# Amandaynzhou/CGC-Net

Hardware: AMD Instinct MI355X
Metric: cell-graphs/sec (fwd+bwd), batch=32, ~1800 nodes/16 feat (higher is better)
Workload: dtype f32; 1 GPU; C3: full CGC-Net (3 conv blocks + 2 DiffPool) fwd+bwd+Adam, 32 graphs/GPU/step, ~1803 nodes, ~16159 edges/graph, 16 feat, max_num_nodes=11404 (C1=1140, C2=114), flags=shipped; global_batch=32, nodes_per_batch=57711, parallelism=dp1, includes=CSR build + fwd + loss + bwd + grad all-reduce + Adam, step_sequencer=True, node_order=draw order, fused_adam=True, optimiser=cgc_adam_step (one launch; torch fused Adam arithmetic)

## Files before the change

### cgc-net_amd/csrc/exec.hip

```cpp
#include <stdio.h>
#include <stdlib.h>
#include <string.h>

#include "common.hpp"
#include "groups.hpp"

struct CatArgs {
  const float* src[4];
  int ld[4], width[4], off[4];
};
__global__ __launch_bounds__(256) void k_cat_cols(float* __restrict__ dst, int ldd, long long rows, int total_w, CatArgs a, int nsrc,
                                                  int accumulate) {
  const long long total = rows * total_w;
  for (long long i = blockIdx.x * 256ll + threadIdx.x; i < total; i += (long long)gridDim.x * 256) {
    const long long r = i / total_w;
    const int c = (int)(i - r * total_w);
    int s = 0;
#pragma unroll
    for (int k = 1; k < 4; ++k)
      if (k < nsrc && c >= a.off[k]) s = k;
    const float v = a.src[s][r * a.ld[s] + (c - a.off[s])];
    float* p = dst + r * ldd + c;
    *p = accumulate ? *p + v : v;
  }
}

extern "C" int cgc_cat_cols(float* dst, int ldd, int rows, int nsrc, const float* const* srcs, const int* lds, const int* widths,
                            int accumulate, cgc_stream_t stream) {
  if (nsrc < 1 || nsrc > 4) return CGC_EINVAL;
  CatArgs a;
  int off = 0;
  for (int k = 0; k < 4; ++k) {
    a.src[k] = k < nsrc ? srcs[k] : nullptr;
    a.ld[k] = k < nsrc ? lds[k] : 0;
    a.width[k] = k < nsrc ? widths[k] : 0;
    a.off[k] = off;
    off += a.width[k];
  }
  if (rows <= 0 || off <= 0) return 0;
  const long long total = (long long)rows * off;
  const long long blocks = (total + 255) / 256;
  hipLaunchKernelGGL(k_cat_cols, dim3((unsigned)(blocks < 4096 ? blocks : 4096)), dim3(256), 0, as_stream(stream), dst, ldd,
                     (long long)rows, off, a, nsrc, accumulate);
  CGC_RETURN_IF_LAUNCH_FAILED();
  return 0;
}

__global__ __launch_bounds__(256) void k_transpose(const float* __restrict__ src, int lds, int rows, int cols, float* __restrict__ dst,
                                                   int ldd) {
  __shared__ float t[32][33];
  const int tx = threadIdx.x & 31, ty = threadIdx.x >> 5;
  const int r0 = blockIdx.y * 32, c0 = blockIdx.x * 32;
  for (int j = ty; j < 32; j += 8) {
    const int r = r0 + j, c = c0 + tx;
    if (r < rows && c < cols) t[j][tx] = src[(size_t)r * lds + c];
  }
  __syncthreads();
  for (int j = ty; j < 32; j += 8) {
    const int c = c0 + j, r = r0 + tx;
    if (r < rows && c < cols) dst[(size_t)c * ldd + r] = t[tx][j];
  }
}

extern "C" int cgc_transpose(const float* src, int lds, int rows, int cols, float* dst, int ldd, cgc_stream_t stream) {
  if (rows <= 0 || cols <= 0) return 0;
  hipLaunchKernelGGL(k_transpose, dim3((unsigned)ceil_div(cols, 32), (unsigned)ceil_div(rows, 32)), dim3(256), 0, as_stream(stream), src,
                     lds, rows, cols, dst, ldd);
  CGC_RETURN_IF_LAUNCH_FAILED();
  return 0;
}

int reduce_batch_sum_rows(const float* ws, float* out, int parts, int rows, int width, int ldo, float beta, hipStream_t stream);

namespace {

struct Arena {
  float* base;
  size_t off = 0, high = 0;
  explicit Arena(float* b) : base(b) {}
  float* f(size_t n) {
    off = (off + 63) & ~(size_t)63;
    float* p = base + off;
    off += n;
    if (off > high) high = off;
    return p;
  }
  int* i(size_t n) { return reinterpret_cast<int*>(f(n)); }
  size_t mark() const { return off; }
  void release(size_t m) { off = m; }
};

struct Ctx {
  cgc_stream_t s;
  bool dry;
  Arena* scratch;
  float* gws;
  int64_t gws_floats;
  int gemm_mode = CGC_GEMM_EXACT;
};

static int fail_at(int rc, const char* what, int line) {
  static const bool verbose = getenv("CGC_EXEC_DEBUG") != nullptr;
  if (verbose) fprintf(stderr, "cgc exec.hip:%d: rc %d from %s\n", line, rc, what);
  return rc;
}
#define CALL(expr)                                              \
  do {                                                          \
    if (!c.dry) {                                               \
      const int rc__ = (expr);                                  \
      if (rc__ != 0) return fail_at(rc__, #expr, __LINE__);     \
    }                                                           \
  } while (0)
#define TRY(expr)                                               \
  do {                                                          \
    const int rc__ = (expr);                                    \
    if (rc__ != 0) return fail_at(rc__, #expr, __LINE__);       \
  } while (0)

inline int up(int v, int m) { return (v + m - 1) / m * m; }
inline int wide_ld(int F) { return (F >= 256 && F % 32 != 0) ? up(F, 32) : (F > 32 && F % 4 != 0) ? up(F, 4) : F; }
inline int pad4_ld(int c) { return (c > 32 && c % 4 != 0) ? up(c, 4) : c; }

int gemm(const Ctx& c, int tA, int tB, int M, int N, int K, const float* A, int lda, const float* B, int ldb, float beta, float* C, int ldc,
         const float* bias = nullptr, int batch = 1, int64_t sA = 0, int64_t sB = 0, int64_t sC = 0, const int* gptr = nullptr,
         int ragged = 0, int max_ragged = 0, int nx = 0, const float* const* xA = nullptr, const int* xlda = nullptr,
         const int64_t* xsA = nullptr, const float* const* xB = nullptr, const int* xldb = nullptr, const int64_t* xsB = nullptr,
         const int* xK = nullptr) {
  if (c.dry) return 0;
  return cgc_gemm_f32(tA, tB, M, N, K, 1.f, A, lda, B, ldb, beta, C, ldc, bias, batch, sA, sB, sC, gptr, ragged, max_ragged, nx, xA, xlda,
                      xsA, xB, xldb, xsB, xK, c.gws, c.gws_floats, c.gemm_mode, c.s);
}

int gemm_x1(const Ctx& c, int tA, int tB, int M, int N, int K, const float* A, int lda, const float* B, int ldb, float beta, float* C, int ldc,
            const float* bias, int batch, int64_t sA, int64_t sB, int64_t sC, const int* gptr, int ragged, int max_ragged, const float* xA,
            int xlda, int64_t xsA, const float* xB, int xldb, int64_t xsB, int xK) {
  return gemm(c, tA, tB, M, N, K, A, lda, B, ldb, beta, C, ldc, bias, batch, sA, sB, sC, gptr, ragged, max_ragged, 1, &xA, &xlda, &xsA,
              &xB, &xldb, &xsB, &xK);
}

int split_parts(int Fa, int Fb, int n) {
  const int tm = Fa <= 32 ? 32 : Fa <= 64 ? 64 : 128, tn = Fb <= 32 ? 32 : Fb <= 64 ? 64 : 128;
  const int tiles = ceil_div(Fa, tm) * ceil_div(Fb, tn);
  int best = 1;
  double best_score = -1.0;
  int hi = n / 512;
  if (hi > 128) hi = 128;
  if (hi < 1) hi = 1;
  for (int parts = 1; parts <= hi; ++parts) {
    const int blocks = tiles * parts, rounds = ceil_div(blocks, 512);
    const double fill = (double)blocks / ((double)rounds * 512.0);
    const double score = fill - 0.02 * rounds - (blocks < 256 ? 0.5 : 0.0);
    if (score > best_score + 1e-9) {
      best = parts;
      best_score = score;
    }
  }
  return best;
}

int gemm_tn_rows(const Ctx& c, const float* A, int lda, int Fa, const float* B, int ldb, int Fb, int n, float* out, int ldo = 0) {
  if (ldo <= 0) ldo = Fb;
  int parts = split_parts(Fa, Fb, n);
  if (parts == 1) return gemm(c, 1, 0, Fa, Fb, n, A, lda, B, ldb, 0.f, out, ldo);
  const int chunk = up(ceil_div(n, parts), 32);
  parts = ceil_div(n, chunk);
  const size_t m = c.scratch->mark();
  float* ws = c.scratch->f((size_t)parts * Fa * Fb);
  TRY(gemm(c, 1, 0, Fa, Fb, n, A, lda, B, ldb, 0.f, ws, Fb, nullptr, parts, 0, 0, (int64_t)Fa * Fb, nullptr, 3, chunk));
  CALL(reduce_batch_sum_rows(ws, out, parts, Fa, Fb, ldo, 0.f, as_stream(c.s)));
  c.scratch->release(m);
  return 0;
}

struct T3 {
  float* p;
  int b, r, c, ld;
  int64_t bs() const { return (int64_t)r * ld; }
};

int bgemm(const Ctx& c, const T3& A, const T3& B, const T3& C, int tA, int tB, float beta = 0.f) {
  const int batch = C.b, M = C.r, N = C.c, Kd = tA ? A.r : A.c;
  if (tA && !tB && M <= 128 && N <= 128 && Kd >= 512 && batch * 2 < 256 && C.ld == N) {
    int parts = Kd / 128;
    const int want = ceil_div(384, batch * (N > 64 ? 2 : 1));
    if (want < parts) parts = want;
    if (parts < 2) parts = 2;
    const int step = up(ceil_div(Kd, parts), 32);
    parts = ceil_div(Kd, step);
    const size_t m = c.scratch->mark();
    float* ws = c.scratch->f((size_t)batch * parts * M * N);
    TRY(gemm(c, 1, 0, M, N, Kd, A.p, A.ld, B.p, B.ld, 0.f, ws, N, nullptr, batch * parts, 0, 0, (int64_t)M * N, nullptr, 3, step));
    CALL(cgc_reduce_batched(ws, C.p, batch, parts, M * N, beta, c.s));
    c.scratch->release(m);
    return 0;
  }
  return gemm(c, tA, tB, M, N, Kd, A.p, A.ld, B.p, B.ld, beta, C.p, C.ld, nullptr, batch, A.bs(), B.bs(), C.bs());
}

int cat2(const Ctx& c, float* dst, int ldd, int rows, const float* a, int lda, int wa, const float* b, int ldb, int wb, int accumulate = 0) {
  const float* s[2] = {a, b};
  const int l[2] = {lda, ldb}, w[2] = {wa, wb};
  CALL(cgc_cat_cols(dst, ldd, rows, 2, s, l, w, accumulate, c.s));
  return 0;
}
int cat3(const Ctx& c, float* dst, int ldd, int rows, const float* a, int lda, int wa, const float* b, int ldb, int wb, const float* d, int ldd3,
         int wd) {
  const float* s[3] = {a, b, d};
  const int l[3] = {lda, ldb, ldd3}, w[3] = {wa, wb, wd};
  CALL(cgc_cat_cols(dst, ldd, rows, 3, s, l, w, 0, c.s));
  return 0;
}
int add1(const Ctx& c, float* dst, int ldd, int rows, const float* a, int lda, int wa) {
  const float* s[1] = {a};
  const int l[1] = {lda}, w[1] = {wa};
  CALL(cgc_cat_cols(dst, ldd, rows, 1, s, l, w, 1, c.s));
  return 0;
}

struct LayerP {
  const float *W, *b, *gamma, *beta;
  float *rm, *rv;
  int64_t* nbt;
  float eps, mom;
};
struct LayerS {
  float *hn, *rinv, *mean, *istd;
};

inline LayerP layer_params(const cgc_level_desc& d, const cgc_block_params* p, int k, int slot) {
  LayerP r;
  r.W = p->W[k];
  r.b = d.has_bias ? p->b[k] : nullptr;
  r.gamma = d.has_bn ? p->gamma[k] : nullptr;
  r.beta = d.has_bn ? p->beta[k] : nullptr;
  r.rm = d.has_bn ? p->running_mean[k] : nullptr;
  r.rv = d.has_bn ? p->running_var[k] : nullptr;
  r.nbt = d.has_bn ? p->num_batches_tracked[k] : nullptr;
  r.eps = d.bn_eps[slot];
  r.mom = d.bn_momentum[slot];
  return r;
}

inline size_t stats_ws_floats(int n, int F) { return (size_t)cgc_stats_ws_floats(n, F); }

int layer_fwd(const Ctx& c, const cgc_level_desc& d, const LayerP& p, const LayerS& s, const float* agg, int lda, int n, int fin, int F,
              float* y, int ldy, float* y2 = nullptr, int ldy2 = 0) {
  const size_t m = c.scratch->mark();
  const int batch_stats = d.has_bn && !d.eval;
  float* ws = batch_stats ? c.scratch->f(stats_ws_floats(n, F)) : nullptr;
  int fused = 0;
  if ((F >= 256 || F <= 32) && fin <= 32 && !c.dry) {
    int rc;
    if (F <= 32)
      rc = cgc_sage_narrow_fwd(agg, lda, p.W, p.b, n, fin, F, 1, d.act, s.hn, s.rinv, batch_stats, ws, d.count, p.eps, p.mom, p.rm, p.rv, p.nbt,
                               s.mean, s.istd, c.s);
    else
      rc = cgc_sage_wide_fwd(agg, lda, p.W, p.b, n, fin, F, 1, d.act, s.hn, F, s.rinv, batch_stats, ws, d.count, p.eps, p.mom, p.rm, p.rv, p.nbt,
                             s.mean, s.istd, c.s);
    if (rc == 0) fused = 1;
    else if (rc != CGC_EINVAL) return rc;
  }
  if (!fused) {
    TRY(gemm(c, 0, 0, n, F, fin, agg, lda, p.W, F, 0.f, s.hn, F, p.b));
    if (batch_stats)
      CALL(cgc_l2norm_act_bn(s.hn, n, F, 1, d.act, s.hn, s.rinv, ws, d.count, p.eps, p.mom, p.rm, p.rv, p.nbt, s.mean, s.istd, c.s));
    else
      CALL(cgc_l2norm_act_stats(s.hn, n, F, 1, d.act, s.hn, s.rinv, nullptr, nullptr, c.s));
  }
  if (d.has_bn && d.eval) CALL(cgc_bn_running_stats(p.rm, p.rv, F, p.eps, s.mean, s.istd, c.s));
  CALL(cgc_bn_act_apply(s.hn, n, F, d.act, d.has_bn ? s.mean : nullptr, s.istd, p.gamma, p.beta, y, ldy, y2, ldy2, c.s));
  c.scratch->release(m);
  return 0;
}

int layer_bwd(const Ctx& c, const cgc_level_desc& d, const LayerP& p, const LayerS& s, const float* agg, int lda, int n, int fin, int F,
              const float* dy, int ldy, float* dagg, int ldd, float* dwdb, float* sums) {
  const size_t m = c.scratch->mark();
  const int mode = d.has_bn ? 2 : 0;
  const size_t slot_floats = (size_t)(cgc_stats_blocks(n, F) > 1 ? cgc_stats_blocks(n, F) : 1) * 2 * F;
  if (d.has_bn) {
    float* ws = c.scratch->f(slot_floats);
    CALL(cgc_bn_bwd_reduce(dy, ldy, s.hn, n, F, d.act, s.mean, s.istd, sums, ws, c.s));
  }
  float* db = d.has_bias ? dwdb + (size_t)fin * F : nullptr;
  if (F <= 32 && fin <= 32) {
    float* ws = c.scratch->f((size_t)cgc_sage_narrow_ws_floats(n, fin, F));
    CALL(cgc_sage_narrow_bwd(dy, ldy, s.hn, s.rinv, n, F, d.act, 1, mode, s.mean, s.istd, p.gamma, d.has_bn ? sums : nullptr, d.count, agg,
                             lda, fin, p.W, dagg, ldd, dwdb, ws, c.s));
  } else {
    float* dh = c.scratch->f((size_t)n * F);
    float* ws = db ? c.scratch->f(slot_floats) : nullptr;
    CALL(cgc_bn_act_l2_bwd(dy, ldy, s.hn, s.rinv, n, F, d.act, 1, mode, s.mean, s.istd, p.gamma, d.has_bn ? sums : nullptr, d.count, dh, db, ws,
                           c.s));
    if (dagg) TRY(gemm(c, 0, 1, n, fin, F, dh, F, p.W, F, 0.f, dagg, ldd));
    TRY(gemm_tn_rows(c, agg, lda, fin, dh, F, F, n, dwdb));
  }
  c.scratch->release(m);
  return 0;
}

inline bool pairable(int fin_e, int F_e, int fin_p, int F_p) { return fin_e == fin_p && F_e == F_p && fin_e <= 32 && F_e <= 32; }

int layer_fwd_pair(const Ctx& c, const cgc_level_desc& d, const LayerP* p, const LayerS* s, const float* const* agg, int lda, int n, int fin, int F,
                   float* const* y, int ldy, float* const* y2, const int* ldy2) {
  const size_t m = c.scratch->mark();
  SnFwdPtrs g[2];
  SnFwdBn bn[2];
  BnApplyPtrs ap[2];
  const int batch_stats = d.has_bn && !d.eval;
  for (int i = 0; i < 2; ++i) {
    float* ws = batch_stats ? c.scratch->f(stats_ws_floats(n, F)) : nullptr;
    g[i] = SnFwdPtrs{agg[i], p[i].W, p[i].b, s[i].hn, s[i].rinv, ws};
    bn[i] = SnFwdBn{p[i].eps, p[i].mom, p[i].rm, p[i].rv, p[i].nbt, s[i].mean, s[i].istd};
    ap[i] = BnApplyPtrs{s[i].hn, d.has_bn ? s[i].mean : nullptr, s[i].istd, p[i].gamma, p[i].beta, y[i], y2[i], ldy2[i]};
  }
  CALL(sage_narrow_fwd_groups(g, bn, 2, lda, n, fin, F, 1, d.act, batch_stats, d.count, as_stream(c.s)));
  if (d.has_bn && d.eval)
    for (int i = 0; i < 2; ++i) CALL(cgc_bn_running_stats(p[i].rm, p[i].rv, F, p[i].eps, s[i].mean, s[i].istd, c.s));
  CALL(bn_act_apply_groups(ap, 2, n, F, d.act, ldy, as_stream(c.s)));
  c.scratch->release(m);
  return 0;
}

int layer_bwd_pair(const Ctx& c, const cgc_level_desc& d, const LayerP* p, const LayerS* s, const float* const* agg, int lda, int n, int fin, int F,
                   const float* const* dy, int ldy, float* const* dagg, int ldd, float* const* dwdb, float* const* sums) {
  const size_t m = c.scratch->mark();
  const int mode = d.has_bn ? 2 : 0;
  const size_t slot_floats = (size_t)(cgc_stats_blocks(n, F) > 1 ? cgc_stats_blocks(n, F) : 1) * 2 * F;
  if (d.has_bn) {
    BnRedPtrs r[2];
    for (int i = 0; i < 2; ++i) r[i] = BnRedPtrs{dy[i], s[i].hn, s[i].mean, s[i].istd, c.scratch->f(slot_floats)};
    CALL(bn_bwd_reduce_groups(r, sums, 2, ldy, n, F, d.act, as_stream(c.s)));
  }
  SnBwdPtrs g[2];
  for (int i = 0; i < 2; ++i)
    g[i] = SnBwdPtrs{dy[i], s[i].hn, s[i].rinv, s[i].mean, s[i].istd, p[i].gamma, d.has_bn ? sums[i] : nullptr, agg[i], p[i].W, dagg[i],
                     c.scratch->f((size_t)cgc_sage_narrow_ws_floats(n, fin, F))};
  CALL(sage_narrow_bwd_groups(g, dwdb, 2, ldy, n, F, d.act, 1, mode, d.count, lda, fin, ldd, as_stream(c.s)));
  c.scratch->release(m);
  return 0;
}

struct Level {
  const cgc_level_desc& d;
  int n, B, R, fin, H, E, AH, C, D, D3, wp, wt, ldp, ldC, ldP, ldW, ftot, npad_jk, seg_nmax;
  bool dense, pool, tall;
  float *At, *An, *invd, *ge1, *agg0, *pair[2], *xcat, *aggk[2], *hp3, *cat_e, *HS, *CS, *jk_out, *x12, *S, *P;
  float *G, *keep;
  bool reg;
  double reg_numel, reg_rows;
  int* arg;
  LayerS L[6];
  cgc_level_grad_layout gl;

  explicit Level(const cgc_level_desc& dd) : d(dd) {
    n = d.n; B = d.B; R = d.rows_per_graph; fin = d.fin; H = d.H; E = d.E; AH = d.AH; C = d.C;
    dense = d.level >= 2;
    pool = C > 0;
    D3 = 2 * H + E;
    D = d.jk ? H : D3;
    wp = pool ? H + AH : H;
    wt = 2 * wp + fin;
    ldp = dense ? wt : wp;
    ldC = pool ? wide_ld(C) : 0;
    ldP = dense ? pad4_ld(C) : ldC;
    ftot = 2 * AH + C;
    tall = pool && n >= 8 * C;
    ldW = wide_ld(C);
    npad_jk = up(n > 1 ? n : 1, 1024);
    seg_nmax = dense ? R : d.npad;
    reg = pool && (d.flags & 8);
    const double N = dense ? R : d.npad;
    reg_numel = (double)B * N * N;
    reg_rows = (double)B * N;
    memset(&gl, 0, sizeof(gl));
  }

  void layout_saved(Arena& a) {
    At = An = invd = ge1 = nullptr;
    if (dense) {
      if (d.renorm) At = a.f((size_t)n * R);
      An = a.f((size_t)n * R);
      invd = a.f(n);
      ge1 = a.f(n);
    }
    agg0 = a.f((size_t)n * fin);
    xcat = dense ? a.f((size_t)n * wt) : nullptr;
    for (int k = 0; k < 2; ++k) {
      pair[k] = dense ? xcat + (1 - k) * wp : a.f((size_t)n * wp);
      aggk[k] = a.f((size_t)n * wp);
    }
    hp3 = pool ? a.f((size_t)n * ldC) : nullptr;
    for (int k = 0; k < 6; ++k) {
      const bool emb = k < 3;
      if (!emb && !pool) {
        L[k].hn = L[k].rinv = L[k].mean = L[k].istd = nullptr;
        continue;
      }
      const int F = width_out(k);
      L[k].hn = a.f((size_t)n * F);
      L[k].rinv = a.f(n);
      L[k].mean = a.f(F);
      L[k].istd = a.f(F);
    }
    cat_e = a.f((size_t)n * D3);
    HS = CS = jk_out = nullptr;
    if (d.jk) {
      const int Hh = 3 * H / 2;
      HS = a.f((size_t)6 * Hh * npad_jk);
      CS = a.f((size_t)6 * Hh * npad_jk);
      jk_out = a.f((size_t)n * H);
    }
    arg = a.i((size_t)B * D);
    x12 = S = P = nullptr;
    if (pool) {
      x12 = a.f((size_t)n * 2 * AH);
      S = a.f((size_t)n * ldC);
      P = a.f((size_t)n * ldP);
    }
    G = keep = nullptr;
    if (reg) {
// ... 84 lines not shown
  TRY(aggregate(c, L, g, gptr, x_in, L.fin, L.fin, L.agg0));
  if (L.dense) {
    const float* s1[1] = {x_in};
    const int l1[1] = {L.fin}, w1[1] = {L.fin};
    CALL(cgc_cat_cols(L.xcat + 2 * wp, L.wt, n, 1, s1, l1, w1, 0, c.s));
  }
  for (int k = 0; k < 3; ++k) {
    const float* ain = k == 0 ? L.agg0 : L.aggk[k - 1];
    const int lda = k == 0 ? L.fin : wp;
    if (k < 2 && L.pool && pairable(L.width_in(k), H, L.width_in(3 + k), AH)) {
      const LayerP pp[2] = {layer_params(d, emb, k, k), layer_params(d, pl, k, 3 + k)};
      const LayerS ss[2] = {L.L[k], L.L[3 + k]};
      const float* ag[2] = {ain, k == 0 ? ain : ain + H};
      float* yy[2] = {L.pair[k], L.pair[k] + H};
      float* y2[2] = {L.cat_e + k * H, L.x12 + k * AH};
      const int l2[2] = {L.D3, 2 * AH};
      TRY(layer_fwd_pair(c, d, pp, ss, ag, lda, n, L.width_in(k), H, yy, L.ldp, y2, l2));
      if (k < 2) TRY(aggregate(c, L, g, gptr, L.pair[k], L.ldp, wp, L.aggk[k]));
      continue;
    }
    if (k < 2)
      TRY(layer_fwd(c, d, layer_params(d, emb, k, k), L.L[k], ain, lda, n, L.width_in(k), L.width_out(k), L.pair[k], L.ldp, L.cat_e + k * H,
                    L.D3));
    else
      TRY(layer_fwd(c, d, layer_params(d, emb, k, k), L.L[k], ain, lda, n, L.width_in(k), L.width_out(k), L.cat_e + 2 * H, L.D3));
    if (L.pool) {
      const float* ainp = k == 0 ? ain : ain + H;
      if (k < 2)
        TRY(layer_fwd(c, d, layer_params(d, pl, k, 3 + k), L.L[3 + k], ainp, lda, n, L.width_in(3 + k), L.width_out(3 + k), L.pair[k] + H, L.ldp,
                      L.x12 + k * AH, 2 * AH));
      else
        TRY(layer_fwd(c, d, layer_params(d, pl, k, 3 + k), L.L[3 + k], ainp, lda, n, L.width_in(3 + k), L.width_out(3 + k), L.hp3, L.ldC));
    }
    if (k < 2) TRY(aggregate(c, L, g, gptr, L.pair[k], L.ldp, wp, L.aggk[k]));
  }
  if (d.jk) CALL(cgc_jk_lstm_fwd(L.cat_e, n, L.npad_jk, H, jk->lstm, jk->w_att, jk->b_att, L.jk_out, L.HS, L.CS, c.s));
  CALL(cgc_segment_max_fwd(L.embed(), gptr, L.B, L.D, L.seg_nmax, readout, L.arg, c.s));
  if (!L.pool) return 0;
  {
    const bool wide_main = C > 2 * AH;
    const float* xm = wide_main ? L.hp3 : L.x12;
    const float* xe = wide_main ? L.x12 : L.hp3;
    const int ldm = wide_main ? L.ldC : 2 * AH, lde = wide_main ? 2 * AH : L.ldC;
    const int wm = wide_main ? C : 2 * AH, we = wide_main ? 2 * AH : C;
    const int om = wide_main ? 2 * AH : 0, oe = wide_main ? 0 : 2 * AH;
    if (L.tall) {
      const size_t m = c.scratch->mark();
      float* wt = c.scratch->f((size_t)L.ftot * L.ldW);
      CALL(cgc_transpose(pl->lin_W, L.ftot, C, L.ftot, wt, L.ldW, c.s));
      TRY(gemm_x1(c, 0, 0, n, C, wm, xm, ldm, wt + (size_t)om * L.ldW, L.ldW, 0.f, L.S, L.ldC, pl->lin_b, 1, 0, 0, 0, nullptr, 0, 0, xe, lde, 0,
                  wt + (size_t)oe * L.ldW, L.ldW, 0, we));
      c.scratch->release(m);
    } else {
      TRY(gemm_x1(c, 0, 1, n, C, wm, xm, ldm, pl->lin_W + om, L.ftot, 0.f, L.S, L.ldC, pl->lin_b, 1, 0, 0, 0, nullptr, 0, 0, xe, lde, 0,
                  pl->lin_W + oe, L.ftot, 0, we));
    }
  }
  CALL(cgc_softmax_fwd(L.S, n, C, L.ldC, L.S, c.s));
  if (!L.dense) {
    CALL(cgc_spmm_graphs(g->rowptr, g->col, nullptr, g->val, nullptr, nullptr, L.S, L.P, n, C, L.ldC, gptr, L.B, d.nmax, 1 | (g->spatial ? 4 : 0), g->gorder, c.s));
    TRY(gemm(c, 1, 0, C, L.D, 0, L.S, L.ldC, L.embed(), L.D, 0.f, x_out, L.D, nullptr, L.B, 0, 0, (int64_t)C * L.D, gptr, 2, d.nmax));
    TRY(gemm(c, 1, 0, C, C, 0, L.S, L.ldC, L.P, L.ldC, 0.f, A_out, C, nullptr, L.B, 0, 0, (int64_t)C * C, gptr, 2, d.nmax));
  } else {
    const T3 s3{L.S, L.B, L.R, C, L.ldC}, e3{const_cast<float*>(L.embed()), L.B, L.R, L.D, L.D}, p3{L.P, L.B, L.R, C, L.ldP};
    const T3 a3{const_cast<float*>(d.renorm ? L.At : A_in), L.B, L.R, L.R, L.R};
    TRY(bgemm(c, s3, e3, T3{x_out, L.B, C, L.D, L.D}, 1, 0));
    TRY(bgemm(c, a3, s3, p3, 0, 0));
    TRY(bgemm(c, s3, p3, T3{A_out, L.B, C, C, C}, 1, 0));
  }
  if (L.reg) TRY(reg_fwd(c, L, g, gptr, A_in, A_out, reg_out));
  return 0;
}

int level_bwd_blocks(const Ctx& c, Level& L, const cgc_block_params* emb, const cgc_block_params* pl, const cgc_jk_params* jk,
                     const cgc_graph* g, const int* gptr, const float* x_in, const float* A_in, float* d_embed, const float* dx12,
                     float* dagg1, const float* gAt, float* grads, float* d_x_in, float* d_A_in) {
  const cgc_level_desc& d = L.d;
  Arena& sc = *c.scratch;
  const int n = L.n, H = L.H, AH = L.AH, wp = L.wp, B = L.B, R = L.R, D3 = L.D3, fin = L.fin;
  auto sums = [&](int k) { return grads + L.gl.W[k] + (int64_t)L.width_in(k) * L.width_out(k) + L.width_out(k); };
  float* d_cat = d_embed;
  if (d.jk) {
    d_cat = sc.f((size_t)n * D3);
    const size_t m = sc.mark();
    float* ws = sc.f((size_t)cgc_jk_bwd_ws_floats(H));
    CALL(cgc_jk_lstm_bwd_flat(L.cat_e, d_embed, n, L.npad_jk, H, jk->lstm, jk->w_att, jk->b_att, L.HS, L.CS, d_cat, grads + L.gl.jk, ws, c.s));
    sc.release(m);
  }
  float* dagg[2];
  const int ldg = L.ldp;
  float* const gcat = dagg1 != nullptr ? dagg1 : sc.f((size_t)n * ldg);
  dagg[1] = gcat;
  TRY(layer_bwd(c, d, layer_params(d, emb, 2, 2), L.L[2], L.aggk[1], wp, n, H, L.E, d_cat + 2 * H, D3, dagg[1], ldg, grads + L.gl.W[2], sums(2)));
  float* dpair = nullptr;
  for (int k = 1; k >= 0; --k) {
    dpair = sc.f((size_t)n * wp);
    TRY(aggregate_t(c, L, g, gptr, dagg[k], ldg, wp, dpair));
    if (L.pool) TRY(cat2(c, dpair, wp, n, d_cat + k * H, D3, H, dx12 + k * AH, 2 * AH, AH, 1));
    else TRY(add1(c, dpair, wp, n, d_cat + k * H, D3, H));
    const bool first = k == 0;
    const bool need_in = !first || L.dense;
    const float* ain = first ? L.agg0 : L.aggk[k - 1];
    const int lda = first ? fin : wp;
    const int fi_e = L.width_in(k), fi_p = L.width_in(3 + k);
    float *de = nullptr, *dp = nullptr;
    int ldd = ldg;
    if (need_in && !first) {
      de = dagg[0] = L.dense ? gcat + wp : sc.f((size_t)n * wp);
      dp = de + H;
    } else if (need_in) {
      de = gcat + 2 * wp;
      dp = L.pool ? sc.f((size_t)n * ldg) : nullptr;
    }
    if (L.pool && pairable(fi_e, H, fi_p, AH)) {
      const LayerP pp[2] = {layer_params(d, emb, k, k), layer_params(d, pl, k, 3 + k)};
      const LayerS ss[2] = {L.L[k], L.L[3 + k]};
      const float* ag[2] = {ain, first ? ain : ain + H};
      const float* dyy[2] = {dpair, dpair + H};
      float* dg[2] = {de, dp};
      float* dw[2] = {grads + L.gl.W[k], grads + L.gl.W[3 + k]};
      float* sm[2] = {sums(k), sums(3 + k)};
      TRY(layer_bwd_pair(c, d, pp, ss, ag, lda, n, fi_e, H, dyy, wp, dg, ldd, dw, sm));
    } else {
      TRY(layer_bwd(c, d, layer_params(d, emb, k, k), L.L[k], ain, lda, n, fi_e, H, dpair, wp, de, ldd, grads + L.gl.W[k], sums(k)));
      if (L.pool)
        TRY(layer_bwd(c, d, layer_params(d, pl, k, 3 + k), L.L[3 + k], first ? ain : ain + H, lda, n, fi_p, AH, dpair + H, wp, dp, ldd,
                      grads + L.gl.W[3 + k], sums(3 + k)));
    }
    if (first && L.dense) {
      if (L.pool) TRY(add1(c, de, ldg, n, dp, ldg, fin));
      TRY(aggregate_t(c, L, g, gptr, de, ldg, fin, d_x_in));
      float* dAn = sc.f((size_t)n * R);
      TRY(bgemm(c, T3{gcat, B, R, L.wt, L.wt}, T3{L.xcat, B, R, L.wt, L.wt}, T3{dAn, B, R, R, R}, 0, 1));
      CALL(cgc_adj_prep_bwd(A_in, L.An, L.invd, L.ge1, dAn, gAt, n, R, d.renorm ? d.renorm_p : -1.f, d_A_in, c.s));
    }
  }
  return 0;
}

int level_bwd(const Ctx& c, Level& L, const cgc_block_params* emb, const cgc_block_params* pl, const cgc_jk_params* jk, const cgc_graph* g,
              const int* gptr, const float* x_in, const float* A_in, const float* d_readout, const float* d_xo, const float* d_ao, float* grads,
              float* d_x_in, float* d_A_in, const float* d_reg = nullptr) {
  const cgc_level_desc& d = L.d;
  Arena& sc = *c.scratch;
  const int n = L.n, H = L.H, AH = L.AH, wp = L.wp, C = L.C, D = L.D, B = L.B, R = L.R;
  float* d_embed = sc.f((size_t)n * D);
  CALL(cgc_segment_max_bwd_full(d_readout, L.arg, gptr, B, D, L.seg_nmax, d_embed, c.s));
  float *dx12 = nullptr, *gAt = nullptr;
  if (L.pool) {
    float *Gs = nullptr, *coef = nullptr;
    if (L.reg) {
      float* dao = sc.f((size_t)B * C * C);
      Gs = sc.f((size_t)B * C * C);
      coef = sc.f(4);
      CALL(cgc_diffpool_reg_bwd_prep(d_reg, L.keep, L.reg_numel, L.reg_rows, d_ao, dao, L.G, Gs, B, C, coef, c.s));
      d_ao = dao;
    }
    const size_t m0 = sc.mark();
    float* ds = sc.f((size_t)n * L.ldC);
    if (!L.dense) {
      float* dp = sc.f((size_t)n * L.ldC);
      TRY(gemm(c, 0, 0, 0, C, C, L.S, L.ldC, d_ao, C, 0.f, dp, L.ldC, nullptr, B, 0, (int64_t)C * C, 0, gptr, 1, d.nmax));
      CALL(cgc_spmm_graphs(g->t_rowptr, g->t_col, nullptr, g->t_val, nullptr, nullptr, dp, ds, n, C, L.ldC, gptr, B, d.nmax, 2 | (g->spatial ? 4 : 0), g->gorder,
                           c.s));
      TRY(gemm_x1(c, 0, 1, 0, C, C, L.P, L.ldC, d_ao, C, 1.f, ds, L.ldC, nullptr, B, 0, (int64_t)C * C, 0, gptr, 1, d.nmax, L.embed(), D, 0, d_xo,
                  D, (int64_t)C * D, D));
      if (L.reg) TRY(gemm(c, 0, 0, 0, C, C, L.S, L.ldC, Gs, C, 1.f, ds, L.ldC, nullptr, B, 0, (int64_t)C * C, 0, gptr, 1, d.nmax));
      TRY(gemm(c, 0, 0, 0, D, C, L.S, L.ldC, d_xo, D, 1.f, d_embed, D, nullptr, B, 0, (int64_t)C * D, 0, gptr, 1, d.nmax));
    } else {
      gAt = sc.f((size_t)n * R);
      float* dP = sc.f((size_t)n * L.ldP);
      const T3 s3{L.S, B, R, C, L.ldC}, e3{const_cast<float*>(L.embed()), B, R, D, D}, p3{L.P, B, R, C, L.ldP};
      const T3 a3{const_cast<float*>(d.renorm ? L.At : A_in), B, R, R, R};
      const T3 dao{const_cast<float*>(d_ao), B, C, C, C}, dxo{const_cast<float*>(d_xo), B, C, D, D};
      const T3 ds3{ds, B, R, C, L.ldC}, dP3{dP, B, R, C, L.ldP};
      TRY(bgemm(c, p3, dao, ds3, 0, 1));
      TRY(bgemm(c, s3, dao, dP3, 0, 0));
      TRY(bgemm(c, dP3, s3, T3{gAt, B, R, R, R}, 0, 1));
      TRY(bgemm(c, a3, dP3, ds3, 1, 0, 1.f));
      TRY(bgemm(c, e3, dxo, ds3, 0, 1, 1.f));
      TRY(bgemm(c, s3, dxo, T3{d_embed, B, R, D, D}, 0, 0, 1.f));
      if (L.reg) {
        TRY(bgemm(c, s3, T3{Gs, B, C, C, C}, ds3, 0, 0, 1.f));
        CALL(cgc_diffpool_reg_adj_bwd(a3.p, (int64_t)n * R, coef, gAt, 1, c.s));
      }
    }
    if (L.reg) CALL(cgc_diffpool_reg_entropy_bwd(L.S, n, C, L.ldC, coef, ds, L.ldC, c.s));
    float* dz = sc.f((size_t)n * L.ldC);
    {
      const size_t m = sc.mark();
      float* ws = sc.f((size_t)(cgc_stats_blocks(n, C) > 1 ? cgc_stats_blocks(n, C) : 1) * 2 * C);
      CALL(cgc_softmax_bwd(L.S, ds, n, C, L.ldC, dz, grads + L.gl.lin_b, ws, c.s));
      sc.release(m);
    }
    dx12 = sc.f((size_t)n * 2 * AH);
    float* dy3 = sc.f((size_t)n * L.ldC);
    TRY(gemm(c, 0, 0, n, 2 * AH, C, dz, L.ldC, pl->lin_W, L.ftot, 0.f, dx12, 2 * AH));
    TRY(gemm(c, 0, 0, n, C, C, dz, L.ldC, pl->lin_W + 2 * AH, L.ftot, 0.f, dy3, L.ldC));
    {
      float* dW = grads + L.gl.lin_W;
      TRY(gemm_tn_rows(c, dz, L.ldC, C, L.x12, 2 * AH, 2 * AH, n, dW, L.ftot));
      TRY(gemm_tn_rows(c, dz, L.ldC, C, L.hp3, L.ldC, C, n, dW + 2 * AH, L.ftot));
    }
    (void)m0;
    float* dagg1 = sc.f((size_t)n * L.ldp);
    TRY(layer_bwd(c, d, layer_params(d, pl, 2, 5), L.L[5], L.aggk[1] + H, wp, n, AH, C, dy3, L.ldC, dagg1 + H, L.ldp, grads + L.gl.W[5],
                  grads + L.gl.W[5] + (int64_t)AH * C + C));
    return level_bwd_blocks(c, L, emb, pl, jk, g, gptr, x_in, A_in, d_embed, dx12, dagg1, gAt, grads, d_x_in, d_A_in);
  }
  return level_bwd_blocks(c, L, emb, pl, jk, g, gptr, x_in, A_in, d_embed, nullptr, nullptr, nullptr, grads, d_x_in, d_A_in);
}

template <class Body>
int run_level(const cgc_level_desc* d, float* saved, float* scratch, cgc_stream_t stream, Body&& body) {
  Level L(*d);
  Arena sv(saved), sc(scratch);
  L.layout_saved(sv);
  L.layout_grads();
  Ctx c{stream, false, &sc, nullptr, cgc_gemm_ws_floats()};
  c.gws = sc.f((size_t)c.gws_floats);
  c.gemm_mode = (d->flags & 2) ? CGC_GEMM_SPLIT_BF16 : (d->flags & 4) ? CGC_GEMM_SPLIT_F16 : CGC_GEMM_EXACT;
  return body(c, L);
}

}

extern "C" int cgc_level_supported(const cgc_level_desc* d) {
  if (d == nullptr || d->level < 1 || d->level > 3 || d->B < 1 || d->B > 65535 || d->n < 1) return 0;
  if (d->fin < 1 || d->H < 1 || d->E < 1 || d->act < 0 || d->act > 3) return 0;
  if (d->level >= 2 && (d->rows_per_graph < 1 || (long long)d->B * d->rows_per_graph != d->n)) return 0;
  if (d->level == 1 && (d->nmax < 1 || d->npad < d->nmax)) return 0;
  if (d->C > 0 && (d->AH < 1 || d->H + d->AH > 256 || (2 * d->AH) % 4 != 0)) return 0;
  if (d->C == 0 && d->level == 1) return 0;
  if ((d->flags & ~14) || (d->flags & 6) == 6) return 0;
  if ((d->flags & 8) && d->C == 0) return 0;
  if (d->jk && (d->E != d->H || !cgc_jk_matrix_core(d->H))) return 0;
  return 1;
}

extern "C" int64_t cgc_level_saved_floats(const cgc_level_desc* d) {
  if (!cgc_level_supported(d)) return -1;
  Level L(*d);
  Arena a(nullptr);
  L.layout_saved(a);
  return (int64_t)a.high + 64;
}

extern "C" int cgc_level_grad_layout_of(const cgc_level_desc* d, cgc_level_grad_layout* out) {
  if (!cgc_level_supported(d) || out == nullptr) return CGC_EINVAL;
  Level L(*d);
  L.layout_grads();
  *out = L.gl;
  return 0;
}

extern "C" int64_t cgc_level_scratch_floats(const cgc_level_desc* d) {
  if (!cgc_level_supported(d)) return -1;
  Level L(*d);
  Arena sv(nullptr);
  L.layout_saved(sv);
  L.layout_grads();
  size_t high = 0;
  for (int pass = 0; pass < (d->eval ? 1 : 2); ++pass) {
    Arena sc(nullptr);
    Ctx c{nullptr, true, &sc, nullptr, 0};
    sc.f((size_t)cgc_gemm_ws_floats());
    cgc_block_params bp;
    memset(&bp, 0, sizeof(bp));
    cgc_jk_params jp;
    memset(&jp, 0, sizeof(jp));
    cgc_graph gr;
    memset(&gr, 0, sizeof(gr));
    const int rc = pass == 0 ? level_fwd(c, L, &bp, &bp, &jp, &gr, nullptr, nullptr, nullptr, nullptr, nullptr, nullptr)
                             : level_bwd(c, L, &bp, &bp, &jp, &gr, nullptr, nullptr, nullptr, nullptr, nullptr, nullptr, nullptr, nullptr, nullptr);
    if (rc != 0) return -1;
    if (sc.high > high) high = sc.high;
  }
  return (int64_t)high + 64;
}

extern "C" int cgc_level_fwd(const cgc_level_desc* d, const cgc_block_params* emb, const cgc_block_params* pool, const cgc_jk_params* jk,
                             const cgc_graph* g, const int* gptr, const float* x_in, const float* A_in, float* saved, float* scratch,
                             float* readout, float* x_out, float* A_out, const float** assign_out, int* assign_ld, float* reg_out,
                             cgc_stream_t stream) {
  if (!cgc_level_supported(d) || saved == nullptr || scratch == nullptr) return CGC_EINVAL;
  if (!aligned16(saved) || !aligned16(scratch)) return CGC_EINVAL;
  if ((d->flags & 8) && reg_out == nullptr) return CGC_EINVAL;
  return run_level(d, saved, scratch, stream, [&](const Ctx& c, Level& L) {
    const int rc = level_fwd(c, L, emb, pool, jk, g, gptr, x_in, A_in, readout, x_out, A_out, reg_out);
    if (assign_out != nullptr) *assign_out = L.S;
    if (assign_ld != nullptr) *assign_ld = L.ldC;
    return rc;
  });
}

extern "C" int cgc_level_bwd(const cgc_level_desc* d, const cgc_block_params* emb, const cgc_block_params* pool, const cgc_jk_params* jk,
                             const cgc_graph* g, const int* gptr, const float* x_in, const float* A_in, const float* saved, float* scratch,
                             const float* d_readout, const float* d_x_out, const float* d_A_out, const float* d_reg, float* grads,
                             float* d_x_in, float* d_A_in, cgc_stream_t stream) {
  if (!cgc_level_supported(d) || saved == nullptr || scratch == nullptr || grads == nullptr || d->eval) return CGC_EINVAL;
  if (!aligned16(saved) || !aligned16(scratch) || !aligned16(grads)) return CGC_EINVAL;
  if ((d->flags & 8) && d_reg == nullptr) return CGC_EINVAL;
  return run_level(d, const_cast<float*>(saved), scratch, stream, [&](const Ctx& c, Level& L) {
    return level_bwd(c, L, emb, pool, jk, g, gptr, x_in, A_in, d_readout, d_x_out, d_A_out, grads, d_x_in, d_A_in, d_reg);
  });
}
```

### cgc-net_amd/csrc/gemm.hip

```cpp
#include "gemm_common.hpp"

template <int ROWS>
struct KContigLoader {
  static constexpr int UNITS = ROWS * (BK / 4);
  static constexpr int PER_T = (UNITS + 255) / 256;
  float4 reg[PER_T];
  __device__ __forceinline__ void load(const float* __restrict__ base, int ld, int row0, int row_lim, int k0, int k_lim, bool vec_ok) {
#pragma unroll
    for (int i = 0; i < PER_T; ++i) {
      const int u = threadIdx.x + i * 256;
      float4 v = make_float4(0.f, 0.f, 0.f, 0.f);
      if (UNITS % 256 == 0 || u < UNITS) {
        const int row = row0 + u / (BK / 4);
        const int k = k0 + (u % (BK / 4)) * 4;
        if (row < row_lim && k < k_lim) {
          const float* p = base + (size_t)row * ld + k;
          if (vec_ok && k + 3 < k_lim) {
            v = *reinterpret_cast<const float4*>(p);
          } else {
            v.x = p[0];
            if (k + 1 < k_lim) v.y = p[1];
            if (k + 2 < k_lim) v.z = p[2];
            if (k + 3 < k_lim) v.w = p[3];
          }
        }
      }
      reg[i] = v;
    }
  }
  __device__ __forceinline__ void load_fast(const float* __restrict__ base, int ld, int row0, int row_last, int k0) {
#pragma unroll
    for (int i = 0; i < PER_T; ++i) {
      const int u = threadIdx.x + i * 256;
      const int row = min(row0 + u / (BK / 4), row_last);
      reg[i] = *reinterpret_cast<const float4*>(base + (size_t)row * ld + k0 + (u % (BK / 4)) * 4);
    }
  }
  __device__ __forceinline__ void offsets(unsigned (&off)[PER_T], int ld, int row0, int row_last) const {
#pragma unroll
    for (int i = 0; i < PER_T; ++i) {
      const int u = threadIdx.x + i * 256;
      off[i] = (unsigned)min(row0 + u / (BK / 4), row_last) * (unsigned)ld * 4u + (unsigned)(u % (BK / 4)) * 16u;
    }
  }
  static __device__ __forceinline__ unsigned tile_soffset(int , int k0) { return (unsigned)k0 * 4u; }
  __device__ __forceinline__ void load_buf_part(int i, __amdgpu_buffer_rsrc_t rsrc, const unsigned (&off)[PER_T], unsigned soff) {
    reg[i] = __builtin_bit_cast(float4, __builtin_amdgcn_raw_buffer_load_b128(rsrc, off[i], soff, 0));
  }
  __device__ __forceinline__ void load_fast_masked(const float* __restrict__ base, int ld, int row0, int row_last, int k0, int k_lim) {
    const int k_last4 = (k_lim - 1) & ~3;
#pragma unroll
    for (int i = 0; i < PER_T; ++i) {
      const int u = threadIdx.x + i * 256;
      const int row = min(row0 + u / (BK / 4), row_last);
      const int k = k0 + (u % (BK / 4)) * 4;
      float4 v = *reinterpret_cast<const float4*>(base + (size_t)row * ld + min(k, k_last4));
      if (k >= k_lim) v.x = 0.f;
      if (k + 1 >= k_lim) v.y = 0.f;
      if (k + 2 >= k_lim) v.z = 0.f;
      if (k + 3 >= k_lim) v.w = 0.f;
      reg[i] = v;
    }
  }
  __device__ __forceinline__ void store_part(int i, float* __restrict__ lds) const {
    const int u = threadIdx.x + i * 256;
    if (UNITS % 256 == 0 || u < UNITS)
      *reinterpret_cast<float4*>(&lds[(u / (BK / 4)) * KC_LD + (u % (BK / 4)) * 4]) = reg[i];
  }
  __device__ __forceinline__ void store(float* __restrict__ lds) const {
#pragma unroll
    for (int i = 0; i < PER_T; ++i) store_part(i, lds);
  }
};

template <int COLS>
struct MnContigLoader {
  static constexpr int UNITS = BK * (COLS / 4);
  static constexpr int PER_T = (UNITS + 255) / 256;
  float4 reg[PER_T];
  __device__ __forceinline__ void load(const float* __restrict__ base, int ld, int col0, int col_lim, int k0, int k_lim, bool vec_ok) {
#pragma unroll
    for (int i = 0; i < PER_T; ++i) {
      const int u = threadIdx.x + i * 256;
// ... 485 lines not shown
  if (ragged == 1 && (transA || a.gptr == nullptr)) return CGC_EINVAL;
  if (ragged == 2 && (!transA || transB || a.gptr == nullptr || a.nx > 0)) return CGC_EINVAL;
  if (ragged == 3 && (!transA || transB || a.nx > 0 || max_ragged <= 0 || K <= 0 || batch % ceil_div(K, max_ragged) != 0)) return CGC_EINVAL;
  if (ragged < 0 || ragged > 3) return CGC_EINVAL;
  a.chunk = ragged == 3 ? max_ragged : 0;
  const int m_extent = ragged == 1 ? max_ragged : M;
  if (m_extent <= 0) return 0;
  const int k_extent = ragged >= 2 ? max_ragged : K;
  constexpr int shortk_max = 160, fill_min = 448;
  const bool sk = k_extent <= shortk_max && a.nx == 0;
  const long long fill = (long long)ceil_div(m_extent, 128) * batch;
  const bool want_split = mode == CGC_GEMM_SPLIT_BF16, want_half = mode == CGC_GEMM_SPLIT_F16;
  auto big_route = [&](bool shortk, float* w) -> int {
    if ((want_split || want_half) && !shortk && !(transA && transB) && gemm_all_fast(a, transA, transB, batch, m_extent, k_extent)) {
      int rc = want_half ? gemm_half_launch(a, transA, transB, batch, m_extent, k_extent, w, ws_floats, stream) : CGC_EINVAL;
      if (rc == CGC_EINVAL) rc = gemm_split_launch(a, transA, transB, batch, m_extent, k_extent, w, ws_floats, stream);
      if (rc != CGC_EINVAL) return rc;
    }
    return launch_cfg<2, 2, 2, 2>(a, transA, transB, batch, m_extent, k_extent, shortk, w, ws_floats, stream);
  };
  const int force = g_force_cfg;
  if (force > 0) {
    const bool fsk = force >= 20 ? true : force >= 10 ? false : sk;
    switch (force % 10) {
      case 1: return big_route(fsk, ws);
      case 2: return launch_cfg<4, 1, 1, 2>(a, transA, transB, batch, m_extent, k_extent, fsk, ws, ws_floats, stream);
      case 3: return launch_cfg<1, 4, 2, 1>(a, transA, transB, batch, m_extent, k_extent, fsk, ws, ws_floats, stream);
      case 4: return launch_cfg<2, 2, 1, 1>(a, transA, transB, batch, m_extent, k_extent, fsk, ws, ws_floats, stream);
      case 5: return launch_cfg<4, 1, 1, 1>(a, transA, transB, batch, m_extent, k_extent, fsk, ws, ws_floats, stream);
      case 6: return launch_cfg<1, 4, 1, 1>(a, transA, transB, batch, m_extent, k_extent, fsk, ws, ws_floats, stream);
      default: break;
    }
  }
  if (N <= 32) return launch_cfg<4, 1, 1, 1>(a, transA, transB, batch, m_extent, k_extent, sk, ws, ws_floats, stream);
  if (N <= 64) {
    if (m_extent > 64 && fill < fill_min) return launch_cfg<2, 2, 1, 1>(a, transA, transB, batch, m_extent, k_extent, sk, ws, ws_floats, stream);
    return launch_cfg<4, 1, 1, 2>(a, transA, transB, batch, m_extent, k_extent, sk, ws, ws_floats, stream);
  }
  if (m_extent <= 32) return launch_cfg<1, 4, 1, 1>(a, transA, transB, batch, m_extent, k_extent, sk, ws, ws_floats, stream);
  if (m_extent <= 64) return launch_cfg<1, 4, 2, 1>(a, transA, transB, batch, m_extent, k_extent, sk, ws, ws_floats, stream);
  if (fill * ceil_div(N, 128) < fill_min) {
    if (N <= 128) {
      if (k_extent > 256 && m_extent > 128)
        return launch_cfg<4, 1, 1, 1>(a, transA, transB, batch, m_extent, k_extent, sk, ws, ws_floats, stream);
      return launch_cfg<2, 2, 1, 1>(a, transA, transB, batch, m_extent, k_extent, sk, ws, ws_floats, stream);
    }
    if (transA) {
      if (!sk && ws != nullptr && k_extent >= 24 * BK) return big_route(sk, ws);
      return launch_cfg<4, 1, 1, 2>(a, transA, transB, batch, m_extent, k_extent, sk, ws, ws_floats, stream);
    }
    return launch_cfg<1, 4, 2, 1>(a, transA, transB, batch, m_extent, k_extent, sk, ws, ws_floats, stream);
  }
  return big_route(sk, ws);
}

extern "C" int cgc_gemm_f32(int transA, int transB, int M, int N, int K, float alpha, const float* A, int lda, const float* B, int ldb,
                            float beta, float* C, int ldc, const float* bias, int batch, int64_t strideA, int64_t strideB,
                            int64_t strideC, const int* gptr, int ragged, int max_ragged, int nx, const float* const* xA,
                            const int* xlda, const int64_t* xstrideA, const float* const* xB, const int* xldb,
                            const int64_t* xstrideB, const int* xK, float* ws, int64_t ws_floats, int mode, cgc_stream_t stream_) {
  if (nx < 0 || nx > 2) return CGC_EINVAL;
  if (mode != CGC_GEMM_EXACT && mode != CGC_GEMM_SPLIT_BF16 && mode != CGC_GEMM_SPLIT_F16) return CGC_EINVAL;
  GemmArgs a;
  a.A = A; a.B = B; a.C = C; a.bias = bias; a.gptr = gptr;
  a.M = M; a.N = N; a.K = K; a.lda = lda; a.ldb = ldb; a.ldc = ldc;
  a.strideA = strideA; a.strideB = strideB; a.strideC = strideC;
  a.alpha = alpha; a.beta = beta; a.ragged = ragged; a.tiles_n = 0;
  a.per_batch = a.nb = 0; a.ws = nullptr; a.resident = 0; a.s_max = 1; a.chunk = 0; a.scale = nullptr;
  for (int i = 0; i < 2; ++i) { a.xA[i] = a.xB[i] = nullptr; a.xlda[i] = a.xldb[i] = a.xK[i] = 0; a.xsA[i] = a.xsB[i] = 0; }
  int kept = 0;
  for (int i = 0; i < nx; ++i) {
    if (xK[i] <= 0) continue;
    a.xA[kept] = xA[i]; a.xB[kept] = xB[i]; a.xlda[kept] = xlda[i]; a.xldb[kept] = xldb[i]; a.xK[kept] = xK[i];
    a.xsA[kept] = xstrideA[i]; a.xsB[kept] = xstrideB[i];
    ++kept;
  }
  a.nx = kept;
  return gemm_dispatch(a, transA, transB, batch, max_ragged, ws, ws_floats, mode, as_stream(stream_));
}

__global__ void k_reduce_batch_sum(const float* __restrict__ ws, float* __restrict__ out, int parts, long long numel, float beta, int width,
                                   int ldo) {
  for (long long i = blockIdx.x * (long long)blockDim.x + threadIdx.x; i < numel; i += (long long)gridDim.x * blockDim.x) {
    float s = 0.f;
    for (int p = 0; p < parts; ++p) s += ws[(size_t)p * numel + i];
    const long long o = (i / width) * ldo + i % width;
    out[o] = beta != 0.f ? s + beta * out[o] : s;
  }
}

__global__ __launch_bounds__(256) void k_reduce_many_parts(const float* __restrict__ ws, float* __restrict__ out, int parts, int numel,
                                                           float beta, int width, int ldo) {
  __shared__ float part[8][32];
  const int cl = threadIdx.x & 31, grp = threadIdx.x >> 5;
  const int c = blockIdx.x * 32 + cl;
  ws += (size_t)blockIdx.y * parts * numel;
  out += (size_t)blockIdx.y * numel;
  float s = 0.f;
  if (c < numel) {
    float a[8];
#pragma unroll
    for (int u = 0; u < 8; ++u) a[u] = 0.f;
    int k = grp;
    for (; k + 56 < parts; k += 64) {
#pragma unroll
      for (int u = 0; u < 8; ++u) a[u] += ws[(size_t)(k + 8 * u) * numel + c];
    }
    for (; k < parts; k += 8) a[0] += ws[(size_t)k * numel + c];
    s = ((a[0] + a[1]) + (a[2] + a[3])) + ((a[4] + a[5]) + (a[6] + a[7]));
  }
  part[grp][cl] = s;
  __syncthreads();
  if (grp == 0 && c < numel) {
    float t = part[0][cl];
#pragma unroll
    for (int g = 1; g < 8; ++g) t += part[g][cl];
    const int o = (c / width) * ldo + c % width;
    out[o] = beta != 0.f ? t + beta * out[o] : t;
  }
}

extern "C" int cgc_reduce_batched(const float* ws, float* out, int outer, int parts, int numel, float beta, cgc_stream_t stream) {
  if (numel <= 0 || outer <= 0) return 0;
  if (outer > 65535) return CGC_EINVAL;
  hipLaunchKernelGGL(k_reduce_many_parts, dim3((unsigned)ceil_div(numel, 32), (unsigned)outer), dim3(256), 0, as_stream(stream), ws, out,
                     parts, numel, beta, numel, numel);
  CGC_RETURN_IF_LAUNCH_FAILED();
  return 0;
}

int reduce_batch_sum_rows(const float* ws, float* out, int parts, int rows, int width, int ldo, float beta, hipStream_t stream) {
  const int64_t numel = (int64_t)rows * width;
  if (numel <= 0) return 0;
  if (width <= 0 || ldo < width || numel > 0x7fffffff) return CGC_EINVAL;
  if (parts >= 16 && numel <= (1 << 20)) {
    hipLaunchKernelGGL(k_reduce_many_parts, dim3((unsigned)ceil_div((int)numel, 32), 1u), dim3(256), 0, stream, ws, out, parts, (int)numel, beta,
                       width, ldo);
  } else {
    const int64_t blocks = ceil_div64(numel, 256);
    hipLaunchKernelGGL(k_reduce_batch_sum, dim3((unsigned)(blocks < 4096 ? blocks : 4096)), dim3(256), 0, stream, ws, out, parts,
                       (long long)numel, beta, width, ldo);
  }
  CGC_RETURN_IF_LAUNCH_FAILED();
  return 0;
}

extern "C" int cgc_reduce_batch_sum(const float* ws, float* out, int parts, int64_t numel, float beta, cgc_stream_t stream) {
  if (numel <= 0) return 0;
  if (parts >= 16 && numel <= (1 << 20)) return cgc_reduce_batched(ws, out, 1, parts, (int)numel, beta, stream);
  const int64_t blocks = ceil_div64(numel, 256);
  const int w = numel <= 0x7fffffff ? (int)numel : 0x7fffffff;
  hipLaunchKernelGGL(k_reduce_batch_sum, dim3((unsigned)(blocks < 4096 ? blocks : 4096)), dim3(256), 0, as_stream(stream), ws, out,
                     parts, (long long)numel, beta, w, w);
  CGC_RETURN_IF_LAUNCH_FAILED();
  return 0;
}
```

### cgc-net_amd/csrc/groups.hpp

```cpp
#pragma once
#include "common.hpp"

struct SnFwdPtrs {
  const float *agg, *W, *bias;
  float *hn, *rinv, *ws;
};
struct SnFwdBn {
  float eps, momentum;
  float *running_mean, *running_var;
  int64_t* nbt;
  float *mean, *istd;
};
struct SnBwdPtrs {
  const float *dy, *hn, *rinv, *mean, *istd, *gamma, *sums, *agg, *W;
  float *dagg, *ws;
};
struct StatsFinPtrs {
  const float* ws;
  float *running_mean, *running_var, *mean, *istd;
  long long* nbt;
  float eps, momentum;
};
struct BnApplyPtrs {
  const float *hn, *mean, *istd, *gamma, *beta;
  float *y, *y2;
  int ldy2;
};
struct BnRedPtrs {
  const float *dy, *hn, *mean, *istd;
  float* ws;
};

int sage_narrow_fwd_groups(const SnFwdPtrs* g, const SnFwdBn* bn, int ng, int lda, int n, int K, int F, int normalize, int act, int stats,
                           double count, hipStream_t st);
int sage_narrow_bwd_groups(const SnBwdPtrs* g, float* const* dwdb, int ng, int ldy, int n, int F, int act, int normalize, int mode, double count,
                           int lda, int fin, int ldd, hipStream_t st);
int bn_act_apply_groups(const BnApplyPtrs* g, int ng, int n, int F, int act, int ldy, hipStream_t stream);
int bn_bwd_reduce_groups(const BnRedPtrs* g, float* const* sums, int ng, int ldy, int n, int F, int act, hipStream_t stream);
int launch_stats_finalize_groups(const StatsFinPtrs* g, int ng, int slots, int F, double count, hipStream_t stream);
int launch_reduce_slots_f32_pair(const float* ws0, float* out0, const float* ws1, float* out1, int ng, int slots, int width, hipStream_t stream);
```

### cgc-net_amd/csrc/jk.hip

```cpp
#include "jk.hpp"

template <int C>
__device__ __forceinline__ void jk_fill_lds(const JkWeights& w, float4* Wt, float4* B4, float* watt, int nthreads) {
  constexpr int H = JkDims<C>::H, KIN = JkDims<C>::KIN;
  for (int idx = threadIdx.x; idx < 2 * H * KIN; idx += nthreads) {
    const int d = idx / (H * KIN), rem = idx - d * H * KIN, j = rem / KIN, k = rem - j * KIN;
    float v[4];
#pragma unroll
    for (int g = 0; g < 4; ++g) {
      const int row = g * H + j;
      v[g] = k < C ? w.w_ih[d][row * C + k] : w.w_hh[d][row * H + (k - C)];
    }
    Wt[idx] = make_float4(v[0], v[1], v[2], v[3]);
  }
  for (int idx = threadIdx.x; idx < 2 * H; idx += nthreads) {
    const int d = idx / H, j = idx - d * H;
    float v[4];
#pragma unroll
    for (int g = 0; g < 4; ++g) v[g] = w.b_ih[d][g * H + j] + w.b_hh[d][g * H + j];
    B4[idx] = make_float4(v[0], v[1], v[2], v[3]);
    watt[idx] = w.w_att[idx];
  }
  if (threadIdx.x == 0) watt[2 * H] = w.b_att[0];
}
// ... 255 lines not shown
extern "C" int cgc_jk_matrix_core(int C) { return C == 4 || C == 8 || C == 12 || C == 16 || C == 20; }

#define JK_FOR_EACH_C(X) X(2) X(4) X(6) X(8) X(10) X(12) X(14) X(16) X(18) X(20) X(22) X(24) X(26) X(28) X(30) X(32)

template <int C>
static void jk_allow_lds() {
  static bool done_f[CGC_MAX_DEVICES] = {}, done_b[CGC_MAX_DEVICES] = {};
  cgc_allow_lds(reinterpret_cast<const void*>(&k_jk_fwd<C>), (int)JkDims<C>::lds_bytes, done_f);
  cgc_allow_lds(reinterpret_cast<const void*>(&k_jk_bwd<C>), (int)JkDims<C>::lds_bytes, done_b);
}

template <int C>
static int launch_jk_fwd(const float* xs, int n, int npad, const JkWeights& w, float* out, float* HS, float* CS, hipStream_t st) {
  jk_allow_lds<C>();
  hipLaunchKernelGGL(k_jk_fwd<C>, dim3(ceil_div(2 * n, JK_THREADS)), dim3(JK_THREADS), JkDims<C>::lds_bytes, st, xs, n, npad, w, out, HS, CS);
  CGC_RETURN_IF_LAUNCH_FAILED();
  return 0;
}
template <int C>
static int launch_jk_bwd(const float* xs, const float* dout, int n, int npad, const JkWeights& w, const float* HS, const float* CS,
                         float* dxs, float* DGT, float* INT, float* DHC, hipStream_t st) {
  jk_allow_lds<C>();
  hipLaunchKernelGGL(k_jk_bwd<C>, dim3(ceil_div(2 * npad, JK_THREADS)), dim3(JK_THREADS), JkDims<C>::lds_bytes, st, xs, dout, n, npad, w,
                     HS, CS, dxs, DGT, INT, DHC);
  CGC_RETURN_IF_LAUNCH_FAILED();
  return 0;
}

extern "C" int cgc_jk_lstm_fwd(const float* xs, int n, int npad, int C, const float* const* lstm, const float* w_att,
                               const float* b_att, float* out, float* HS, float* CS, cgc_stream_t stream) {
  if (n <= 0) return 0;
  if (!jk_npad_ok(n, npad)) return CGC_EINVAL;
  JkWeights w;
  fill_weights(w, lstm, w_att, b_att);
  const int rc = jk_mfma_fwd(xs, n, npad, C, w, out, HS, CS, as_stream(stream));
  if (rc != CGC_EINVAL) return rc;
  switch (C) {
#define X(C_) case C_: return launch_jk_fwd<C_>(xs, n, npad, w, out, HS, CS, as_stream(stream));
    JK_FOR_EACH_C(X)
#undef X
    default: return CGC_EINVAL;
  }
}

extern "C" int cgc_jk_lstm_bwd(const float* xs, const float* dout, int n, int npad, int C, const float* const* lstm,
                               const float* w_att, const float* b_att, const float* HS, const float* CS, float* dxs, float* DGT,
                               float* INT, float* DHC, cgc_stream_t stream) {
  if (n <= 0) return 0;
  if (!jk_npad_ok(n, npad)) return CGC_EINVAL;
  JkWeights w;
  fill_weights(w, lstm, w_att, b_att);
  const int rc = jk_mfma_bwd(xs, dout, n, npad, C, w, HS, CS, dxs, DGT, INT, as_stream(stream));
  if (rc != CGC_EINVAL) return rc;
  switch (C) {
#define X(C_) case C_: return launch_jk_bwd<C_>(xs, dout, n, npad, w, HS, CS, dxs, DGT, INT, DHC, as_stream(stream));
    JK_FOR_EACH_C(X)
#undef X
    default: return CGC_EINVAL;
  }
}

extern "C" int64_t cgc_jk_bwd_ws_floats(int C) { return jk_mfma_bwd_ws_floats(C); }

extern "C" int cgc_jk_lstm_bwd_params(const float* xs, const float* dout, int n, int npad, int C, const float* const* lstm,
                                      const float* w_att, const float* b_att, const float* HS, const float* CS, float* dxs,
                                      float* G, float* ws, cgc_stream_t stream) {
  if (n <= 0) return 0;
  if (!jk_npad_ok(n, npad)) return CGC_EINVAL;
  JkWeights w;
  fill_weights(w, lstm, w_att, b_att);
  return jk_mfma_bwd_params(xs, dout, n, npad, C, w, HS, CS, dxs, G, ws, as_stream(stream));
}

extern "C" int cgc_jk_lstm_bwd_flat(const float* xs, const float* dout, int n, int npad, int C, const float* const* lstm,
                                    const float* w_att, const float* b_att, const float* HS, const float* CS, float* dxs,
                                    float* flat, float* ws, cgc_stream_t stream) {
  if (n <= 0) return 0;
  if (!jk_npad_ok(n, npad)) return CGC_EINVAL;
  JkWeights w;
  fill_weights(w, lstm, w_att, b_att);
  return jk_mfma_bwd_flat(xs, dout, n, npad, C, w, HS, CS, dxs, flat, ws, as_stream(stream));
}

__global__ void k_jk_unpack(const float* __restrict__ G, int C, int H, float* __restrict__ flat) {
  const int NI = C + 2 * H + 1, NG = 4 * H + 1;
  const int per_dir = 4 * H * C + 4 * H * H + 8 * H, total = 2 * per_dir + 2 * H + 1;
  for (int i = blockIdx.x * blockDim.x + threadIdx.x; i < total; i += gridDim.x * blockDim.x) {
    float v;
    if (i < 2 * per_dir) {
      const int d = i / per_dir;
      int e = i - d * per_dir;
      const float* Gd = G + (size_t)d * NG * NI;
      if (e < 4 * H * C) v = Gd[(e / C) * NI + (e % C)];
      else if ((e -= 4 * H * C) < 4 * H * H) v = Gd[(e / H) * NI + C + (e % H)];
      else { e -= 4 * H * H; v = Gd[(e % (4 * H)) * NI + C + H]; }
    } else {
      const int e = i - 2 * per_dir;
      if (e < 2 * H) v = G[((size_t)(e / H) * NG + 4 * H) * NI + C + H + 1 + (e % H)];
      else v = G[(size_t)(4 * H) * NI + C + H];
    }
    flat[i] = v;
  }
}

extern "C" int64_t cgc_jk_param_grad_floats(int C) {
  const int64_t H = 3 * (int64_t)C / 2;
  return 2 * (4 * H * C + 4 * H * H + 8 * H) + 2 * H + 1;
}

extern "C" int cgc_jk_unpack_param_grads(const float* G, int C, float* flat, cgc_stream_t stream) {
  if (C <= 0) return CGC_EINVAL;
  const int H = 3 * C / 2;
  const int total = (int)cgc_jk_param_grad_floats(C);
  hipLaunchKernelGGL(k_jk_unpack, dim3(ceil_div(total, 256)), dim3(256), 0, as_stream(stream), G, C, H, flat);
  CGC_RETURN_IF_LAUNCH_FAILED();
  return 0;
}
```

### cgc-net_amd/csrc/jk.hpp

```cpp
#pragma once
#include "common.hpp"

__device__ __forceinline__ float sigmoidf_(float x) { return 1.f / (1.f + expf(-x)); }

template <int C>
struct JkDims {
  static constexpr int H = 3 * C / 2;
  static constexpr int KIN = C + H;
  static constexpr size_t lds_bytes = sizeof(float4) * (2 * H * KIN + 2 * H) + sizeof(float) * (2 * H + 4);
};

struct JkWeights {
  const float* w_ih[2];
  const float* w_hh[2];
  const float* b_ih[2];
  const float* b_hh[2];
  const float* w_att;
  const float* b_att;
};


int jk_mfma_fwd(const float* xs, int n, int npad, int C, const JkWeights& w, float* out, float* HS, float* CS, hipStream_t st);
int jk_mfma_bwd(const float* xs, const float* dout, int n, int npad, int C, const JkWeights& w, const float* HS, const float* CS,
                float* dxs, float* DGT, float* INT, hipStream_t st);
int64_t jk_mfma_bwd_ws_floats(int C);
int jk_mfma_bwd_params(const float* xs, const float* dout, int n, int npad, int C, const JkWeights& w, const float* HS,
                       const float* CS, float* dxs, float* G, float* ws, hipStream_t st);
int jk_mfma_bwd_flat(const float* xs, const float* dout, int n, int npad, int C, const JkWeights& w, const float* HS, const float* CS,
                     float* dxs, float* flat, float* ws, hipStream_t st);
```

### cgc-net_amd/csrc/jk_mfma.hip

```cpp
#include "jk.hpp"

typedef float floatx16 __attribute__((ext_vector_type(16)));

constexpr int JKB_TILES = 2;
constexpr int JKB_THREADS = JKB_TILES * 128;

template <int C>
struct JkM {
  static constexpr int H = 3 * C / 2;
  static constexpr int XG = (C + 7) / 8;
  static constexpr int HG = (H + 7) / 8;
  static constexpr int NQ = XG + HG;
  static constexpr int W_FLOATS = 2 * 4 * NQ * 32 * 8;
  static constexpr int B_OFF = W_FLOATS;
  static constexpr int A_OFF = B_OFF + 2 * 4 * 32;
  static constexpr int S_OFF = A_OFF + 2 * 32 + 4;
  static constexpr int TOTAL = S_OFF + 2 * 2 * 3 * 32;
  static_assert(H <= 32 && C % 4 == 0, "one 32-row tile per gate; 16-byte x fragments");
};

__device__ __forceinline__ float jk_rcp(float d) {
  const float r = __builtin_amdgcn_rcpf(d);
  return fmaf(fmaf(-d, r, 1.f), r, r);
}
__device__ __forceinline__ float jk_exp(float a) {
  const float t = a * 0x1.715476p+0f;
  const float r = fmaf(a, 0x1.4ae0cp-26f, fmaf(a, 0x1.715476p+0f, -t));
  const float e = __builtin_amdgcn_exp2f(t);
  return fmaf(e, t >= 16.f ? r * 0x1.62e43p-1f : 0.f, e);
}
__device__ __forceinline__ float fast_sigmoid(float x) { return jk_rcp(1.f + jk_exp(fminf(-x, 87.f))); }
__device__ __forceinline__ float fast_tanh(float x) {
  const float ax = fabsf(x), x2 = x * x;
  const float e = __expf(-2.f * ax);
  const float big = (1.f - e) * jk_rcp(1.f + e);
  const float small = ax * fmaf(x2, fmaf(x2, fmaf(x2, fmaf(x2, 62.f / 2835.f, -17.f / 315.f), 2.f / 15.f), -1.f / 3.f), 1.f);
  return copysignf(ax < 0.25f ? small : big, x);
}

template <int C>
__device__ __forceinline__ void jkm_fill(const JkWeights& w, float* lds, int nthreads) {
  using M = JkM<C>;
  constexpr int H = M::H, XG = M::XG, NQ = M::NQ;
  {
    const int tt = threadIdx.x & 3, lhi = (threadIdx.x >> 2) & 1, j = (threadIdx.x >> 3) & 31;
    float v[2 * 4 * NQ];
#pragma unroll
    for (int it = 0; it < 2 * 4 * NQ; ++it) {
      const int q = it % NQ, g = (it / NQ) & 3, d = it / (4 * NQ);
      v[it] = 0.f;
      if (q < XG) {
        const int k = 8 * q + 4 * lhi + tt;
        if (j < H && k < C) v[it] = w.w_ih[d][(g * H + j) * C + k];
      } else {
        const int k = 8 * (q - XG) + 4 * lhi + tt;
        if (j < H && k < H) v[it] = w.w_hh[d][(g * H + j) * H + k];
      }
    }
#pragma unroll
    for (int it = 0; it < 2 * 4 * NQ; ++it) lds[it * 256 + threadIdx.x] = v[it];
  }
  for (int idx = threadIdx.x; idx < 2 * 4 * 32; idx += nthreads) {
    const int j = idx & 31, g = (idx >> 5) & 3, d = idx >> 7;
    lds[M::B_OFF + idx] = j < H ? w.b_ih[d][g * H + j] + w.b_hh[d][g * H + j] : 0.f;
  }
  for (int idx = threadIdx.x; idx < 2 * 32; idx += nthreads) {
    const int j = idx & 31, d = idx >> 5;
    lds[M::A_OFF + idx] = j < H ? w.w_att[d * H + j] : 0.f;
  }
  if (threadIdx.x == 0) lds[M::A_OFF + 64] = w.b_att[0];
}

template <int C>
__global__ __launch_bounds__(JKB_THREADS) void k_jk_bwd_mfma(const float* __restrict__ xs, const float* __restrict__ dout, int n, int npad,
                                                     const JkWeights w, const float* __restrict__ HS, const float* __restrict__ CS,
                                                     float* __restrict__ dxs, float* __restrict__ DGT, float* __restrict__ INT,
                                                     float* __restrict__ ) {
  using M = JkM<C>;
  constexpr int H = M::H, XG = M::XG, HG = M::HG, NQ = M::NQ;
  constexpr int NG = 4 * H + 1, NI = C + 2 * H + 1;
  extern __shared__ __attribute__((aligned(16))) float lds[];
  if (threadIdx.x < 256) jkm_fill<C>(w, lds, 256);
  __syncthreads();
// ... 146 lines not shown
        if (8 * q + 4 * lhi < C) {
          inT[(size_t)(8 * q + 4 * lhi + 0) * ktot + col] = xt[q].x;
          inT[(size_t)(8 * q + 4 * lhi + 1) * ktot + col] = xt[q].y;
          inT[(size_t)(8 * q + 4 * lhi + 2) * ktot + col] = xt[q].z;
          inT[(size_t)(8 * q + 4 * lhi + 3) * ktot + col] = xt[q].w;
        }
      }
#pragma unroll
      for (int q = 0; q < HG; ++q) {
        const float4 wa = *reinterpret_cast<const float4*>(Al + 8 * q);
        const float was[4] = {wa.x, wa.y, wa.z, wa.w};
#pragma unroll
        for (int u = 0; u < 4; ++u) {
          const int r = 4 * q + u, j = u + 8 * q + 4 * lhi;
          const float gi = fast_sigmoid(acc[0][r]), gf = fast_sigmoid(acc[1][r]);
          const float gg = fast_tanh(acc[2][r]), go = fast_sigmoid(acc[3][r]);
          const float c = gf * cprev[r] + gi * gg;
          const float th = fast_tanh(c);
          const float dh = fmaf(dst, was[u], dhc[r]);
          const float dc = fmaf(dh * go, 1.f - th * th, dcc[r]);
          dcc[r] = dc * gf;
          const float qi = dc * gg * gi * (1.f - gi), qf = dc * cprev[r] * gf * (1.f - gf);
          const float qg = dc * gi * (1.f - gg * gg), qo = dh * th * go * (1.f - go);
          acc[0][r] = qi; acc[1][r] = qf; acc[2][r] = qg; acc[3][r] = qo;
          if (8 * q + u < H && j < H) {
            dgt[(size_t)(0 * H + j) * ktot + col] = qi;
            dgt[(size_t)(1 * H + j) * ktot + col] = qf;
            dgt[(size_t)(2 * H + j) * ktot + col] = qg;
            dgt[(size_t)(3 * H + j) * ktot + col] = qo;
            inT[(size_t)(C + j) * ktot + col] = hprev[r];
            inT[(size_t)(C + H + 1 + j) * ktot + col] = go * th;
          }
        }
      }
      floatx16 dh2, dx2;
#pragma unroll
      for (int r = 0; r < 16; ++r) { dh2[r] = 0.f; dx2[r] = 0.f; }
#pragma unroll
      for (int g = 0; g < 4; ++g)
#pragma unroll
        for (int q = 0; q < HG; ++q) {
          float ah[4], ax[4];
#pragma unroll
          for (int u = 0; u < 4; ++u) {
            ax[u] = WtX[g * NQ * 256 + (8 * q + u) * 8];
            ah[u] = s > 0 ? WtH[g * NQ * 256 + (8 * q + u) * 8] : 0.f;
          }
#pragma unroll
          for (int u = 0; u < 4; ++u) {
            dx2 = __builtin_amdgcn_mfma_f32_32x32x2f32(ax[u], acc[g][4 * q + u], dx2, 0, 0, 0);
            if (s > 0) dh2 = __builtin_amdgcn_mfma_f32_32x32x2f32(ah[u], acc[g][4 * q + u], dh2, 0, 0, 0);
          }
        }
      if (s > 0) dhc = dh2;
#pragma unroll
      for (int q = 0; q < XG; ++q) Ex[(t * XG + q) * 64] = make_float4(dx2[4 * q + 0], dx2[4 * q + 1], dx2[4 * q + 2], dx2[4 * q + 3]);
    }

    __syncthreads();
    if (d == 0 && valid) {
      const float4* Eo = Ex + 3 * XG * 64;
#pragma unroll
      for (int q = 0; q < XG; ++q) {
        if (8 * q + 4 * lhi < C) {
          const float4 dy = *reinterpret_cast<const float4*>(dout + (size_t)node * C + 8 * q + 4 * lhi);
#pragma unroll
          for (int t = 0; t < 3; ++t) {
            const float4 p0 = Ex[(t * XG + q) * 64], p1 = Eo[(t * XG + q) * 64];
            float4 v;
            v.x = fmaf(a3[t], dy.x, p0.x + p1.x); v.y = fmaf(a3[t], dy.y, p0.y + p1.y);
            v.z = fmaf(a3[t], dy.z, p0.z + p1.z); v.w = fmaf(a3[t], dy.w, p0.w + p1.w);
            *reinterpret_cast<float4*>(dxs + (size_t)node * 3 * C + t * C + 8 * q + 4 * lhi) = v;
          }
        }
      }
    }
    __syncthreads();
  }
}

__global__ void k_jk_pg_fold(const float* __restrict__ part, int P, int P2, int per, float* __restrict__ tmp) {
  const int e = blockIdx.x * blockDim.x + threadIdx.x, p2 = blockIdx.y, d = blockIdx.z;
  if (e >= per) return;
  const float* src = part + ((size_t)d * P + (size_t)p2 * 16) * per + e;
  const int cnt = min(16, P - p2 * 16);
  float a = 0.f;
  for (int k = 0; k < cnt; ++k) a += src[(size_t)k * per];
  tmp[((size_t)d * P2 + p2) * per + e] = a;
}

template <int C>
struct JkU {
  static constexpr int H = 3 * C / 2, XG = (C + 7) / 8, HG = (H + 7) / 8, NQ = XG + HG;
  static constexpr int W_FLOATS = 2 * 4 * NQ * 256;
  static constexpr int B_OFF = W_FLOATS;
  static constexpr int A_OFF = B_OFF + 256;
  static constexpr int S_OFF = A_OFF + 68;
  static constexpr int X_OFF = S_OFF + 768;
  static constexpr int FWD_TOTAL = X_OFF + 2 * 8 * 256;
  static constexpr int Q_OFF = S_OFF + 768;
  static constexpr int I_OFF = Q_OFF + 8 * 1152;
  static constexpr int P_OFF = I_OFF + 4 * 1152;
  static constexpr int BWD_TOTAL = P_OFF + 8 * XG * 256;
  static constexpr int PG_SLOTS = 37;
  static constexpr int PG_FLOATS = 8 * PG_SLOTS * 64;
  static_assert(H <= 30 && C % 4 == 0, "column 31 of the h tile is the bias column; 16-byte x fragments");
};

template <int C>
__device__ __forceinline__ void jku_fill(const JkWeights& w, float* lds) {
  using U = JkU<C>;
  constexpr int H = U::H, XG = U::XG, NQ = U::NQ;
  const int tid = threadIdx.x, d = tid >> 8;
  const float* wih = d ? w.w_ih[1] : w.w_ih[0];
  const float* whh = d ? w.w_hh[1] : w.w_hh[0];
  const float* bih = d ? w.b_ih[1] : w.b_ih[0];
  const float* bhh = d ? w.b_hh[1] : w.b_hh[0];
  const int tt = tid & 3, lhi = (tid >> 2) & 1, rho = (tid >> 3) & 31, g = rho >> 3, u = rho & 7;
  float v[4 * NQ];
#pragma unroll
  for (int it = 0; it < 4 * NQ; ++it) {
    const int q = it % NQ, ww = it / NQ, j = 8 * ww + u;
    const int jr = j < H ? j : H - 1;
    if (q < XG) {
      const int k = 8 * q + 4 * lhi + tt;
      const float ld = wih[(g * H + jr) * C + (k < C ? k : C - 1)];
      v[it] = (j < H && k < C) ? ld : 0.f;
    } else {
      const int k = 8 * (q - XG) + 4 * lhi + tt;
      const float ld = whh[(g * H + jr) * H + (k < H ? k : H - 1)];
      v[it] = (j < H && k < H) ? ld : 0.f;
    }
  }
#pragma unroll
  for (int it = 0; it < 4 * NQ; ++it) lds[(d * 4 * NQ + it) * 256 + (tid & 255)] = v[it];
  if ((tid & 255) < 128) {
    const int r2 = tid & 31, ww = (tid >> 5) & 3, j = 8 * ww + (r2 & 7), gg = r2 >> 3;
    lds[U::B_OFF + (d * 4 + ww) * 32 + r2] = j < H ? bih[gg * H + j] + bhh[gg * H + j] : 0.f;
  } else if ((tid & 255) < 160) {
    const int j = tid & 31;
    lds[U::A_OFF + d * 32 + j] = j < H ? w.w_att[d * H + j] : 0.f;
  }
  if (tid == 0) lds[U::A_OFF + 64] = w.b_att[0];
}

template <int C>
__global__ __launch_bounds__(512) void k_jku_fwd(const float* __restrict__ xs, int n, int npad, const JkWeights w,
                                                 float* __restrict__ out, float* __restrict__ HS, float* __restrict__ CS) {
  using U = JkU<C>;
  constexpr int H = U::H, XG = U::XG, HG = U::HG, NQ = U::NQ;
  extern __shared__ __attribute__((aligned(16))) float lds[];
  jku_fill<C>(w, lds);
  __syncthreads();
  const int lane = threadIdx.x & 63, l31 = lane & 31, lhi = lane >> 5;
  const int wave = __builtin_amdgcn_readfirstlane(threadIdx.x >> 6), d = wave & 1, ww = wave >> 1;
  const float4* Wl = reinterpret_cast<const float4*>(lds) + (size_t)(d * 4 + ww) * NQ * 64 + l31 * 2 + lhi;
  const float* Bl = lds + U::B_OFF + (d * 4 + ww) * 32 + 4 * lhi;
  const float4 wa4 = *reinterpret_cast<const float4*>(lds + U::A_OFF + d * 32 + 8 * ww + 4 * lhi);
  const float was[4] = {wa4.x, wa4.y, wa4.z, wa4.w};
  float* Sx = lds + U::S_OFF;
  float4* Hx = reinterpret_cast<float4*>(lds + U::X_OFF);
  const int ntiles = (n + 31) / 32;

  for (int tile = blockIdx.x; tile < ntiles; tile += gridDim.x) {
    const int node = tile * 32 + l31;
    const bool valid = node < n, keep = node < npad;
    const float* xrow = xs + (size_t)(valid ? node : 0) * 3 * C + 4 * lhi;
    float cst[4] = {0.f, 0.f, 0.f, 0.f};
    float4 hq[HG];
#pragma unroll
    for (int q = 0; q < HG; ++q) hq[q] = make_float4(0.f, 0.f, 0.f, 0.f);
// ... 306 lines not shown
          dW1 = __builtin_amdgcn_mfma_f32_32x32x2f32(af[kk], bf1[kk], dW1, 0, 0, 0);
        }
      }
      __builtin_amdgcn_sched_barrier(0);
      if (s > 0) {
        const float4* P0 = reinterpret_cast<const float4*>(lds + U::Q_OFF) + ww * 64 + lane;
        float4 a = P0[(0 * 2 + d) * 288];
        const float4 b = P0[(1 * 2 + d) * 288], c2 = P0[(2 * 2 + d) * 288], e = P0[(3 * 2 + d) * 288];
        a.x += b.x; a.y += b.y; a.z += b.z; a.w += b.w;
        a.x += c2.x; a.y += c2.y; a.z += c2.z; a.w += c2.w;
        a.x += e.x; a.y += e.y; a.z += e.z; a.w += e.w;
        dhc[0] = a.x; dhc[1] = a.y; dhc[2] = a.z; dhc[3] = a.w;
      }
      if (ww < XG) {
        float4 a = Dx[((0 * 2 + d) * XG + ww) * 64 + lane];
#pragma unroll
        for (int v = 1; v < 4; ++v) {
          const float4 b = Dx[((v * 2 + d) * XG + ww) * 64 + lane];
          a.x += b.x; a.y += b.y; a.z += b.z; a.w += b.w;
        }
        if (s == 2) dxs2 = a;
        else if (s == 1) dxs1 = a;
        else dxs0 = a;
      }
      __syncthreads();
    }
    if (ww < XG) {
      Dx[((d * XG + ww) * 3 + (d ? 2 : 0)) * 64 + lane] = dxs0;
      Dx[((d * XG + ww) * 3 + 1) * 64 + lane] = dxs1;
      Dx[((d * XG + ww) * 3 + (d ? 0 : 2)) * 64 + lane] = dxs2;
    }
    __syncthreads();
    if (d == 0 && ww < XG && valid && 8 * ww + 4 * lhi < C) {
      const int q = ww;
      const float4 dy = *reinterpret_cast<const float4*>(dout + (size_t)node * C + 8 * q + 4 * lhi);
#pragma unroll
      for (int t = 0; t < 3; ++t) {
        const float4 p0 = Dx[((0 * XG + q) * 3 + t) * 64 + lane], p1 = Dx[((1 * XG + q) * 3 + t) * 64 + lane];
        float4 v;
        v.x = fmaf(a3[t], dy.x, p0.x + p1.x); v.y = fmaf(a3[t], dy.y, p0.y + p1.y);
        v.z = fmaf(a3[t], dy.z, p0.z + p1.z); v.w = fmaf(a3[t], dy.w, p0.w + p1.w);
        *reinterpret_cast<float4*>(dxs + (size_t)node * 3 * C + t * C + 8 * q + 4 * lhi) = v;
      }
    }
  }
#undef JKU_LOAD_STEP
  float* pw = PART + (size_t)blockIdx.x * U::PG_FLOATS + (size_t)wave * U::PG_SLOTS * 64 + lane;
#pragma unroll
  for (int r = 0; r < 16; ++r) { pw[r * 64] = dW0[r]; pw[(16 + r) * 64] = dW1[r]; }
#pragma unroll
  for (int o = 16; o >= 1; o >>= 1) {
#pragma unroll
    for (int i = 0; i < 4; ++i) wacc[i] += __shfl_xor(wacc[i], o);
    bacc += __shfl_xor(bacc, o);
  }
#pragma unroll
  for (int i = 0; i < 4; ++i) pw[(32 + i) * 64] = wacc[i];
  pw[36 * 64] = bacc;
}

template <int C>
__device__ __forceinline__ float jku_gather(const float* __restrict__ tmp, int P2, int d, int row, int col, int att) {
  using U = JkU<C>;
  constexpr int H = U::H, per = U::PG_FLOATS;
  float a = 0.f;
  if (att < 0) {
    const int g = row / H, j = row - g * H, ww = j >> 3, u = j & 7, lhi = u >> 2, r = 4 * g + (u & 3);
    const int m = col < C ? 1 : 0;
    const int kin = col < C ? col : (col == C + H ? 31 : col - C);
    const int e = ((ww * 2 + d) * U::PG_SLOTS + m * 16 + r) * 64 + lhi * 32 + kin;
    for (int k = 0; k < P2; ++k) a += tmp[(size_t)k * per + e];
  } else if (att < H) {
    const int j = att, ww = j >> 3, u = j & 7, lhi = u >> 2;
    const int e = ((ww * 2 + d) * U::PG_SLOTS + 32 + (u & 3)) * 64 + lhi * 32;
    for (int k = 0; k < P2; ++k) a += tmp[(size_t)k * per + e];
  } else {
    for (int k = 0; k < P2; ++k) a += tmp[(size_t)k * per + 36 * 64];
  }
  return a;
}

template <int C>
__global__ void k_jku_finish_flat(const float* __restrict__ tmp, int P2, float* __restrict__ flat) {
  constexpr int H = JkU<C>::H;
  constexpr int per_dir = 4 * H * C + 4 * H * H + 8 * H, total = 2 * per_dir + 2 * H + 1;
  const int i = blockIdx.x * blockDim.x + threadIdx.x;
  if (i >= total) return;
  int d, row = 0, col = 0, att = -1;
  if (i < 2 * per_dir) {
    d = i / per_dir;
    int e = i - d * per_dir;
    if (e < 4 * H * C) { row = e / C; col = e % C; }
    else if ((e -= 4 * H * C) < 4 * H * H) { row = e / H; col = C + e % H; }
    else { e -= 4 * H * H; row = e % (4 * H); col = C + H; }
  } else {
    const int e = i - 2 * per_dir;
    if (e < 2 * H) { d = e / H; att = e % H; }
    else { d = 0; att = H; }
  }
  flat[i] = jku_gather<C>(tmp, P2, d, row, col, att);
}

template <int C>
__global__ void k_jku_finish_G(const float* __restrict__ tmp, int P2, float* __restrict__ G) {
  constexpr int H = JkU<C>::H, NG = 4 * H + 1, NI = C + 2 * H + 1;
  const int i = blockIdx.x * blockDim.x + threadIdx.x;
  if (i >= 2 * NG * NI) return;
  const int d = i / (NG * NI), e = i - d * NG * NI, row = e / NI, col = e - row * NI;
  float v = 0.f;
  if (row < 4 * H) {
    if (col <= C + H) v = jku_gather<C>(tmp, P2, d, row, col, -1);
  } else if (col > C + H) {
    v = jku_gather<C>(tmp, P2, d, 0, 0, col - (C + H + 1));
  } else if (col == C + H && d == 0) {
    v = jku_gather<C>(tmp, P2, 0, 0, 0, H);
  }
  G[i] = v;
}

template <int C>
static int launch_fwd(const float* xs, int n, int npad, const JkWeights& w, float* out, float* HS, float* CS, hipStream_t st) {
  constexpr size_t lds = sizeof(float) * JkU<C>::FWD_TOTAL;
  static bool attr_set[CGC_MAX_DEVICES] = {};
  cgc_allow_lds(reinterpret_cast<const void*>(&k_jku_fwd<C>), (int)lds, attr_set);
  int grid = ceil_div(n, 32);
  if (grid > 512) grid = 512;
  hipLaunchKernelGGL(k_jku_fwd<C>, dim3(grid), dim3(512), lds, st, xs, n, npad, w, out, HS, CS);
  CGC_RETURN_IF_LAUNCH_FAILED();
  return 0;
}

int jk_mfma_fwd(const float* xs, int n, int npad, int C, const JkWeights& w, float* out, float* HS, float* CS, hipStream_t st) {
  if ((reinterpret_cast<uintptr_t>(xs) & 15u) || (reinterpret_cast<uintptr_t>(out) & 15u)) return CGC_EINVAL;
  switch (C) {
    case 4: return launch_fwd<4>(xs, n, npad, w, out, HS, CS, st);
    case 8: return launch_fwd<8>(xs, n, npad, w, out, HS, CS, st);
    case 12: return launch_fwd<12>(xs, n, npad, w, out, HS, CS, st);
    case 16: return launch_fwd<16>(xs, n, npad, w, out, HS, CS, st);
    case 20: return launch_fwd<20>(xs, n, npad, w, out, HS, CS, st);
    default: return CGC_EINVAL;
  }
}

template <int C>
static int launch_bwd(const float* xs, const float* dout, int n, int npad, const JkWeights& w, const float* HS, const float* CS,
                      float* dxs, float* DGT, float* INT, hipStream_t st) {
  const size_t lds = sizeof(float) * (JkM<C>::TOTAL + JKB_TILES * 192) + sizeof(float4) * JKB_TILES * 2 * 3 * JkM<C>::XG * 64;
  static bool attr_set[CGC_MAX_DEVICES] = {};
  cgc_allow_lds(reinterpret_cast<const void*>(&k_jk_bwd_mfma<C>), (int)lds, attr_set);
  int grid = ceil_div(npad / 32, JKB_TILES);
  if (grid > 256) grid = 256;
  hipLaunchKernelGGL(k_jk_bwd_mfma<C>, dim3(grid), dim3(JKB_THREADS), lds, st, xs, dout, n, npad, w, HS, CS, dxs, DGT, INT, nullptr);
  CGC_RETURN_IF_LAUNCH_FAILED();
  return 0;
}

template <int C>
static int launch_bwd_params(const float* xs, const float* dout, int n, int npad, const JkWeights& w, const float* HS, const float* CS,
                             float* dxs, float* G, float* ws, hipStream_t st, float* flat) {
  constexpr size_t lds = sizeof(float) * JkU<C>::BWD_TOTAL;
  static bool attr_set[CGC_MAX_DEVICES] = {};
  cgc_allow_lds(reinterpret_cast<const void*>(&k_jku_bwd<C>), (int)lds, attr_set);
  int grid = ceil_div(n, 32);
  if (grid > 256) grid = 256;
  hipLaunchKernelGGL(k_jku_bwd<C>, dim3(grid), dim3(512), lds, st, xs, dout, n, npad, w, HS, CS, dxs, ws);
  CGC_RETURN_IF_LAUNCH_FAILED();
  constexpr int per = JkU<C>::PG_FLOATS, H = JkU<C>::H;
  const int P = grid, P2 = ceil_div(P, 16);
  float* tmp = ws + (size_t)P * per;
  hipLaunchKernelGGL(k_jk_pg_fold, dim3(ceil_div(per, 256), P2, 1), dim3(256), 0, st, ws, P, P2, per, tmp);
  if (flat != nullptr) {
    constexpr int total = 2 * (4 * H * C + 4 * H * H + 8 * H) + 2 * H + 1;
    hipLaunchKernelGGL(k_jku_finish_flat<C>, dim3(ceil_div(total, 128)), dim3(128), 0, st, tmp, P2, flat);
  } else {
    constexpr int total = 2 * (4 * H + 1) * (C + 2 * H + 1);
    hipLaunchKernelGGL(k_jku_finish_G<C>, dim3(ceil_div(total, 128)), dim3(128), 0, st, tmp, P2, G);
  }
  CGC_RETURN_IF_LAUNCH_FAILED();
  return 0;
}

int jk_mfma_bwd(const float* xs, const float* dout, int n, int npad, int C, const JkWeights& w, const float* HS, const float* CS,
                float* dxs, float* DGT, float* INT, hipStream_t st) {
  if ((reinterpret_cast<uintptr_t>(xs) & 15u) || (reinterpret_cast<uintptr_t>(dout) & 15u) || (reinterpret_cast<uintptr_t>(dxs) & 15u) ||
      npad % (32 * JKB_TILES) != 0)
    return CGC_EINVAL;
  switch (C) {
    case 4: return launch_bwd<4>(xs, dout, n, npad, w, HS, CS, dxs, DGT, INT, st);
    case 8: return launch_bwd<8>(xs, dout, n, npad, w, HS, CS, dxs, DGT, INT, st);
    case 12: return launch_bwd<12>(xs, dout, n, npad, w, HS, CS, dxs, DGT, INT, st);
    case 16: return launch_bwd<16>(xs, dout, n, npad, w, HS, CS, dxs, DGT, INT, st);
    case 20: return launch_bwd<20>(xs, dout, n, npad, w, HS, CS, dxs, DGT, INT, st);
    default: return CGC_EINVAL;
  }
}

int64_t jk_mfma_bwd_ws_floats(int C) {
  const int64_t per = (8 * 16 + 16 + 1) * 64;
  (void)C;
  return 2 * 512 * per + 2 * 32 * per;
}

int jk_mfma_bwd_flat(const float* xs, const float* dout, int n, int npad, int C, const JkWeights& w, const float* HS, const float* CS,
                     float* dxs, float* flat, float* ws, hipStream_t st) {
  if ((reinterpret_cast<uintptr_t>(xs) & 15u) || (reinterpret_cast<uintptr_t>(dout) & 15u) || (reinterpret_cast<uintptr_t>(dxs) & 15u))
    return CGC_EINVAL;
  switch (C) {
    case 4: return launch_bwd_params<4>(xs, dout, n, npad, w, HS, CS, dxs, nullptr, ws, st, flat);
    case 8: return launch_bwd_params<8>(xs, dout, n, npad, w, HS, CS, dxs, nullptr, ws, st, flat);
    case 12: return launch_bwd_params<12>(xs, dout, n, npad, w, HS, CS, dxs, nullptr, ws, st, flat);
    case 16: return launch_bwd_params<16>(xs, dout, n, npad, w, HS, CS, dxs, nullptr, ws, st, flat);
    case 20: return launch_bwd_params<20>(xs, dout, n, npad, w, HS, CS, dxs, nullptr, ws, st, flat);
    default: return CGC_EINVAL;
  }
}

int jk_mfma_bwd_params(const float* xs, const float* dout, int n, int npad, int C, const JkWeights& w, const float* HS,
                       const float* CS, float* dxs, float* G, float* ws, hipStream_t st) {
  if ((reinterpret_cast<uintptr_t>(xs) & 15u) || (reinterpret_cast<uintptr_t>(dout) & 15u) || (reinterpret_cast<uintptr_t>(dxs) & 15u))
    return CGC_EINVAL;
  switch (C) {
    case 4: return launch_bwd_params<4>(xs, dout, n, npad, w, HS, CS, dxs, G, ws, st, nullptr);
    case 8: return launch_bwd_params<8>(xs, dout, n, npad, w, HS, CS, dxs, G, ws, st, nullptr);
    case 12: return launch_bwd_params<12>(xs, dout, n, npad, w, HS, CS, dxs, G, ws, st, nullptr);
    case 16: return launch_bwd_params<16>(xs, dout, n, npad, w, HS, CS, dxs, G, ws, st, nullptr);
    case 20: return launch_bwd_params<20>(xs, dout, n, npad, w, HS, CS, dxs, G, ws, st, nullptr);
    default: return CGC_EINVAL;
  }
}
```

### cgc-net_amd/csrc/rowops.hip

```cpp
#include <type_traits>

#include "common.hpp"
#include "groups.hpp"

#define L2_EPS 1e-12f
#define RENORM_EPS 1e-15f
#define MAX_SLOTS 1024

template <int VEC, int MAXJ, int NQ>
__device__ __forceinline__ void col_reduce_store(float (&acc)[NQ][MAXJ][VEC], int F, int lpr, float* smem, float* slot) {
  const int lane = threadIdx.x & 63, wave = threadIdx.x >> 6;
#pragma unroll
  for (int q = 0; q < NQ; ++q)
#pragma unroll
    for (int j = 0; j < MAXJ; ++j)
#pragma unroll
      for (int v = 0; v < VEC; ++v)
        for (int o = 32; o >= lpr; o >>= 1) acc[q][j][v] += __shfl_xor(acc[q][j][v], o);
  if (wave > 0 && lane < lpr) {
#pragma unroll
    for (int q = 0; q < NQ; ++q)
#pragma unroll
      for (int j = 0; j < MAXJ; ++j)
#pragma unroll
        for (int v = 0; v < VEC; ++v) {
          const int c = (lane + lpr * j) * VEC + v;
          if (c < F) smem[((wave - 1) * NQ + q) * F + c] = acc[q][j][v];
        }
  }
  __syncthreads();
  if (wave == 0 && lane < lpr) {
#pragma unroll
    for (int q = 0; q < NQ; ++q)
#pragma unroll
      for (int j = 0; j < MAXJ; ++j)
#pragma unroll
        for (int v = 0; v < VEC; ++v) {
          const int c = (lane + lpr * j) * VEC + v;
          if (c < F) {
            float t = acc[q][j][v];
            for (int w = 0; w < 3; ++w) t += smem[(w * NQ + q) * F + c];
            slot[q * F + c] = t;
          }
        }
  }
}

template <int VEC, int MAXJ>
__device__ __forceinline__ void col_reduce_store_f64(double (&acc)[2][MAXJ][VEC], int F, int lpr, double* smem, double* slot) {
  const int lane = threadIdx.x & 63, wave = threadIdx.x >> 6;
#pragma unroll
  for (int q = 0; q < 2; ++q) {
#pragma unroll
    for (int j = 0; j < MAXJ; ++j)
#pragma unroll
      for (int v = 0; v < VEC; ++v)
        for (int o = 32; o >= lpr; o >>= 1) acc[q][j][v] += __shfl_xor(acc[q][j][v], o);
    if (q > 0) __syncthreads();
    if (wave > 0 && lane < lpr) {
#pragma unroll
      for (int j = 0; j < MAXJ; ++j)
#pragma unroll
        for (int v = 0; v < VEC; ++v) {
          const int c = (lane + lpr * j) * VEC + v;
          if (c < F) smem[(wave - 1) * F + c] = acc[q][j][v];
        }
    }
    __syncthreads();
    if (wave == 0 && lane < lpr) {
#pragma unroll
      for (int j = 0; j < MAXJ; ++j)
#pragma unroll
        for (int v = 0; v < VEC; ++v) {
          const int c = (lane + lpr * j) * VEC + v;
          if (c < F) {
            double t = acc[q][j][v];
            for (int w = 0; w < 3; ++w) t += smem[w * F + c];
            slot[q * F + c] = t;
          }
        }
    }
  }
}

#define RS_GROUPS 32
template <typename OUT, typename IN = float>
__global__ __launch_bounds__(32 * RS_GROUPS) void k_reduce_slots(const IN* __restrict__ ws, int slots, int width, OUT* __restrict__ out) {
  __shared__ double part[RS_GROUPS][32];
  const int cl = threadIdx.x & 31, grp = threadIdx.x >> 5;
  const int c = blockIdx.x * 32 + cl;
  double s = 0.0;
  if (c < width) {
    double a[4] = {0.0, 0.0, 0.0, 0.0};
    int k = grp;
    for (; k + 3 * RS_GROUPS < slots; k += 4 * RS_GROUPS) {
#pragma unroll
      for (int u = 0; u < 4; ++u) a[u] += (double)ws[(size_t)(k + RS_GROUPS * u) * width + c];
    }
    for (; k < slots; k += RS_GROUPS) a[0] += (double)ws[(size_t)k * width + c];
    s = (a[0] + a[1]) + (a[2] + a[3]);
  }
  part[grp][cl] = s;
  __syncthreads();
  if (grp == 0 && c < width) {
    double t[4] = {0.0, 0.0, 0.0, 0.0};
#pragma unroll
    for (int g = 0; g < RS_GROUPS; g += 4) { t[0] += part[g][cl]; t[1] += part[g + 1][cl]; t[2] += part[g + 2][cl]; t[3] += part[g + 3][cl]; }
    out[c] = (OUT)((t[0] + t[1]) + (t[2] + t[3]));
  }
}
#define REDUCE_SLOTS_GRID(width) dim3(ceil_div((width), 32))

__global__ __launch_bounds__(32 * RS_GROUPS) void k_reduce_slots_pair(const float* __restrict__ ws0, float* __restrict__ out0,
                                                                     const float* __restrict__ ws1, float* __restrict__ out1, int slots, int width) {
  const float* __restrict__ ws = blockIdx.y ? ws1 : ws0;
  float* __restrict__ out = blockIdx.y ? out1 : out0;
  __shared__ double part[RS_GROUPS][32];
  const int cl = threadIdx.x & 31, grp = threadIdx.x >> 5;
  const int c = blockIdx.x * 32 + cl;
  double s = 0.0;
  if (c < width) {
    double a[4] = {0.0, 0.0, 0.0, 0.0};
    int k = grp;
    for (; k + 3 * RS_GROUPS < slots; k += 4 * RS_GROUPS) {
#pragma unroll
      for (int u = 0; u < 4; ++u) a[u] += (double)ws[(size_t)(k + RS_GROUPS * u) * width + c];
    }
    for (; k < slots; k += RS_GROUPS) a[0] += (double)ws[(size_t)k * width + c];
    s = (a[0] + a[1]) + (a[2] + a[3]);
  }
  part[grp][cl] = s;
  __syncthreads();
  if (grp == 0 && c < width) {
    double t[4] = {0.0, 0.0, 0.0, 0.0};
#pragma unroll
    for (int g = 0; g < RS_GROUPS; g += 4) { t[0] += part[g][cl]; t[1] += part[g + 1][cl]; t[2] += part[g + 2][cl]; t[3] += part[g + 3][cl]; }
    out[c] = (float)((t[0] + t[1]) + (t[2] + t[3]));
  }
}
int launch_reduce_slots_f32_pair(const float* ws0, float* out0, const float* ws1, float* out1, int ng, int slots, int width, hipStream_t stream) {
  hipLaunchKernelGGL(k_reduce_slots_pair, dim3(ceil_div(width, 32), ng), dim3(32 * RS_GROUPS), 0, stream, ws0, out0, ws1, out1, slots, width);
  CGC_RETURN_IF_LAUNCH_FAILED();
  return 0;
}

int launch_reduce_slots_f32(const float* ws, int slots, int width, float* out, hipStream_t stream) {
  hipLaunchKernelGGL(k_reduce_slots<float>, REDUCE_SLOTS_GRID(width), dim3(32 * RS_GROUPS), 0, stream, ws, slots, width, out);
  CGC_RETURN_IF_LAUNCH_FAILED();
  return 0;
}

struct ColCfg {
  int vec, maxj, lpr, blocks;
  bool ok;
};
static ColCfg col_cfg(int n, int F, bool vec_ok) {
  ColCfg c;
  c.vec = vec_ok ? 4 : 1;
  c.ok = true;
  int chunks = F / c.vec;
  if (chunks <= 64) {
    c.maxj = 1;
    c.lpr = pick_lpr(chunks);
  } else {
    c.lpr = 64;
    int need = ceil_div(chunks, 64);
    if (c.vec == 4 && need > 8) {
      c.vec = 1;
      need = ceil_div(F, 64);
    }
    c.ok = need <= 32;
    c.maxj = need <= 2 ? 2 : need <= 4 ? 4 : (need == 5 && c.vec == 4) ? 5 : need <= 8 ? 8 : need <= 16 ? 16 : 32;
  }
  c.blocks = row_blocks(n, c.lpr, MAX_SLOTS);
  return c;
}

#define DISPATCH_COL(KERNEL, cfg, smem_bytes, stream, ...)                                                   \
  do {                                                                                                       \
    dim3 g__((cfg).blocks), b__(CGC_BLOCK);                                                                  \
    if ((cfg).vec == 4) {                                                                                    \
      switch ((cfg).maxj) {                                                                                  \
        case 1: hipLaunchKernelGGL((KERNEL<4, 1>), g__, b__, smem_bytes, stream, __VA_ARGS__); break;        \
        case 2: hipLaunchKernelGGL((KERNEL<4, 2>), g__, b__, smem_bytes, stream, __VA_ARGS__); break;        \
        case 4: hipLaunchKernelGGL((KERNEL<4, 4>), g__, b__, smem_bytes, stream, __VA_ARGS__); break;        \
        case 5: hipLaunchKernelGGL((KERNEL<4, 5>), g__, b__, smem_bytes, stream, __VA_ARGS__); break;        \
        default: hipLaunchKernelGGL((KERNEL<4, 8>), g__, b__, smem_bytes, stream, __VA_ARGS__); break;       \
      }                                                                                                      \
    } else {                                                                                                 \
      switch ((cfg).maxj) {                                                                                  \
        case 1: hipLaunchKernelGGL((KERNEL<1, 1>), g__, b__, smem_bytes, stream, __VA_ARGS__); break;        \
        case 2: hipLaunchKernelGGL((KERNEL<1, 2>), g__, b__, smem_bytes, stream, __VA_ARGS__); break;        \
        case 4: hipLaunchKernelGGL((KERNEL<1, 4>), g__, b__, smem_bytes, stream, __VA_ARGS__); break;        \
        case 8: hipLaunchKernelGGL((KERNEL<1, 8>), g__, b__, smem_bytes, stream, __VA_ARGS__); break;        \
        case 16: hipLaunchKernelGGL((KERNEL<1, 16>), g__, b__, smem_bytes, stream, __VA_ARGS__); break;      \
        default: hipLaunchKernelGGL((KERNEL<1, 32>), g__, b__, smem_bytes, stream, __VA_ARGS__); break;      \
      }                                                                                                      \
    }                                                                                                        \
  } while (0)

#define DISPATCH_COL_Y(KERNEL, cfg, ny, smem_bytes, stream, ...)                                                   \
  do {                                                                                                       \
    dim3 g__((cfg).blocks, (ny)), b__(CGC_BLOCK);                                                                    \
    if ((cfg).vec == 4) {                                                                                    \
      switch ((cfg).maxj) {                                                                                  \
        case 1: hipLaunchKernelGGL((KERNEL<4, 1>), g__, b__, smem_bytes, stream, __VA_ARGS__); break;        \
        case 2: hipLaunchKernelGGL((KERNEL<4, 2>), g__, b__, smem_bytes, stream, __VA_ARGS__); break;        \
        case 4: hipLaunchKernelGGL((KERNEL<4, 4>), g__, b__, smem_bytes, stream, __VA_ARGS__); break;        \
        case 5: hipLaunchKernelGGL((KERNEL<4, 5>), g__, b__, smem_bytes, stream, __VA_ARGS__); break;        \
        default: hipLaunchKernelGGL((KERNEL<4, 8>), g__, b__, smem_bytes, stream, __VA_ARGS__); break;       \
      }                                                                                                      \
    } else {                                                                                                 \
      switch ((cfg).maxj) {                                                                                  \
        case 1: hipLaunchKernelGGL((KERNEL<1, 1>), g__, b__, smem_bytes, stream, __VA_ARGS__); break;        \
        case 2: hipLaunchKernelGGL((KERNEL<1, 2>), g__, b__, smem_bytes, stream, __VA_ARGS__); break;        \
        case 4: hipLaunchKernelGGL((KERNEL<1, 4>), g__, b__, smem_bytes, stream, __VA_ARGS__); break;        \
        case 8: hipLaunchKernelGGL((KERNEL<1, 8>), g__, b__, smem_bytes, stream, __VA_ARGS__); break;        \
        case 16: hipLaunchKernelGGL((KERNEL<1, 16>), g__, b__, smem_bytes, stream, __VA_ARGS__); break;      \
        default: hipLaunchKernelGGL((KERNEL<1, 32>), g__, b__, smem_bytes, stream, __VA_ARGS__); break;      \
      }                                                                                                      \
    }                                                                                                        \
// ... 407 lines not shown
    const int normalize = HOT ? 1 : normalize_rt;
    for (int base = rg.gwave * rg.rpw; base < n; base += rg.nwaves * rg.rpw) {
      const int row = min(base + rg.sub, n - 1);
      const bool valid = base + rg.sub < n;
      Vec<VEC> g[MAXJ], x[MAXJ];
      float dot = 0.f;
  #pragma unroll
      for (int j = 0; j < MAXJ; ++j) {
        const int c = min((rg.sl + lpr * j) * VEC, F - VEC);
        load_wide<VEC, MAXJ>(g[j], dy + (size_t)row * ldy + c);
        load_wide<VEC, MAXJ>(x[j], hn + (size_t)row * F + c);
      }
  #pragma unroll
      for (int j = 0; j < MAXJ; ++j) {
        const int c = (rg.sl + lpr * j) * VEC;
        if (valid && c < F) {
          Vec<VEC> pa, pb, pc, pm, pi;
          if (!REGC && mode != 0) {
            pa.load(lc + c);
            if (mode == 2) { pb.load(lc + F + c); pc.load(lc + 2 * F + c); pm.load(lc + 3 * F + c); pi.load(lc + 4 * F + c); }
          }
  #pragma unroll
          for (int v = 0; v < VEC; ++v) {
            const float xv = x[j].v[v];
            float a_, b_ = 0.f, c_ = 0.f, m_ = 0.f, i_ = 0.f;
            if (REGC) {
              a_ = ca[REGC ? j : 0][REGC ? v : 0]; b_ = cb[REGC ? j : 0][REGC ? v : 0]; c_ = cc[REGC ? j : 0][REGC ? v : 0];
              m_ = mu[REGC ? j : 0][REGC ? v : 0]; i_ = is[REGC ? j : 0][REGC ? v : 0];
            } else if (mode != 0) {
              a_ = pa.v[v];
              if (mode == 2) { b_ = pb.v[v]; c_ = pc.v[v]; m_ = pm.v[v]; i_ = pi.v[v]; }
            } else {
              a_ = 1.f;
            }
            float go = a_ * g[j].v[v];
            if (mode == 2) go = go - b_ - (act_fwd(xv, ACT) - m_) * i_ * c_;
            go *= act_bwd(xv, ACT);
            g[j].v[v] = go;
            dot += xv * go;
          }
        } else {
  #pragma unroll
          for (int v = 0; v < VEC; ++v) g[j].v[v] = x[j].v[v] = 0.f;
        }
      }
      if (normalize) dot = group_sum(dot, lpr);
      if (!valid) continue;
      const float r = normalize ? rinv[row] : 1.f;
      const bool clamped = normalize && !(r < 1.f / L2_EPS);
  #pragma unroll
      for (int j = 0; j < MAXJ; ++j) {
        const int c = (rg.sl + lpr * j) * VEC;
        if (c < F) {
          Vec<VEC> o;
  #pragma unroll
          for (int v = 0; v < VEC; ++v) {
            const float gv = g[j].v[v];
            o.v[v] = !normalize ? gv : (clamped ? gv * (1.f / L2_EPS) : r * (gv - x[j].v[v] * dot));
            csum[0][j][v] += o.v[v];
          }
          o.store(dh + (size_t)row * F + c);
        }
      }
    }
  };
  if (mode == 2 && normalize) {
    switch (act) {
      case CGC_ACT_RELU: rows(std::integral_constant<int, CGC_ACT_RELU>(), std::true_type()); break;
      case CGC_ACT_ELU: rows(std::integral_constant<int, CGC_ACT_ELU>(), std::true_type()); break;
      case CGC_ACT_LEAKYRELU: rows(std::integral_constant<int, CGC_ACT_LEAKYRELU>(), std::true_type()); break;
      default: rows(std::integral_constant<int, CGC_ACT_IDENTITY>(), std::true_type()); break;
    }
  } else {
    switch (act) {
      case CGC_ACT_RELU: rows(std::integral_constant<int, CGC_ACT_RELU>(), std::false_type()); break;
      case CGC_ACT_ELU: rows(std::integral_constant<int, CGC_ACT_ELU>(), std::false_type()); break;
      case CGC_ACT_LEAKYRELU: rows(std::integral_constant<int, CGC_ACT_LEAKYRELU>(), std::false_type()); break;
      default: rows(std::integral_constant<int, CGC_ACT_IDENTITY>(), std::false_type()); break;
    }
  }
  if (ws != nullptr) col_reduce_store<VEC, MAXJ, 1>(csum, F, lpr, smem, ws + (size_t)blockIdx.x * F);
}

extern "C" int cgc_bn_act_l2_bwd(const float* dy, int ldy, const float* hn, const float* rinv, int n, int F, int act,
                                 int normalize, int mode, const float* mean, const float* istd, const float* gamma,
                                 const float* sums, double count, float* dh, float* dh_colsum, float* ws, cgc_stream_t stream) {
  if (F <= 0) return 0;
  if (n <= 0) {
    if (dh_colsum) (void)hipMemsetAsync(dh_colsum, 0, sizeof(float) * F, as_stream(stream));
    return 0;
  }
  if (dh_colsum != nullptr && ws == nullptr) return CGC_EINVAL;
  const bool vec = (F % 4 == 0) && (ldy % 4 == 0) && aligned16(dy) && aligned16(hn) && aligned16(dh);
  ColCfg cfg = col_cfg(n, F, vec);
  if (!cfg.ok) return CGC_EINVAL;
  if (dh_colsum == nullptr) cfg.blocks = row_blocks(n, cfg.lpr);
  const float inv_count = (float)(1.0 / count);
  const size_t smem = sizeof(float) * (3 + 5) * F;
  DISPATCH_COL(k_bn_act_l2_bwd, cfg, smem, as_stream(stream), dy, ldy, hn, rinv, n, F, cfg.lpr, act, normalize, mode, mean, istd,
               gamma, sums, inv_count, dh, dh_colsum ? ws : (float*)nullptr);
  CGC_RETURN_IF_LAUNCH_FAILED();
  if (dh_colsum) {
    hipLaunchKernelGGL(k_reduce_slots<float>, REDUCE_SLOTS_GRID(F), dim3(32 * RS_GROUPS), 0, as_stream(stream), ws, cfg.blocks, F, dh_colsum);
    CGC_RETURN_IF_LAUNCH_FAILED();
  }
  return 0;
}

template <int VEC, int MAXJ>
__global__ __launch_bounds__(256) void k_colsum(const float* __restrict__ x, int ld, int n, int F, int lpr, float* __restrict__ ws) {
  extern __shared__ __attribute__((aligned(16))) float smem[];
  const RowGroup rg(lpr);
  float acc[1][MAXJ][VEC];
#pragma unroll
  for (int j = 0; j < MAXJ; ++j)
#pragma unroll
    for (int v = 0; v < VEC; ++v) acc[0][j][v] = 0.f;
  for (int base = rg.gwave * rg.rpw; base < n; base += rg.nwaves * rg.rpw) {
    const int row = base + rg.sub;
    if (row < n) {
#pragma unroll
      for (int j = 0; j < MAXJ; ++j) {
        const int c = (rg.sl + lpr * j) * VEC;
        if (c < F) {
          Vec<VEC> d;
          d.load(x + (size_t)row * ld + c);
#pragma unroll
          for (int v = 0; v < VEC; ++v) acc[0][j][v] += d.v[v];
        }
      }
    }
  }
  col_reduce_store<VEC, MAXJ, 1>(acc, F, lpr, smem, ws + (size_t)blockIdx.x * F);
}

extern "C" int cgc_colsum(const float* x, int ld, int n, int F, float* out, float* ws, cgc_stream_t stream) {
  if (F <= 0) return 0;
  if (n <= 0) {
    (void)hipMemsetAsync(out, 0, sizeof(float) * F, as_stream(stream));
    return 0;
  }
  const bool vec_ok = (F % 4 == 0) && (ld % 4 == 0) && aligned16(x);
  ColCfg cfg = col_cfg(n, F, vec_ok);
  if (!cfg.ok) return CGC_EINVAL;
  const size_t smem = sizeof(float) * 3 * F;
  DISPATCH_COL(k_colsum, cfg, smem, as_stream(stream), x, ld, n, F, cfg.lpr, ws);
  CGC_RETURN_IF_LAUNCH_FAILED();
  hipLaunchKernelGGL(k_reduce_slots<float>, REDUCE_SLOTS_GRID(F), dim3(32 * RS_GROUPS), 0, as_stream(stream), ws, cfg.blocks, F, out);
  CGC_RETURN_IF_LAUNCH_FAILED();
  return 0;
}

template <int VEC>
__global__ __launch_bounds__(256) void k_softmax_fwd(const float* __restrict__ x, int n, int C, int ld, int lpr, float* __restrict__ out) {
  const RowGroup rg(lpr);
  for (int base = rg.gwave * rg.rpw; base < n; base += rg.nwaves * rg.rpw) {
    const int row = base + rg.sub;
    const bool valid = row < n;
    const float* xr = x + (size_t)row * ld;
    float m = -INFINITY;
    if (valid)
      for (int c = rg.sl * VEC; c < C; c += lpr * VEC) {
        Vec<VEC> t;
        t.load(xr + c);
#pragma unroll
        for (int v = 0; v < VEC; ++v) m = fmaxf(m, t.v[v]);
      }
    m = group_max(m, lpr);
    float s = 0.f;
    if (valid)
      for (int c = rg.sl * VEC; c < C; c += lpr * VEC) {
        Vec<VEC> t;
        t.load(xr + c);
#pragma unroll
        for (int v = 0; v < VEC; ++v) s += expf(t.v[v] - m);
      }
    s = group_sum(s, lpr);
    if (!valid) continue;
    const float inv = 1.f / s;
    for (int c = rg.sl * VEC; c < C; c += lpr * VEC) {
      Vec<VEC> t;
      t.load(xr + c);
#pragma unroll
      for (int v = 0; v < VEC; ++v) t.v[v] = expf(t.v[v] - m) * inv;
      t.store(out + (size_t)row * ld + c);
    }
// ... 37 lines not shown
    const float inv = 1.f / s;
#pragma unroll
    for (int j = 0; j < MAXJ; ++j) {
      const int c = (rg.sl + lpr * j) * VEC;
      if (c < C) {
#pragma unroll
        for (int v = 0; v < VEC; ++v) t[j].v[v] *= inv;
        t[j].store(out + (size_t)row * ld + c);
      }
    }
  }
}

template <int VEC, int MAXJ>
__global__ __launch_bounds__(256) void k_softmax_bwd(const float* __restrict__ S, const float* __restrict__ dS, int n, int C,
                                                     int ld, int lpr, float* __restrict__ dx, float* __restrict__ ws) {
  extern __shared__ __attribute__((aligned(16))) float smem[];
  const RowGroup rg(lpr);
  float csum[1][MAXJ][VEC];
#pragma unroll
  for (int j = 0; j < MAXJ; ++j)
#pragma unroll
    for (int v = 0; v < VEC; ++v) csum[0][j][v] = 0.f;
  for (int base = rg.gwave * rg.rpw; base < n; base += rg.nwaves * rg.rpw) {
    const int row = min(base + rg.sub, n - 1);
    const bool valid = base + rg.sub < n;
    Vec<VEC> s[MAXJ], d[MAXJ];
    float dot = 0.f;
#pragma unroll
    for (int j = 0; j < MAXJ; ++j) {
      const int c = min((rg.sl + lpr * j) * VEC, C - VEC);
      load_wide<VEC, MAXJ>(s[j], S + (size_t)row * ld + c);
      load_wide<VEC, MAXJ>(d[j], dS + (size_t)row * ld + c);
    }
#pragma unroll
    for (int j = 0; j < MAXJ; ++j) {
      const bool ok = valid && (rg.sl + lpr * j) * VEC < C;
#pragma unroll
      for (int v = 0; v < VEC; ++v) {
        s[j].v[v] = ok ? s[j].v[v] : 0.f;
        d[j].v[v] = ok ? d[j].v[v] : 0.f;
        dot += s[j].v[v] * d[j].v[v];
      }
    }
    dot = group_sum(dot, lpr);
    if (!valid) continue;
#pragma unroll
    for (int j = 0; j < MAXJ; ++j) {
      const int c = (rg.sl + lpr * j) * VEC;
      if (c < C) {
#pragma unroll
        for (int v = 0; v < VEC; ++v) {
          d[j].v[v] = s[j].v[v] * (d[j].v[v] - dot);
          csum[0][j][v] += d[j].v[v];
        }
        d[j].store(dx + (size_t)row * ld + c);
      }
    }
  }
  if (ws != nullptr) col_reduce_store<VEC, MAXJ, 1>(csum, C, lpr, smem, ws + (size_t)blockIdx.x * C);
}

extern "C" int cgc_softmax_fwd(const float* x, int n, int C, int ld, float* out, cgc_stream_t stream) {
  if (n <= 0 || C <= 0) return 0;
  if (ld < C) return CGC_EINVAL;
  const bool vec = (C % 4 == 0) && (ld % 4 == 0) && aligned16(x) && aligned16(out);
  ColCfg cfg = col_cfg(n, C, vec);
  if (cfg.ok && cfg.maxj <= 8) {
    cfg.blocks = row_blocks(n, cfg.lpr);
    DISPATCH_COL(k_softmax_fwd_reg, cfg, 0, as_stream(stream), x, n, C, ld, cfg.lpr, out);
    CGC_RETURN_IF_LAUNCH_FAILED();
    return 0;
  }
  const int lpr = pick_lpr(vec ? C / 4 : C);
  dim3 grid(row_blocks(n, lpr)), block(CGC_BLOCK);
  if (vec)
    hipLaunchKernelGGL(k_softmax_fwd<4>, grid, block, 0, as_stream(stream), x, n, C, ld, lpr, out);
  else
    hipLaunchKernelGGL(k_softmax_fwd<1>, grid, block, 0, as_stream(stream), x, n, C, ld, lpr, out);
  CGC_RETURN_IF_LAUNCH_FAILED();
  return 0;
}

extern "C" int cgc_softmax_bwd(const float* S, const float* dS, int n, int C, int ld, float* dx, float* dx_colsum, float* ws,
                               cgc_stream_t stream) {
  if (C <= 0) return 0;
  if (ld < C) return CGC_EINVAL;
  if (n <= 0) {
    if (dx_colsum) (void)hipMemsetAsync(dx_colsum, 0, sizeof(float) * C, as_stream(stream));
    return 0;
  }
  if (dx_colsum != nullptr && ws == nullptr) return CGC_EINVAL;
  const bool vec = (C % 4 == 0) && (ld % 4 == 0) && aligned16(S) && aligned16(dS) && aligned16(dx);
  ColCfg cfg = col_cfg(n, C, vec);
  if (!cfg.ok) return CGC_EINVAL;
  if (dx_colsum == nullptr) cfg.blocks = row_blocks(n, cfg.lpr);
  const size_t smem = dx_colsum ? sizeof(float) * 3 * C : 0;
  DISPATCH_COL(k_softmax_bwd, cfg, smem, as_stream(stream), S, dS, n, C, ld, cfg.lpr, dx, dx_colsum ? ws : (float*)nullptr);
  CGC_RETURN_IF_LAUNCH_FAILED();
  if (dx_colsum) {
    hipLaunchKernelGGL(k_reduce_slots<float>, REDUCE_SLOTS_GRID(C), dim3(32 * RS_GROUPS), 0, as_stream(stream), ws, cfg.blocks, C, dx_colsum);
    CGC_RETURN_IF_LAUNCH_FAILED();
  }
  return 0;
}

#define SEGMAX_WAVES 16
__global__ __launch_bounds__(64 * SEGMAX_WAVES) void k_segment_max_fwd(const float* __restrict__ x, const int* __restrict__ gptr,
                                                                       int D, int nmax, float* __restrict__ out,
                                                                       int* __restrict__ arg) {
  __shared__ float bv[SEGMAX_WAVES][64];
  __shared__ int bi[SEGMAX_WAVES][64];
  const int b = blockIdx.x;
  const int lane = threadIdx.x & 63, wave = threadIdx.x >> 6;
  int dp = 64;
  if (D <= 32) dp = D <= 2 ? 2 : D <= 4 ? 4 : D <= 8 ? 8 : D <= 16 ? 16 : 32;
  const int rpw = 64 / dp, sub = lane / dp, dl = lane - sub * dp;
  const int d = blockIdx.y * 64 + dl;
  const int lo = gptr[b], hi = gptr[b + 1];
  float best = -INFINITY;
  int idx = -1;
  if (d < D) {
    const int stride = SEGMAX_WAVES * rpw;
    int r = lo + wave * rpw + sub;
    for (; r + 3 * stride < hi; r += 4 * stride) {
      float v[4];
#pragma unroll
      for (int u = 0; u < 4; ++u) v[u] = x[(size_t)(r + u * stride) * D + d];
#pragma unroll
      for (int u = 0; u < 4; ++u)
        if (v[u] > best) { best = v[u]; idx = r + u * stride; }
    }
    for (; r < hi; r += stride) {
      const float v = x[(size_t)r * D + d];
      if (v > best) { best = v; idx = r; }
    }
  }
  bv[wave][lane] = best;
  bi[wave][lane] = idx;
  __syncthreads();
  if (wave == 0 && sub == 0 && d < D) {
    for (int w = 0; w < SEGMAX_WAVES; ++w)
      for (int s2 = (w == 0 ? 1 : 0); s2 < rpw; ++s2) {
        const float v = bv[w][s2 * dp + dl];
        const int i = bi[w][s2 * dp + dl];
        if (i >= 0 && (v > best || (v == best && i < idx) || idx < 0)) { best = v; idx = i; }
      }
    if (idx < 0) { best = 0.f; }
    else if (hi - lo < nmax && best < 0.f) { best = 0.f; idx = -1; }
    out[(size_t)b * D + d] = best;
    arg[(size_t)b * D + d] = idx;
  }
}

__global__ void k_segment_max_bwd(const float* __restrict__ dout, const int* __restrict__ arg, int total, int D, float* __restrict__ dx) {
  const int i = blockIdx.x * blockDim.x + threadIdx.x;
  if (i >= total) return;
  const int a = arg[i];
  if (a >= 0) dx[(size_t)a * D + (i % D)] = dout[i];
}

extern "C" int cgc_segment_max_fwd(const float* x, const int* gptr, int B, int D, int nmax, float* out, int* arg, cgc_stream_t stream) {
  if (B <= 0 || D <= 0) return 0;
  hipLaunchKernelGGL(k_segment_max_fwd, dim3(B, ceil_div(D, 64)), dim3(64 * SEGMAX_WAVES), 0, as_stream(stream), x, gptr, D, nmax, out, arg);
  CGC_RETURN_IF_LAUNCH_FAILED();
  return 0;
}

__global__ void k_segment_max_bwd_full(const float* __restrict__ dout, const int* __restrict__ arg, const int* __restrict__ gptr, int D,
                                       float* __restrict__ dx) {
  const int b = blockIdx.y;
  const int g0 = gptr[b], cnt = (gptr[b + 1] - g0) * D;
  for (int i = blockIdx.x * blockDim.x + threadIdx.x; i < cnt; i += gridDim.x * blockDim.x) {
    const int r = i / D, d = i - r * D;
    dx[(size_t)g0 * D + i] = (arg[b * D + d] == g0 + r) ? dout[b * D + d] : 0.f;
  }
}

extern "C" int cgc_segment_max_bwd_full(const float* dout, const int* arg, const int* gptr, int B, int D, int nmax, float* dx,
                                        cgc_stream_t stream) {
  if (B <= 0 || D <= 0 || nmax <= 0) return 0;
  if (B > 65535) return CGC_EINVAL;
  int bx = ceil_div(nmax * D, 256 * 4);
  if (bx < 1) bx = 1;
// ... 444 lines not shown
```

### cgc-net_amd/csrc/sagenarrow.hip

```cpp
#include "common.hpp"
#include "groups.hpp"

#define L2_EPS 1e-12f
typedef float floatx16 __attribute__((ext_vector_type(16)));

template <int CTRL>
__device__ __forceinline__ float dpp_step(float v) {
  return v + __builtin_bit_cast(float, __builtin_amdgcn_mov_dpp(__builtin_bit_cast(int, v), CTRL, 0xF, 0xF, true));
}
__device__ __forceinline__ float half_sum(float v) {
  v = dpp_step<0xB1>(v);
  v = dpp_step<0x4E>(v);
  v = dpp_step<0x141>(v);
  v = dpp_step<0x140>(v);
  return v + __shfl_xor(v, 16);
}

#define SN_LDT 33

template <int FS, int ACT>
__global__ __launch_bounds__(256) void k_sage_narrow_bwd(const SnBwdPtrs p0, const SnBwdPtrs p1, int ldy, int n, int F, int ,
                                                         int normalize, int mode, float inv_count, int lda, int fin, int ldd, int tiles) {
  const bool second = blockIdx.y != 0;
  const float* __restrict__ dy = second ? p1.dy : p0.dy;
// ... 49 lines not shown
      float go = ca * g;
      if (mode == 2) go = go - cb - (act_fwd(x, ACT) - mu) * is * cc;
      go *= act_bwd(x, ACT);
      if (!(ok && fok)) go = 0.f;
      float o = go;
      if (normalize) {
        const float dot = half_sum(x * go);
        const float r_ = rinv[rc];
        const float r = ok ? r_ : 1.f;
        const bool clamped = !(r < 1.f / L2_EPS);
        o = clamped ? go * (1.f / L2_EPS) : r * (go - x * dot);
      }
      dh[s] = o;
      db += o;
    }
#pragma unroll
    for (int s = 0; s < 16; ++s) dw = __builtin_amdgcn_mfma_f32_32x32x2f32(ag[s], dh[s], dw, 0, 0, 0);
    if (dagg != nullptr) {
#pragma unroll
      for (int s = 0; s < 16; ++s) st[(2 * s + half) * SN_LDT + f] = dh[s];
      __builtin_amdgcn_wave_barrier();
      floatx16 da;
#pragma unroll
      for (int r = 0; r < 16; ++r) da[r] = 0.f;
#pragma unroll
      for (int t = 0; t < FS; ++t) da = __builtin_amdgcn_mfma_f32_32x32x2f32(st[f * SN_LDT + 2 * t + half], wb[t], da, 0, 0, 0);
      __builtin_amdgcn_wave_barrier();
      if (f < fin) {
        if (row0 + 32 <= n) {
#pragma unroll
          for (int r = 0; r < 16; ++r) dagg[(size_t)(row0 + (r & 3) + 8 * (r >> 2) + 4 * half) * ldd + f] = da[r];
        } else {
#pragma unroll
          for (int r = 0; r < 16; ++r) {
            const int row = row0 + (r & 3) + 8 * (r >> 2) + 4 * half;
            if (row < n) dagg[(size_t)row * ldd + f] = da[r];
          }
        }
      }
    }
  }
  __syncthreads();
  float* __restrict__ xch = &strip[0][0];
  static_assert(32 * SN_LDT <= 17 * 64, "transposition strip exceeds the per-wave LDS");
#pragma unroll
  for (int r = 0; r < 16; ++r) xch[(wave * 17 + r) * 64 + lane] = dw[r];
  xch[(wave * 17 + 16) * 64 + lane] = db;
  __syncthreads();
  if (wave == 0) {
    float* __restrict__ slot = ws + (size_t)blockIdx.x * (fin * F + F);
#pragma unroll
    for (int r = 0; r < 16; ++r) {
      const float v = (xch[(0 * 17 + r) * 64 + lane] + xch[(1 * 17 + r) * 64 + lane]) + (xch[(2 * 17 + r) * 64 + lane] + xch[(3 * 17 + r) * 64 + lane]);
      const int k = (r & 3) + 8 * (r >> 2) + 4 * half;
      if (fok && k < fin) slot[k * F + f] = v;
    }
    float d = (xch[(0 * 17 + 16) * 64 + lane] + xch[(1 * 17 + 16) * 64 + lane]) + (xch[(2 * 17 + 16) * 64 + lane] + xch[(3 * 17 + 16) * 64 + lane]);
    d += __shfl_xor(d, 32);
    if (fok && half == 0) slot[fin * F + f] = d;
  }
}

int launch_reduce_slots_f32(const float* ws, int slots, int width, float* out, hipStream_t stream);

static int sn_grid(int n) {
  const int tiles = ceil_div(n, 32);
  int g = ceil_div(tiles, 4);
  return g < 1024 ? g : 1024;
}

extern "C" int64_t cgc_sage_narrow_ws_floats(int n, int fin, int F) { return (int64_t)sn_grid(n > 0 ? n : 1) * (fin * F + F); }

int sage_narrow_bwd_groups(const SnBwdPtrs* g, float* const* dwdb, int ng, int ldy, int n, int F, int act, int normalize, int mode, double count,
                           int lda, int fin, int ldd, hipStream_t st) {
  if (F <= 0 || fin <= 0) return 0;
  if (F > 32 || fin > 32 || ng < 1 || ng > 2) return CGC_EINVAL;
  for (int i = 0; i < ng; ++i)
    if (g[i].ws == nullptr || dwdb[i] == nullptr || (g[i].dagg != nullptr && ldd < fin)) return CGC_EINVAL;
  const int width = fin * F + F;
  if (n <= 0) {
    for (int i = 0; i < ng; ++i) (void)hipMemsetAsync(dwdb[i], 0, sizeof(float) * width, st);
    return 0;
  }
  const int tiles = ceil_div(n, 32), grid = sn_grid(n);
  const float inv_count = (float)(1.0 / count);
  const int fs = (F + 1) / 2;
  const SnBwdPtrs& g1 = g[ng - 1];
#define SN_LAUNCH(FS_, ACT_)                                                                                                       \
  hipLaunchKernelGGL((k_sage_narrow_bwd<FS_, ACT_>), dim3(grid, ng), dim3(256), 0, st, g[0], g1, ldy, n, F, act, normalize, mode, inv_count, \
                     lda, fin, ldd, tiles)
#define SN_ACT(FS_)                                                                                        \
  switch (act) {                                                                                           \
    case CGC_ACT_RELU: SN_LAUNCH(FS_, CGC_ACT_RELU); break;                                                \
    case CGC_ACT_ELU: SN_LAUNCH(FS_, CGC_ACT_ELU); break;                                                  \
    case CGC_ACT_LEAKYRELU: SN_LAUNCH(FS_, CGC_ACT_LEAKYRELU); break;                                      \
    default: SN_LAUNCH(FS_, CGC_ACT_IDENTITY); break;                                                      \
  }
  if (fs <= 8) { SN_ACT(8); } else if (fs <= 10) { SN_ACT(10); } else { SN_ACT(16); }
#undef SN_ACT
#undef SN_LAUNCH
  CGC_RETURN_IF_LAUNCH_FAILED();
  return launch_reduce_slots_f32_pair(g[0].ws, dwdb[0], g1.ws, dwdb[ng - 1], ng, grid, width, st);
}

extern "C" int cgc_sage_narrow_bwd(const float* dy, int ldy, const float* hn, const float* rinv, int n, int F, int act, int normalize,
                                   int mode, const float* mean, const float* istd, const float* gamma, const float* sums, double count,
                                   const float* agg, int lda, int fin, const float* W, float* dagg, int ldd, float* dwdb, float* ws,
                                   cgc_stream_t stream_) {
  const SnBwdPtrs g{dy, hn, rinv, mean, istd, gamma, sums, agg, W, dagg, ws};
  float* const out[1] = {dwdb};
  return sage_narrow_bwd_groups(&g, out, 1, ldy, n, F, act, normalize, mode, count, lda, fin, ldd, as_stream(stream_));
}

template <int KS, int ACT>
__global__ __launch_bounds__(256) void k_sage_narrow_fwd(const SnFwdPtrs p0, const SnFwdPtrs p1, int lda, int n, int K, int F, int normalize,
                                                         int , int tiles) {
  const bool second = blockIdx.y != 0;
  const float* __restrict__ agg = second ? p1.agg : p0.agg;
  const float* __restrict__ W = second ? p1.W : p0.W;
  const float* __restrict__ bias = second ? p1.bias : p0.bias;
  float* __restrict__ hn = second ? p1.hn : p0.hn;
  float* __restrict__ rinv_out = second ? p1.rinv : p0.rinv;
  float* __restrict__ ws = second ? p1.ws : p0.ws;
  __shared__ double xch[4][2][32];
  const int lane = threadIdx.x & 63, wave = threadIdx.x >> 6;
  const int f = lane & 31, half = lane >> 5;
  const bool fok = f < F;
  float bw[KS];
#pragma unroll
  for (int s = 0; s < KS; ++s) {
    const int k = 2 * s + half;
    bw[s] = (fok && k < K) ? W[(size_t)k * F + f] : 0.f;
  }
  const float bia = (fok && bias != nullptr) ? bias[f] : 0.f;
  double s1 = 0.0, s2 = 0.0;
  for (int tile = blockIdx.x * 4 + wave; tile < tiles; tile += gridDim.x * 4) {
    const int row0 = tile * 32;
    const float* __restrict__ a = agg + (size_t)min(row0 + f, n - 1) * lda;
    float av[KS];
#pragma unroll
    for (int s = 0; s < KS; ++s) {
      const int k = 2 * s + half;
      const float ld = a[k < K ? k : 0];
      av[s] = k < K ? ld : 0.f;
    }
    floatx16 acc;
#pragma unroll
    for (int r = 0; r < 16; ++r) acc[r] = bia;
#pragma unroll
    for (int s = 0; s < KS; ++s) acc = __builtin_amdgcn_mfma_f32_32x32x2f32(av[s], bw[s], acc, 0, 0, 0);
    float vv[16], rr[16];
#pragma unroll
    for (int r = 0; r < 16; ++r) {
      float v = fok ? acc[r] : 0.f;
      float rin = 1.f;
      if (normalize) {
        const float q = half_sum(v * v);
        rin = 1.f / fmaxf(sqrtf(q), L2_EPS);
        v *= rin;
      }
      vv[r] = v;
      rr[r] = rin;
    }
    if (row0 + 32 <= n) {
      if (fok) {
#pragma unroll
        for (int r = 0; r < 16; ++r) {
          const int row = row0 + (r & 3) + 8 * (r >> 2) + 4 * half;
          const double o = (double)act_fwd(vv[r], ACT);
          s1 += o;
          s2 = fma(o, o, s2);
          hn[(size_t)row * F + f] = vv[r];
        }
      }
      if (f == 0) {
#pragma unroll
        for (int r = 0; r < 16; ++r) rinv_out[row0 + (r & 3) + 8 * (r >> 2) + 4 * half] = rr[r];
      }
    } else {
#pragma unroll
      for (int r = 0; r < 16; ++r) {
        const int row = row0 + (r & 3) + 8 * (r >> 2) + 4 * half;
        if (row < n) {
          if (fok) {
            const double o = (double)act_fwd(vv[r], ACT);
// ... 72 lines not shown
```

### cgc-net_amd/csrc/spmm.hip

```cpp
#include "common.hpp"

constexpr int GATHER_U = 9;

template <int VEC>
__global__ __launch_bounds__(256) void k_spmm(const int* __restrict__ rowptr, const int* __restrict__ col, const int* __restrict__ perm,
                                              const float* __restrict__ val, const float* __restrict__ pre,
                                              const float* __restrict__ post, const float* __restrict__ x, float* __restrict__ out,
                                              int n, int W, int ld, int lpr, int n_ctiles, int rows_per_block, int blocks_per_ct,
                                              int n_chunks, int nt_store, const int* __restrict__ gptr) {
  const int nb = gridDim.x, b = blockIdx.x;
  const int vb = (nb % 8 == 0) ? (b % 8) * (nb / 8) + b / 8 : b;
  const int per_chunk = blocks_per_ct * n_ctiles;
  const int chunk = vb / per_chunk;
  if (chunk >= n_chunks) return;
  const int rem = vb - chunk * per_chunk;
  const int ct = rem / blocks_per_ct, rb = rem - ct * blocks_per_ct;
  int row0, row_end;
  if (gptr != nullptr) {
    const int g0 = gptr[chunk], g1 = gptr[chunk + 1];
    row0 = g0 + rb * rows_per_block;
    if (row0 >= g1) return;
    row_end = min(row0 + rows_per_block, g1);
  } else {
    row0 = (chunk * blocks_per_ct + rb) * rows_per_block;
    row_end = min(row0 + rows_per_block, n);
  }

  const int lane = threadIdx.x & 63, wave = threadIdx.x >> 6;
  const int sl = lane & (lpr - 1), sub = lane / lpr, rpw = 64 / lpr;
  const int c0 = (ct * lpr + sl) * VEC;
  const bool colok = c0 < W;

  for (int rbase = row0 + wave * rpw; rbase < row_end; rbase += 4 * rpw) {
    const int r = rbase + sub;
    const bool valid = r < row_end;
    int s = 0, e = 0;
    if (valid) { s = rowptr[r]; e = rowptr[r + 1]; }
    float acc[VEC];
#pragma unroll
    for (int v = 0; v < VEC; ++v) acc[v] = 0.f;
    for (int k0 = s; k0 < e; k0 += lpr) {
      const int kk = k0 + sl;
      int myc = 0;
      float myw = 0.f;
      if (kk < e) {
        myc = col[kk];
        float w = val != nullptr ? val[perm != nullptr ? perm[kk] : kk] : 1.f;
        if (pre != nullptr) w *= pre[myc];
        myw = w;
      }
      const int cnt = min(lpr, e - k0);
      for (int t = 0; t < cnt; t += GATHER_U) {
        Vec<VEC> xv[GATHER_U];
        float ww[GATHER_U];
#pragma unroll
        for (int u = 0; u < GATHER_U; ++u) {
          const int tt = t + u;
          const int cc = __shfl(myc, tt & (lpr - 1), lpr);
          ww[u] = __shfl(myw, tt & (lpr - 1), lpr);
          if (tt < cnt && colok) {
            xv[u].load(x + (size_t)cc * ld + c0);
          } else {
            ww[u] = 0.f;
#pragma unroll
            for (int v = 0; v < VEC; ++v) xv[u].v[v] = 0.f;
          }
        }
#pragma unroll
        for (int u = 0; u < GATHER_U; ++u)
#pragma unroll
          for (int v = 0; v < VEC; ++v) acc[v] = fmaf(ww[u], xv[u].v[v], acc[v]);
      }
    }
    if (valid && colok) {
      const float ps = post != nullptr ? post[r] : 1.f;
      float* op = out + (size_t)r * ld + c0;
      if (nt_store && VEC == 4) {
        typedef float f4v __attribute__((ext_vector_type(4)));
        f4v o4 = {acc[0] * ps, acc[VEC > 1 ? 1 : 0] * ps, acc[VEC > 2 ? 2 : 0] * ps, acc[VEC > 3 ? 3 : 0] * ps};
        __builtin_nontemporal_store(o4, reinterpret_cast<f4v*>(op));
      } else {
        Vec<VEC> o;
#pragma unroll
        for (int v = 0; v < VEC; ++v) o.v[v] = acc[v] * ps;
        o.store(op);
      }
    }
  }
}

typedef float wide_f4 __attribute__((ext_vector_type(4)));

template <int CNT, bool VAL, bool PERM, bool PRE>
__device__ __forceinline__ void wide_batch(const int* __restrict__ col, const int* __restrict__ perm,
                                           const float* __restrict__ val, const float* __restrict__ pre,
                                           const float* __restrict__ xl, int W, int k, wide_f4& acc) {
  int cc[CNT];
  wide_f4 xv[CNT];
  float ww[CNT];
#pragma unroll
  for (int u = 0; u < CNT; ++u) cc[u] = col[k + u];
#pragma unroll
  for (int u = 0; u < CNT; ++u) xv[u] = *reinterpret_cast<const wide_f4*>(xl + (size_t)cc[u] * W);
#pragma unroll
  for (int u = 0; u < CNT; ++u) ww[u] = 1.f;
  if (VAL) {
    int pi[CNT];
#pragma unroll
    for (int u = 0; u < CNT; ++u) pi[u] = PERM ? perm[k + u] : k + u;
#pragma unroll
    for (int u = 0; u < CNT; ++u) ww[u] = val[pi[u]];
  }
  if (PRE) {
    float pr[CNT];
#pragma unroll
    for (int u = 0; u < CNT; ++u) pr[u] = pre[cc[u]];
#pragma unroll
    for (int u = 0; u < CNT; ++u) ww[u] *= pr[u];
  }
#pragma unroll
  for (int u = 0; u < CNT; ++u) acc += ww[u] * xv[u];
}

template <int N, bool VAL, bool PERM, bool PRE>
__device__ __forceinline__ void wide_tail(int cnt, const int* __restrict__ col, const int* __restrict__ perm,
                                          const float* __restrict__ val, const float* __restrict__ pre,
                                          const float* __restrict__ xl, int W, int k, wide_f4& acc) {
  if constexpr (N > 0) {
    if (cnt == N) wide_batch<N, VAL, PERM, PRE>(col, perm, val, pre, xl, W, k, acc);
    else wide_tail<N - 1, VAL, PERM, PRE>(cnt, col, perm, val, pre, xl, W, k, acc);
  }
}

template <int U, bool VAL, bool PERM, bool PRE>
__global__ __launch_bounds__(256) void k_spmm_wide(const int* __restrict__ rowptr, const int* __restrict__ col,
                                                   const int* __restrict__ perm, const float* __restrict__ val,
                                                   const float* __restrict__ pre, const float* __restrict__ post,
                                                   const float* __restrict__ x, float* __restrict__ out, int n, int W, int ld,
                                                   int n_ctiles, int run, int blocks_per_ct, int n_chunks,
                                                   const int* __restrict__ gptr, int order, const int* __restrict__ gorder) {
  typedef float f4v __attribute__((ext_vector_type(4)));
  const int nb = gridDim.x, b = blockIdx.x;
  const int vb = (nb % 8 == 0) ? (b % 8) * (nb / 8) + b / 8 : b;
  const int per_chunk = blocks_per_ct * n_ctiles;
  const int chunk = vb / per_chunk;
  if (chunk >= n_chunks) return;
  const int rem = vb - chunk * per_chunk;
  const int ct = rem / blocks_per_ct, rb = rem - ct * blocks_per_ct;
  const int rows_per_block = 4 * run;
  int row0, row_end;
  if (gptr != nullptr) {
    int gi = chunk;
    if (gorder != nullptr) {
      gi = gorder[chunk];
    } else if (order == 1) {
      const int per_x = n_chunks >> 3;
      gi = ((n_chunks & 7) == 0 && (nb & 7) == 0) ? (per_x - 1 - chunk % per_x) * 8 + chunk / per_x : n_chunks - 1 - chunk;
    } else if (order == 2) {
      const int per_x = n_chunks >> 3;
      gi = ((n_chunks & 7) == 0 && (nb & 7) == 0) ? (chunk / per_x) * per_x + (per_x - 1 - chunk % per_x) : n_chunks - 1 - chunk;
    }
    const int g0 = gptr[gi], g1 = gptr[gi + 1];
    row0 = g0 + rb * rows_per_block;
    row_end = min(row0 + rows_per_block, g1);
  } else {
    row0 = (chunk * blocks_per_ct + rb) * rows_per_block;
    row_end = min(row0 + rows_per_block, n);
  }
  const int lane = threadIdx.x & 63;
  const int wave = __builtin_amdgcn_readfirstlane(threadIdx.x >> 6);
  const int c0 = (ct * 64 + lane) * 4;
  if (c0 >= W) return;
  const float* __restrict__ xl = x + c0;
  int r = row0 + wave * run;
  const int r_end = min(r + run, row_end);
  if (r >= r_end) return;
  int s = rowptr[r];
  for (; r < r_end; ++r) {
    const int e = rowptr[r + 1];
    f4v acc = {0.f, 0.f, 0.f, 0.f};
    int k = s;
    for (; k + U <= e; k += U) wide_batch<U, VAL, PERM, PRE>(col, perm, val, pre, xl, ld, k, acc);
    wide_tail<U - 1, VAL, PERM, PRE>(e - k, col, perm, val, pre, xl, ld, k, acc);
    if (post != nullptr) acc *= post[r];
    __builtin_nontemporal_store(acc, reinterpret_cast<f4v*>(out + (size_t)r * ld + c0));
    s = e;
  }
}

constexpr int SPMM_PASSES = 2, SPMM_CHUNK = 2048, SPMM_RUN = 2;

static int launch_gather(const int* rowptr, const int* col, const int* perm, const float* val, const float* pre, const float* post,
                         const float* x, float* out, int n, int width, int ld, const int* gptr, int B, int nmax, int order,
                         hipStream_t stream, const int* gorder = nullptr) {
  const bool vec = (width % 4 == 0) && (ld % 4 == 0) && aligned16(x) && aligned16(out);
  const int chunks = vec ? width / 4 : width;
  const int lpr = pick_lpr(chunks);
  const int n_ctiles = ceil_div(chunks, lpr);
  const int rpw = 64 / lpr;
  const int rows_per_block = 4 * rpw * SPMM_PASSES;
  int blocks_per_ct, n_chunks;
  if (gptr != nullptr && n_ctiles > 1) {
    blocks_per_ct = ceil_div(nmax, rows_per_block);
    n_chunks = B;
  } else {
    gptr = nullptr;
    const int chunk_rows = ceil_div(SPMM_CHUNK, rows_per_block) * rows_per_block;
    blocks_per_ct = chunk_rows / rows_per_block;
    n_chunks = ceil_div(n, chunk_rows);
  }
  if (vec && lpr == 64) {
    const int rpb = 4 * SPMM_RUN;
    if (gptr != nullptr) {
      blocks_per_ct = ceil_div(nmax, rpb);
    } else {
      const int chunk_rows = ceil_div(SPMM_CHUNK, rpb) * rpb;
      blocks_per_ct = chunk_rows / rpb;
      n_chunks = ceil_div(n, chunk_rows);
    }
    const int nbw = ceil_div(n_chunks * blocks_per_ct * n_ctiles, 8) * 8;
#define WIDE_LAUNCH(V, P, Q)                                                                                              \
  hipLaunchKernelGGL((k_spmm_wide<GATHER_U, V, P, Q>), dim3(nbw), dim3(CGC_BLOCK), 0, stream, rowptr, col, perm, val, pre, \
                     post, x, out, n, width, ld, n_ctiles, SPMM_RUN, blocks_per_ct, n_chunks, gptr, order, gorder)
    const bool hv = val != nullptr, hp = hv && perm != nullptr, hq = pre != nullptr;
    if (!hv && !hq) WIDE_LAUNCH(false, false, false);
    else if (!hv) WIDE_LAUNCH(false, false, true);
    else if (!hp && !hq) WIDE_LAUNCH(true, false, false);
    else if (!hp) WIDE_LAUNCH(true, false, true);
    else if (!hq) WIDE_LAUNCH(true, true, false);
    else WIDE_LAUNCH(true, true, true);
#undef WIDE_LAUNCH
    CGC_RETURN_IF_LAUNCH_FAILED();
    return 0;
  }
  int nb = n_chunks * blocks_per_ct * n_ctiles;
  nb = ceil_div(nb, 8) * 8;
  dim3 grid(nb), block(CGC_BLOCK);
  const int nt = n_ctiles > 1 ? 1 : 0;
  if (vec)
    hipLaunchKernelGGL(k_spmm<4>, grid, block, 0, stream, rowptr, col, perm, val, pre, post, x, out, n, width, ld, lpr,
                       n_ctiles, rows_per_block, blocks_per_ct, n_chunks, nt, gptr);
  else
    hipLaunchKernelGGL(k_spmm<1>, grid, block, 0, stream, rowptr, col, perm, val, pre, post, x, out, n, width, ld, lpr,
                       n_ctiles, rows_per_block, blocks_per_ct, n_chunks, nt, gptr);
  CGC_RETURN_IF_LAUNCH_FAILED();
  return 0;
}

extern "C" int cgc_spmm(const int* rowptr, const int* col, const int* perm, const float* val, const float* pre, const float* post,
                        const float* x, float* out, int n, int width, cgc_stream_t stream) {
  if (n <= 0 || width <= 0) return 0;
  return launch_gather(rowptr, col, perm, val, pre, post, x, out, n, width, width, nullptr, 0, 0, 0, as_stream(stream));
}

extern "C" int cgc_spmm_graphs(const int* rowptr, const int* col, const int* perm, const float* val, const float* pre,
                               const float* post, const float* x, float* out, int n, int width, int ld, const int* gptr, int B,
                               int nmax, int visit, const int* gorder, cgc_stream_t stream) {
  if (n <= 0 || width <= 0) return 0;
  if (ld < width) return CGC_EINVAL;
  const int trec = width > 64 ? cgc_timing_begin(CGC_TAG_SPMM_WIDE, n, width, ld, val != nullptr, 0, 0, 0, as_stream(stream)) : -1;
  const int rc = launch_gather(rowptr, col, perm, val, pre, post, x, out, n, width, ld, gptr, B, nmax, visit & 3, as_stream(stream), gorder);
  cgc_timing_end(trec, as_stream(stream));
  return rc;
}
```

Baseline: 2854 graphs/s.

## Defer backward weight-gradient reductions into one batched launch and fuse spmm with concat-add

Weight-gradient partial sums from several backward kernels (narrow SAGE, bn/act, split-K TN gemm, JK LSTM, softmax colsum) are no longer reduced right away. Their partials are kept in arena space pinned by a new floor mechanism, and all of them are reduced together in a single table-driven kernel at the end of level backward. The transpose spmm in pool levels now adds the concatenated addends inside its epilogue, replacing a separate cat2 pass. The goal is fewer small kernel launches and fewer memory passes. The cost is higher scratch memory residency and a fixed cap on pending entries.

New measurement: 2864 graphs/s, median of 6. No clear change (+0.4%).

```diff
diff --git a/cgc-net_amd/csrc/deferred.hip b/cgc-net_amd/csrc/deferred.hip
--- /dev/null
+++ b/cgc-net_amd/csrc/deferred.hip
@@ -0,0 +1,70 @@
+#include "reduce_order.hpp"
+
+__global__ __launch_bounds__(1024) void k_deferred_reduce(const DeferredTable t, int count) {
+  __shared__ double sh[2048];
+  DeferredEntry s = t.e[0];
+#pragma unroll
+  for (int k = 1; k < DEF_MAX_ENTRIES; ++k)
+    if (k < count && (int)blockIdx.x >= t.e[k].first_block) s = t.e[k];
+  const int chunk = (int)blockIdx.x - s.first_block;
+  const int tid = threadIdx.x;
+  if (s.kind == DEF_SLOTS) {
+    double(*part)[32] = reinterpret_cast<double(*)[32]>(sh);
+    const int cl = tid & 31, grp = tid >> 5;
+    const int c = chunk * 32 + cl;
+    part[grp][cl] = c < s.numel ? slots_group_sum(s.src, s.parts, s.stride, c, grp) : 0.0;
+    __syncthreads();
+    if (grp == 0 && c < s.numel) s.dst[c] = (float)slots_fold(part, cl);
+  } else if (s.kind == DEF_MANY_PARTS) {
+    float(*part)[32] = reinterpret_cast<float(*)[32]>(sh) + (tid >> 8) * 8;
+    const int cl = tid & 31, grp = (tid >> 5) & 7;
+    const int c = (chunk * 4 + (tid >> 8)) * 32 + cl;
+    part[grp][cl] = c < s.numel ? many_parts_group_sum(s.src, s.parts, s.numel, c, grp) : 0.f;
+    __syncthreads();
+    if (grp == 0 && c < s.numel) s.dst[(size_t)(c / s.width) * s.ldo + c % s.width] = many_parts_fold(part, cl);
+  } else if (s.kind == DEF_BATCH_SUM) {
+    const int i = chunk * 1024 + tid;
+    if (i < s.numel) s.dst[(size_t)(i / s.width) * s.ldo + i % s.width] = batch_sum_plain(s.src, s.parts, s.numel, i);
+  } else {
+    float(*fold)[64] = reinterpret_cast<float(*)[64]>(sh);
+    const int o = tid & 63, k = tid >> 6;
+    const int i = chunk * 64 + o;
+    const int P2 = (s.parts + JKU_FOLD - 1) / JKU_FOLD;
+    const int e = i < s.numel ? jku_flat_element(s.width, i) : 0;
+    if (k < P2) fold[k][o] = jku_fold16(s.src, s.parts, k, s.stride, e);
+    __syncthreads();
+    if (k == 0 && i < s.numel) {
+      float a = 0.f;
+      for (int q = 0; q < P2; ++q) a += fold[q][o];
+      s.dst[i] = a;
+    }
+  }
+}
+
+int launch_deferred(DeferredEntry* entries, int count, hipStream_t stream) {
+  for (int lo = 0; lo < count; lo += DEF_MAX_ENTRIES) {
+    const int m = count - lo < DEF_MAX_ENTRIES ? count - lo : DEF_MAX_ENTRIES;
+    DeferredTable t;
+    memset(&t, 0, sizeof(t));
+    int blocks = 0;
+    for (int k = 0; k < m; ++k) {
+      DeferredEntry& e = entries[lo + k];
+      if (e.src == nullptr || e.dst == nullptr || e.parts < 1 || e.numel < 1 || e.stride < 1) return CGC_EINVAL;
+      if (e.kind == DEF_JK) {
+        if (e.parts > 16 * JKU_FOLD || e.numel != jku_flat_total(e.width)) return CGC_EINVAL;
+      } else if (e.kind == DEF_SLOTS) {
+        if (e.stride < e.numel) return CGC_EINVAL;
+      } else if (e.kind == DEF_MANY_PARTS || e.kind == DEF_BATCH_SUM) {
+        if (e.width < 1 || e.ldo < e.width || e.numel % e.width != 0 || e.stride != e.numel) return CGC_EINVAL;
+      } else {
+        return CGC_EINVAL;
+      }
+      e.first_block = blocks;
+      blocks += ceil_div(e.numel, deferred_chunk(e.kind));
+      t.e[k] = e;
+    }
+    hipLaunchKernelGGL(k_deferred_reduce, dim3((unsigned)blocks), dim3(1024), 0, stream, t, m);
+    CGC_RETURN_IF_LAUNCH_FAILED();
+  }
+  return 0;
+}
diff --git a/cgc-net_amd/csrc/exec.hip b/cgc-net_amd/csrc/exec.hip
--- a/cgc-net_amd/csrc/exec.hip
+++ b/cgc-net_amd/csrc/exec.hip
@@ -4,6 +4,8 @@
 
 #include "common.hpp"
 #include "groups.hpp"
+#include "jk.hpp"
+#include "reduce_order.hpp"
 
 struct CatArgs {
   const float* src[4];
@@ -70,13 +72,12 @@
   return 0;
 }
 
-int reduce_batch_sum_rows(const float* ws, float* out, int parts, int rows, int width, int ldo, float beta, hipStream_t stream);
-
 namespace {
 
 struct Arena {
   float* base;
   size_t off = 0, high = 0;
+  size_t floor = 0;
   explicit Arena(float* b) : base(b) {}
   float* f(size_t n) {
     off = (off + 63) & ~(size_t)63;
@@ -87,7 +88,17 @@
   }
   int* i(size_t n) { return reinterpret_cast<int*>(f(n)); }
   size_t mark() const { return off; }
-  void release(size_t m) { off = m; }
+  void release(size_t m) { off = m > floor ? m : floor; }
+  float* keep(size_t n) {
+    float* p = f(n);
+    floor = off;
+    return p;
+  }
+};
+
+struct Pending {
+  DeferredEntry e[24];
+  int n = 0;
 };
 
 struct Ctx {
@@ -97,6 +108,7 @@
   float* gws;
   int64_t gws_floats;
   int gemm_mode = CGC_GEMM_EXACT;
+  Pending* pending = nullptr;
 };
 
 static int fail_at(int rc, const char* what, int line) {
@@ -158,18 +170,33 @@
   return best;
 }
 
-int gemm_tn_rows(const Ctx& c, const float* A, int lda, int Fa, const float* B, int ldb, int Fb, int n, float* out, int ldo = 0) {
+int defer(const Ctx& c, int kind, const float* src, int parts, int stride, int numel, int width, int ldo, float* dst) {
+  if (c.dry) return 0;
+  Pending& p = *c.pending;
+  if (p.n >= (int)(sizeof(p.e) / sizeof(p.e[0]))) return CGC_EINVAL;
+  p.e[p.n++] = DeferredEntry{src, dst, kind, parts, stride, numel, width, ldo, 0, 0};
+  return 0;
+}
+
+int tn_rows_parts(int Fa, int Fb, int n, int* chunk) {
+  const int parts = split_parts(Fa, Fb, n);
+  if (parts == 1) return 1;
+  *chunk = up(ceil_div(n, parts), 32);
+  return ceil_div(n, *chunk);
+}
+size_t tn_rows_ws_floats(int Fa, int Fb, int n) {
+  int chunk = 0;
+  return split_parts(Fa, Fb, n) == 1 ? 0 : (size_t)tn_rows_parts(Fa, Fb, n, &chunk) * Fa * Fb;
+}
+int gemm_tn_rows(const Ctx& c, const float* A, int lda, int Fa, const float* B, int ldb, int Fb, int n, float* out, int ldo = 0,
+                 float* ws = nullptr) {
   if (ldo <= 0) ldo = Fb;
-  int parts = split_parts(Fa, Fb, n);
-  if (parts == 1) return gemm(c, 1, 0, Fa, Fb, n, A, lda, B, ldb, 0.f, out, ldo);
-  const int chunk = up(ceil_div(n, parts), 32);
-  parts = ceil_div(n, chunk);
-  const size_t m = c.scratch->mark();
-  float* ws = c.scratch->f((size_t)parts * Fa * Fb);
+  if (split_parts(Fa, Fb, n) == 1) return gemm(c, 1, 0, Fa, Fb, n, A, lda, B, ldb, 0.f, out, ldo);
+  int chunk = 0;
+  const int parts = tn_rows_parts(Fa, Fb, n, &chunk);
+  if (ws == nullptr) ws = c.scratch->keep((size_t)parts * Fa * Fb);
   TRY(gemm(c, 1, 0, Fa, Fb, n, A, lda, B, ldb, 0.f, ws, Fb, nullptr, parts, 0, 0, (int64_t)Fa * Fb, nullptr, 3, chunk));
-  CALL(reduce_batch_sum_rows(ws, out, parts, Fa, Fb, ldo, 0.f, as_stream(c.s)));
-  c.scratch->release(m);
-  return 0;
+  return defer(c, combine_many_parts(parts, (int64_t)Fa * Fb) ? DEF_MANY_PARTS : DEF_BATCH_SUM, ws, parts, Fa * Fb, Fa * Fb, Fb, ldo, out);
 }
 
 struct T3 {
@@ -275,25 +302,30 @@
 
 int layer_bwd(const Ctx& c, const cgc_level_desc& d, const LayerP& p, const LayerS& s, const float* agg, int lda, int n, int fin, int F,
               const float* dy, int ldy, float* dagg, int ldd, float* dwdb, float* sums) {
-  const size_t m = c.scratch->mark();
   const int mode = d.has_bn ? 2 : 0;
   const size_t slot_floats = (size_t)(cgc_stats_blocks(n, F) > 1 ? cgc_stats_blocks(n, F) : 1) * 2 * F;
+  float* db = d.has_bias ? dwdb + (size_t)fin * F : nullptr;
+  const bool narrow = F <= 32 && fin <= 32;
+  const int width = fin * F + F;
+  float* ws_par = narrow ? c.scratch->keep((size_t)cgc_sage_narrow_ws_floats(n, fin, F)) : db ? c.scratch->keep(slot_floats) : nullptr;
+  float* ws_tn = (!narrow && tn_rows_ws_floats(fin, F, n) > 0) ? c.scratch->keep(tn_rows_ws_floats(fin, F, n)) : nullptr;
+  const size_t m = c.scratch->mark();
   if (d.has_bn) {
     float* ws = c.scratch->f(slot_floats);
     CALL(cgc_bn_bwd_reduce(dy, ldy, s.hn, n, F, d.act, s.mean, s.istd, sums, ws, c.s));
   }
-  float* db = d.has_bias ? dwdb + (size_t)fin * F : nullptr;
-  if (F <= 32 && fin <= 32) {
-    float* ws = c.scratch->f((size_t)cgc_sage_narrow_ws_floats(n, fin, F));
-    CALL(cgc_sage_narrow_bwd(dy, ldy, s.hn, s.rinv, n, F, d.act, 1, mode, s.mean, s.istd, p.gamma, d.has_bn ? sums : nullptr, d.count, agg,
-                             lda, fin, p.W, dagg, ldd, dwdb, ws, c.s));
+  int slots = 0;
+  if (narrow) {
+    const SnBwdPtrs g{dy, s.hn, s.rinv, s.mean, s.istd, p.gamma, d.has_bn ? sums : nullptr, agg, p.W, dagg, ws_par};
+    CALL(sage_narrow_bwd_partials(&g, 1, ldy, n, F, d.act, 1, mode, d.count, lda, fin, ldd, &slots, as_stream(c.s)));
+    TRY(defer(c, DEF_SLOTS, ws_par, slots, width, width, width, width, dwdb));
   } else {
     float* dh = c.scratch->f((size_t)n * F);
-    float* ws = db ? c.scratch->f(slot_floats) : nullptr;
-    CALL(cgc_bn_act_l2_bwd(dy, ldy, s.hn, s.rinv, n, F, d.act, 1, mode, s.mean, s.istd, p.gamma, d.has_bn ? sums : nullptr, d.count, dh, db, ws,
-                           c.s));
+    CALL(bn_act_l2_bwd_partials(dy, ldy, s.hn, s.rinv, n, F, d.act, 1, mode, s.mean, s.istd, p.gamma, d.has_bn ? sums : nullptr, d.count, dh,
+                                db != nullptr, ws_par, &slots, as_stream(c.s)));
+    if (db) TRY(defer(c, DEF_SLOTS, ws_par, slots, F, F, F, F, db));
     if (dagg) TRY(gemm(c, 0, 1, n, fin, F, dh, F, p.W, F, 0.f, dagg, ldd));
-    TRY(gemm_tn_rows(c, agg, lda, fin, dh, F, F, n, dwdb));
+    TRY(gemm_tn_rows(c, agg, lda, fin, dh, F, F, n, dwdb, 0, ws_tn));
   }
   c.scratch->release(m);
   return 0;
@@ -324,9 +356,12 @@
 
 int layer_bwd_pair(const Ctx& c, const cgc_level_desc& d, const LayerP* p, const LayerS* s, const float* const* agg, int lda, int n, int fin, int F,
                    const float* const* dy, int ldy, float* const* dagg, int ldd, float* const* dwdb, float* const* sums) {
+  const int mode = d.has_bn ? 2 : 0;
+  const int width = fin * F + F;
+  const size_t slot_floats = (size_t)(cgc_stats_blocks(n, F) > 1 ? cgc_stats_blocks(n, F) : 1) * 2 * F;
+  float* ws_par[2];
+  for (int i = 0; i < 2; ++i) ws_par[i] = c.scratch->keep((size_t)cgc_sage_narrow_ws_floats(n, fin, F));
   const size_t m = c.scratch->mark();
-  const int mode = d.has_bn ? 2 : 0;
-  const size_t slot_floats = (size_t)(cgc_stats_blocks(n, F) > 1 ? cgc_stats_blocks(n, F) : 1) * 2 * F;
   if (d.has_bn) {
     BnRedPtrs r[2];
     for (int i = 0; i < 2; ++i) r[i] = BnRedPtrs{dy[i], s[i].hn, s[i].mean, s[i].istd, c.scratch->f(slot_floats)};
@@ -335,8 +370,10 @@
   SnBwdPtrs g[2];
   for (int i = 0; i < 2; ++i)
     g[i] = SnBwdPtrs{dy[i], s[i].hn, s[i].rinv, s[i].mean, s[i].istd, p[i].gamma, d.has_bn ? sums[i] : nullptr, agg[i], p[i].W, dagg[i],
-                     c.scratch->f((size_t)cgc_sage_narrow_ws_floats(n, fin, F))};
-  CALL(sage_narrow_bwd_groups(g, dwdb, 2, ldy, n, F, d.act, 1, mode, d.count, lda, fin, ldd, as_stream(c.s)));
+                     ws_par[i]};
+  int slots = 0;
+  CALL(sage_narrow_bwd_partials(g, 2, ldy, n, F, d.act, 1, mode, d.count, lda, fin, ldd, &slots, as_stream(c.s)));
+  for (int i = 0; i < 2; ++i) TRY(defer(c, DEF_SLOTS, ws_par[i], slots, width, width, width, width, dwdb[i]));
   c.scratch->release(m);
   return 0;
 }
@@ -587,10 +624,10 @@
   float* d_cat = d_embed;
   if (d.jk) {
     d_cat = sc.f((size_t)n * D3);
-    const size_t m = sc.mark();
-    float* ws = sc.f((size_t)cgc_jk_bwd_ws_floats(H));
-    CALL(cgc_jk_lstm_bwd_flat(L.cat_e, d_embed, n, L.npad_jk, H, jk->lstm, jk->w_att, jk->b_att, L.HS, L.CS, d_cat, grads + L.gl.jk, ws, c.s));
-    sc.release(m);
+    float* ws = sc.keep((size_t)jk_mfma_bwd_partials_floats(n));
+    int parts = 0;
+    CALL(jk_lstm_bwd_partials(L.cat_e, d_embed, n, L.npad_jk, H, jk->lstm, jk->w_att, jk->b_att, L.HS, L.CS, d_cat, ws, &parts, as_stream(c.s)));
+    TRY(defer(c, DEF_JK, ws, parts, JKU_PG_FLOATS, jku_flat_total(H), H, jku_flat_total(H), grads + L.gl.jk));
   }
   float* dagg[2];
   const int ldg = L.ldp;
@@ -600,9 +637,14 @@
   float* dpair = nullptr;
   for (int k = 1; k >= 0; --k) {
     dpair = sc.f((size_t)n * wp);
-    TRY(aggregate_t(c, L, g, gptr, dagg[k], ldg, wp, dpair));
-    if (L.pool) TRY(cat2(c, dpair, wp, n, d_cat + k * H, D3, H, dx12 + k * AH, 2 * AH, AH, 1));
-    else TRY(add1(c, dpair, wp, n, d_cat + k * H, D3, H));
+    if (!L.dense && L.pool && (c.dry || spmm_takes_addends(dagg[k], dpair, wp, wp))) {
+      CALL(spmm_graphs_add(g->t_rowptr, g->t_col, g->t_val, g->inv_d, nullptr, dagg[k], dpair, n, wp, wp, gptr, B, d.nmax, d_cat + k * H, D3, H,
+                           dx12 + k * AH, 2 * AH, as_stream(c.s)));
+    } else {
+      TRY(aggregate_t(c, L, g, gptr, dagg[k], ldg, wp, dpair));
+      if (L.pool) TRY(cat2(c, dpair, wp, n, d_cat + k * H, D3, H, dx12 + k * AH, 2 * AH, AH, 1));
+      else TRY(add1(c, dpair, wp, n, d_cat + k * H, D3, H));
+    }
     const bool first = k == 0;
     const bool need_in = !first || L.dense;
     const float* ain = first ? L.agg0 : L.aggk[k - 1];
@@ -693,10 +735,10 @@
     if (L.reg) CALL(cgc_diffpool_reg_entropy_bwd(L.S, n, C, L.ldC, coef, ds, L.ldC, c.s));
     float* dz = sc.f((size_t)n * L.ldC);
     {
-      const size_t m = sc.mark();
-      float* ws = sc.f((size_t)(cgc_stats_blocks(n, C) > 1 ? cgc_stats_blocks(n, C) : 1) * 2 * C);
-      CALL(cgc_softmax_bwd(L.S, ds, n, C, L.ldC, dz, grads + L.gl.lin_b, ws, c.s));
-      sc.release(m);
+      float* ws = sc.keep((size_t)(cgc_stats_blocks(n, C) > 1 ? cgc_stats_blocks(n, C) : 1) * 2 * C);
+      int slots = 0;
+      CALL(softmax_bwd_partials(L.S, ds, n, C, L.ldC, dz, 1, ws, &slots, as_stream(c.s)));
+      TRY(defer(c, DEF_SLOTS, ws, slots, C, C, C, C, grads + L.gl.lin_b));
     }
     dx12 = sc.f((size_t)n * 2 * AH);
     float* dy3 = sc.f((size_t)n * L.ldC);
@@ -791,7 +833,7 @@
   if (!cgc_level_supported(d) || saved == nullptr || scratch == nullptr) return CGC_EINVAL;
   if (!aligned16(saved) || !aligned16(scratch)) return CGC_EINVAL;
   if ((d->flags & 8) && reg_out == nullptr) return CGC_EINVAL;
-  return run_level(d, saved, scratch, stream, [&](const Ctx& c, Level& L) {
+  return run_level(d, saved, scratch, stream, [&](Ctx& c, Level& L) {
     const int rc = level_fwd(c, L, emb, pool, jk, g, gptr, x_in, A_in, readout, x_out, A_out, reg_out);
     if (assign_out != nullptr) *assign_out = L.S;
     if (assign_ld != nullptr) *assign_ld = L.ldC;
@@ -806,7 +848,11 @@
   if (!cgc_level_supported(d) || saved == nullptr || scratch == nullptr || grads == nullptr || d->eval) return CGC_EINVAL;
   if (!aligned16(saved) || !aligned16(scratch) || !aligned16(grads)) return CGC_EINVAL;
   if ((d->flags & 8) && d_reg == nullptr) return CGC_EINVAL;
-  return run_level(d, const_cast<float*>(saved), scratch, stream, [&](const Ctx& c, Level& L) {
-    return level_bwd(c, L, emb, pool, jk, g, gptr, x_in, A_in, d_readout, d_x_out, d_A_out, grads, d_x_in, d_A_in, d_reg);
+  return run_level(d, const_cast<float*>(saved), scratch, stream, [&](Ctx& c, Level& L) {
+    Pending pending;
+    c.pending = &pending;
+    const int rc = level_bwd(c, L, emb, pool, jk, g, gptr, x_in, A_in, d_readout, d_x_out, d_A_out, grads, d_x_in, d_A_in, d_reg);
+    if (rc != 0) return rc;
+    return pending.n > 0 ? launch_deferred(pending.e, pending.n, as_stream(stream)) : 0;
   });
 }
diff --git a/cgc-net_amd/csrc/gemm.hip b/cgc-net_amd/csrc/gemm.hip
--- a/cgc-net_amd/csrc/gemm.hip
+++ b/cgc-net_amd/csrc/gemm.hip
@@ -1,4 +1,5 @@
 #include "gemm_common.hpp"
+#include "reduce_order.hpp"
 
 template <int ROWS>
 struct KContigLoader {
@@ -650,8 +651,7 @@
 __global__ void k_reduce_batch_sum(const float* __restrict__ ws, float* __restrict__ out, int parts, long long numel, float beta, int width,
                                    int ldo) {
   for (long long i = blockIdx.x * (long long)blockDim.x + threadIdx.x; i < numel; i += (long long)gridDim.x * blockDim.x) {
-    float s = 0.f;
-    for (int p = 0; p < parts; ++p) s += ws[(size_t)p * numel + i];
+    const float s = batch_sum_plain(ws, parts, numel, i);
     const long long o = (i / width) * ldo + i % width;
     out[o] = beta != 0.f ? s + beta * out[o] : s;
   }
@@ -664,25 +664,10 @@
   const int c = blockIdx.x * 32 + cl;
   ws += (size_t)blockIdx.y * parts * numel;
   out += (size_t)blockIdx.y * numel;
-  float s = 0.f;
-  if (c < numel) {
-    float a[8];
-#pragma unroll
-    for (int u = 0; u < 8; ++u) a[u] = 0.f;
-    int k = grp;
-    for (; k + 56 < parts; k += 64) {
-#pragma unroll
-      for (int u = 0; u < 8; ++u) a[u] += ws[(size_t)(k + 8 * u) * numel + c];
-    }
-    for (; k < parts; k += 8) a[0] += ws[(size_t)k * numel + c];
-    s = ((a[0] + a[1]) + (a[2] + a[3])) + ((a[4] + a[5]) + (a[6] + a[7]));
-  }
-  part[grp][cl] = s;
+  part[grp][cl] = c < numel ? many_parts_group_sum(ws, parts, numel, c, grp) : 0.f;
   __syncthreads();
   if (grp == 0 && c < numel) {
-    float t = part[0][cl];
-#pragma unroll
-    for (int g = 1; g < 8; ++g) t += part[g][cl];
+    const float t = many_parts_fold(part, cl);
     const int o = (c / width) * ldo + c % width;
     out[o] = beta != 0.f ? t + beta * out[o] : t;
   }
@@ -697,25 +682,9 @@
   return 0;
 }
 
-int reduce_batch_sum_rows(const float* ws, float* out, int parts, int rows, int width, int ldo, float beta, hipStream_t stream) {
-  const int64_t numel = (int64_t)rows * width;
-  if (numel <= 0) return 0;
-  if (width <= 0 || ldo < width || numel > 0x7fffffff) return CGC_EINVAL;
-  if (parts >= 16 && numel <= (1 << 20)) {
-    hipLaunchKernelGGL(k_reduce_many_parts, dim3((unsigned)ceil_div((int)numel, 32), 1u), dim3(256), 0, stream, ws, out, parts, (int)numel, beta,
-                       width, ldo);
-  } else {
-    const int64_t blocks = ceil_div64(numel, 256);
-    hipLaunchKernelGGL(k_reduce_batch_sum, dim3((unsigned)(blocks < 4096 ? blocks : 4096)), dim3(256), 0, stream, ws, out, parts,
-                       (long long)numel, beta, width, ldo);
-  }
-  CGC_RETURN_IF_LAUNCH_FAILED();
-  return 0;
-}
-
 extern "C" int cgc_reduce_batch_sum(const float* ws, float* out, int parts, int64_t numel, float beta, cgc_stream_t stream) {
   if (numel <= 0) return 0;
-  if (parts >= 16 && numel <= (1 << 20)) return cgc_reduce_batched(ws, out, 1, parts, (int)numel, beta, stream);
+  if (combine_many_parts(parts, numel)) return cgc_reduce_batched(ws, out, 1, parts, (int)numel, beta, stream);
   const int64_t blocks = ceil_div64(numel, 256);
   const int w = numel <= 0x7fffffff ? (int)numel : 0x7fffffff;
   hipLaunchKernelGGL(k_reduce_batch_sum, dim3((unsigned)(blocks < 4096 ? blocks : 4096)), dim3(256), 0, as_stream(stream), ws, out,
diff --git a/cgc-net_amd/csrc/groups.hpp b/cgc-net_amd/csrc/groups.hpp
--- a/cgc-net_amd/csrc/groups.hpp
+++ b/cgc-net_amd/csrc/groups.hpp
@@ -35,7 +35,20 @@
                            double count, hipStream_t st);
 int sage_narrow_bwd_groups(const SnBwdPtrs* g, float* const* dwdb, int ng, int ldy, int n, int F, int act, int normalize, int mode, double count,
                            int lda, int fin, int ldd, hipStream_t st);
+
+int sage_narrow_bwd_partials(const SnBwdPtrs* g, int ng, int ldy, int n, int F, int act, int normalize, int mode, double count, int lda, int fin,
+                             int ldd, int* slots, hipStream_t st);
+int bn_act_l2_bwd_partials(const float* dy, int ldy, const float* hn, const float* rinv, int n, int F, int act, int normalize, int mode,
+                           const float* mean, const float* istd, const float* gamma, const float* sums, double count, float* dh,
+                           int want_colsum, float* ws, int* slots_out, hipStream_t stream);
+int softmax_bwd_partials(const float* S, const float* dS, int n, int C, int ld, float* dx, int want_colsum, float* ws, int* slots_out,
+                         hipStream_t stream);
 int bn_act_apply_groups(const BnApplyPtrs* g, int ng, int n, int F, int act, int ldy, hipStream_t stream);
 int bn_bwd_reduce_groups(const BnRedPtrs* g, float* const* sums, int ng, int ldy, int n, int F, int act, hipStream_t stream);
 int launch_stats_finalize_groups(const StatsFinPtrs* g, int ng, int slots, int F, double count, hipStream_t stream);
 int launch_reduce_slots_f32_pair(const float* ws0, float* out0, const float* ws1, float* out1, int ng, int slots, int width, hipStream_t stream);
+
+int spmm_takes_addends(const float* x, const float* out, int width, int ld);
+int spmm_graphs_add(const int* rowptr, const int* col, const float* val, const float* pre, const float* post, const float* x, float* out, int n,
+                    int width, int ld, const int* gptr, int B, int nmax, const float* a, int lda, int wa, const float* b, int ldb,
+                    hipStream_t stream);
diff --git a/cgc-net_amd/csrc/jk.hip b/cgc-net_amd/csrc/jk.hip
--- a/cgc-net_amd/csrc/jk.hip
+++ b/cgc-net_amd/csrc/jk.hip
@@ -361,6 +361,14 @@
   return jk_mfma_bwd_flat(xs, dout, n, npad, C, w, HS, CS, dxs, flat, ws, as_stream(stream));
 }
 
+int jk_lstm_bwd_partials(const float* xs, const float* dout, int n, int npad, int C, const float* const* lstm, const float* w_att,
+                         const float* b_att, const float* HS, const float* CS, float* dxs, float* ws, int* parts, hipStream_t stream) {
+  if (!jk_npad_ok(n, npad)) return CGC_EINVAL;
+  JkWeights w;
+  fill_weights(w, lstm, w_att, b_att);
+  return jk_mfma_bwd_partials(xs, dout, n, npad, C, w, HS, CS, dxs, ws, parts, stream);
+}
+
 __global__ void k_jk_unpack(const float* __restrict__ G, int C, int H, float* __restrict__ flat) {
   const int NI = C + 2 * H + 1, NG = 4 * H + 1;
   const int per_dir = 4 * H * C + 4 * H * H + 8 * H, total = 2 * per_dir + 2 * H + 1;
diff --git a/cgc-net_amd/csrc/jk.hpp b/cgc-net_amd/csrc/jk.hpp
--- a/cgc-net_amd/csrc/jk.hpp
+++ b/cgc-net_amd/csrc/jk.hpp
@@ -28,3 +28,8 @@
                        const float* CS, float* dxs, float* G, float* ws, hipStream_t st);
 int jk_mfma_bwd_flat(const float* xs, const float* dout, int n, int npad, int C, const JkWeights& w, const float* HS, const float* CS,
                      float* dxs, float* flat, float* ws, hipStream_t st);
+int64_t jk_mfma_bwd_partials_floats(int n);
+int jk_mfma_bwd_partials(const float* xs, const float* dout, int n, int npad, int C, const JkWeights& w, const float* HS, const float* CS,
+                         float* dxs, float* ws, int* parts, hipStream_t st);
+int jk_lstm_bwd_partials(const float* xs, const float* dout, int n, int npad, int C, const float* const* lstm, const float* w_att,
+                         const float* b_att, const float* HS, const float* CS, float* dxs, float* ws, int* parts, hipStream_t stream);
diff --git a/cgc-net_amd/csrc/jk_mfma.hip b/cgc-net_amd/csrc/jk_mfma.hip
--- a/cgc-net_amd/csrc/jk_mfma.hip
+++ b/cgc-net_amd/csrc/jk_mfma.hip
@@ -1,4 +1,5 @@
 #include "jk.hpp"
+#include "reduce_order.hpp"
 
 typedef float floatx16 __attribute__((ext_vector_type(16)));
 
@@ -311,11 +312,7 @@
 __global__ void k_jk_pg_fold(const float* __restrict__ part, int P, int P2, int per, float* __restrict__ tmp) {
   const int e = blockIdx.x * blockDim.x + threadIdx.x, p2 = blockIdx.y, d = blockIdx.z;
   if (e >= per) return;
-  const float* src = part + ((size_t)d * P + (size_t)p2 * 16) * per + e;
-  const int cnt = min(16, P - p2 * 16);
-  float a = 0.f;
-  for (int k = 0; k < cnt; ++k) a += src[(size_t)k * per];
-  tmp[((size_t)d * P2 + p2) * per + e] = a;
+  tmp[((size_t)d * P2 + p2) * per + e] = jku_fold16(part + (size_t)d * P * per, P, p2, per, e);
 }
 
 template <int C>
@@ -788,23 +785,13 @@
 
 template <int C>
 __global__ void k_jku_finish_flat(const float* __restrict__ tmp, int P2, float* __restrict__ flat) {
-  constexpr int H = JkU<C>::H;
-  constexpr int per_dir = 4 * H * C + 4 * H * H + 8 * H, total = 2 * per_dir + 2 * H + 1;
+  static_assert(JkU<C>::PG_SLOTS == JKU_PG_SLOTS && JkU<C>::PG_FLOATS == JKU_PG_FLOATS, "reduce_order.hpp describes this layout");
   const int i = blockIdx.x * blockDim.x + threadIdx.x;
-  if (i >= total) return;
-  int d, row = 0, col = 0, att = -1;
-  if (i < 2 * per_dir) {
-    d = i / per_dir;
-    int e = i - d * per_dir;
-    if (e < 4 * H * C) { row = e / C; col = e % C; }
-    else if ((e -= 4 * H * C) < 4 * H * H) { row = e / H; col = C + e % H; }
-    else { e -= 4 * H * H; row = e % (4 * H); col = C + H; }
-  } else {
-    const int e = i - 2 * per_dir;
-    if (e < 2 * H) { d = e / H; att = e % H; }
-    else { d = 0; att = H; }
-  }
-  flat[i] = jku_gather<C>(tmp, P2, d, row, col, att);
+  if (i >= jku_flat_total(C)) return;
+  const int e = jku_flat_element(C, i);
+  float a = 0.f;
+  for (int k = 0; k < P2; ++k) a += tmp[(size_t)k * JKU_PG_FLOATS + e];
+  flat[i] = a;
 }
 
 template <int C>
@@ -863,7 +850,7 @@
 
 template <int C>
 static int launch_bwd_params(const float* xs, const float* dout, int n, int npad, const JkWeights& w, const float* HS, const float* CS,
-                             float* dxs, float* G, float* ws, hipStream_t st, float* flat) {
+                             float* dxs, float* G, float* ws, hipStream_t st, float* flat, int* parts_out = nullptr) {
   constexpr size_t lds = sizeof(float) * JkU<C>::BWD_TOTAL;
   static bool attr_set[CGC_MAX_DEVICES] = {};
   cgc_allow_lds(reinterpret_cast<const void*>(&k_jku_bwd<C>), (int)lds, attr_set);
@@ -872,6 +859,10 @@
   hipLaunchKernelGGL(k_jku_bwd<C>, dim3(grid), dim3(512), lds, st, xs, dout, n, npad, w, HS, CS, dxs, ws);
   CGC_RETURN_IF_LAUNCH_FAILED();
   constexpr int per = JkU<C>::PG_FLOATS, H = JkU<C>::H;
+  if (parts_out != nullptr) {
+    *parts_out = grid;
+    return 0;
+  }
   const int P = grid, P2 = ceil_div(P, 16);
   float* tmp = ws + (size_t)P * per;
   hipLaunchKernelGGL(k_jk_pg_fold, dim3(ceil_div(per, 256), P2, 1), dim3(256), 0, st, ws, P, P2, per, tmp);
@@ -934,3 +925,22 @@
     default: return CGC_EINVAL;
   }
 }
+
+int64_t jk_mfma_bwd_partials_floats(int n) {
+  const int grid = ceil_div(n > 0 ? n : 1, 32);
+  return (int64_t)(grid < 256 ? grid : 256) * JKU_PG_FLOATS;
+}
+int jk_mfma_bwd_partials(const float* xs, const float* dout, int n, int npad, int C, const JkWeights& w, const float* HS, const float* CS,
+                         float* dxs, float* ws, int* parts, hipStream_t st) {
+  if ((reinterpret_cast<uintptr_t>(xs) & 15u) || (reinterpret_cast<uintptr_t>(dout) & 15u) || (reinterpret_cast<uintptr_t>(dxs) & 15u) ||
+      n <= 0 || parts == nullptr)
+    return CGC_EINVAL;
+  switch (C) {
+    case 4: return launch_bwd_params<4>(xs, dout, n, npad, w, HS, CS, dxs, nullptr, ws, st, nullptr, parts);
+    case 8: return launch_bwd_params<8>(xs, dout, n, npad, w, HS, CS, dxs, nullptr, ws, st, nullptr, parts);
+    case 12: return launch_bwd_params<12>(xs, dout, n, npad, w, HS, CS, dxs, nullptr, ws, st, nullptr, parts);
+    case 16: return launch_bwd_params<16>(xs, dout, n, npad, w, HS, CS, dxs, nullptr, ws, st, nullptr, parts);
+    case 20: return launch_bwd_params<20>(xs, dout, n, npad, w, HS, CS, dxs, nullptr, ws, st, nullptr, parts);
+    default: return CGC_EINVAL;
+  }
+}
diff --git a/cgc-net_amd/csrc/reduce_order.hpp b/cgc-net_amd/csrc/reduce_order.hpp
--- /dev/null
+++ b/cgc-net_amd/csrc/reduce_order.hpp
@@ -0,0 +1,135 @@
+#pragma once
+#include <string.h>
+
+#include "common.hpp"
+
+#define RS_GROUPS 32
+template <typename IN>
+__device__ __forceinline__ double slots_group_sum(const IN* __restrict__ ws, int slots, int width, int c, int grp) {
+  double a[4] = {0.0, 0.0, 0.0, 0.0};
+  int k = grp;
+  for (; k + 15 * RS_GROUPS < slots; k += 16 * RS_GROUPS) {
+    IN v[16];
+#pragma unroll
+    for (int u = 0; u < 16; ++u) v[u] = ws[(size_t)(k + RS_GROUPS * u) * width + c];
+#pragma unroll
+    for (int u = 0; u < 16; ++u) a[u & 3] += (double)v[u];
+  }
+  for (; k + 3 * RS_GROUPS < slots; k += 4 * RS_GROUPS) {
+#pragma unroll
+    for (int u = 0; u < 4; ++u) a[u] += (double)ws[(size_t)(k + RS_GROUPS * u) * width + c];
+  }
+  for (; k < slots; k += RS_GROUPS) a[0] += (double)ws[(size_t)k * width + c];
+  return (a[0] + a[1]) + (a[2] + a[3]);
+}
+__device__ __forceinline__ double slots_fold(const double (*part)[32], int cl) {
+  double t[4] = {0.0, 0.0, 0.0, 0.0};
+#pragma unroll
+  for (int g = 0; g < RS_GROUPS; g += 4) { t[0] += part[g][cl]; t[1] += part[g + 1][cl]; t[2] += part[g + 2][cl]; t[3] += part[g + 3][cl]; }
+  return (t[0] + t[1]) + (t[2] + t[3]);
+}
+
+__device__ __forceinline__ float many_parts_group_sum(const float* __restrict__ ws, int parts, int numel, int c, int grp) {
+  float a[8];
+#pragma unroll
+  for (int u = 0; u < 8; ++u) a[u] = 0.f;
+  int k = grp;
+  for (; k + 120 < parts; k += 128) {
+    float v[16];
+#pragma unroll
+    for (int u = 0; u < 16; ++u) v[u] = ws[(size_t)(k + 8 * u) * numel + c];
+#pragma unroll
+    for (int u = 0; u < 16; ++u) a[u & 7] += v[u];
+  }
+  for (; k + 56 < parts; k += 64) {
+#pragma unroll
+    for (int u = 0; u < 8; ++u) a[u] += ws[(size_t)(k + 8 * u) * numel + c];
+  }
+  for (; k < parts; k += 8) a[0] += ws[(size_t)k * numel + c];
+  return ((a[0] + a[1]) + (a[2] + a[3])) + ((a[4] + a[5]) + (a[6] + a[7]));
+}
+__device__ __forceinline__ float many_parts_fold(const float (*part)[32], int cl) {
+  float t = part[0][cl];
+#pragma unroll
+  for (int g = 1; g < 8; ++g) t += part[g][cl];
+  return t;
+}
+
+__device__ __forceinline__ float batch_sum_plain(const float* __restrict__ ws, int parts, long long numel, long long i) {
+  float s = 0.f;
+  for (int p = 0; p < parts; p += 8) {
+    float v[8];
+#pragma unroll
+    for (int u = 0; u < 8; ++u) v[u] = ws[(size_t)min(p + u, parts - 1) * numel + i];
+#pragma unroll
+    for (int u = 0; u < 8; ++u)
+      if (p + u < parts) s += v[u];
+  }
+  return s;
+}
+static inline bool combine_many_parts(int parts, int64_t numel) { return parts >= 16 && numel <= (1 << 20); }
+
+#define JKU_PG_SLOTS 37
+#define JKU_PG_FLOATS (8 * JKU_PG_SLOTS * 64)
+#define JKU_FOLD 16
+__device__ __forceinline__ float jku_fold16(const float* __restrict__ part, int P, int p2, int per, int e) {
+  const float* src = part + (size_t)p2 * JKU_FOLD * per + e;
+  const int cnt = min(JKU_FOLD, P - p2 * JKU_FOLD);
+  float a = 0.f;
+  if (cnt == JKU_FOLD) {
+#pragma unroll
+    for (int k = 0; k < JKU_FOLD; ++k) a += src[(size_t)k * per];
+  } else {
+    for (int k = 0; k < cnt; ++k) a += src[(size_t)k * per];
+  }
+  return a;
+}
+__host__ __device__ static inline int jku_flat_total(int C) {
+  const int H = 3 * C / 2;
+  return 2 * (4 * H * C + 4 * H * H + 8 * H) + 2 * H + 1;
+}
+__device__ __forceinline__ int jku_flat_element(int C, int i) {
+  const int H = 3 * C / 2, per_dir = 4 * H * C + 4 * H * H + 8 * H;
+  int d, row = 0, col = 0, att = -1;
+  if (i < 2 * per_dir) {
+    d = i / per_dir;
+    int e = i - d * per_dir;
+    if (e < 4 * H * C) { row = e / C; col = e % C; }
+    else if ((e -= 4 * H * C) < 4 * H * H) { row = e / H; col = C + e % H; }
+    else { e -= 4 * H * H; row = e % (4 * H); col = C + H; }
+  } else {
+    const int e = i - 2 * per_dir;
+    if (e < 2 * H) { d = e / H; att = e % H; }
+    else { d = 0; att = H; }
+  }
+  if (att < 0) {
+    const int g = row / H, j = row - g * H, ww = j >> 3, u = j & 7, lhi = u >> 2, r = 4 * g + (u & 3);
+    const int m = col < C ? 1 : 0;
+    const int kin = col < C ? col : (col == C + H ? 31 : col - C);
+    return ((ww * 2 + d) * JKU_PG_SLOTS + m * 16 + r) * 64 + lhi * 32 + kin;
+  }
+  if (att < H) {
+    const int j = att, ww = j >> 3, u = j & 7, lhi = u >> 2;
+    return ((ww * 2 + d) * JKU_PG_SLOTS + 32 + (u & 3)) * 64 + lhi * 32;
+  }
+  return 36 * 64;
+}
+
+enum { DEF_SLOTS = 0, DEF_MANY_PARTS = 1, DEF_BATCH_SUM = 2, DEF_JK = 3 };
+struct DeferredEntry {
+  const float* src;
+  float* dst;
+  int kind;
+  int parts;
+  int stride;
+  int numel;
+  int width, ldo;
+  int first_block;
+  int reserved;
+};
+#define DEF_MAX_ENTRIES 16
+struct DeferredTable {
+  DeferredEntry e[DEF_MAX_ENTRIES];
+};
+static inline int deferred_chunk(int kind) { return kind == DEF_SLOTS ? 32 : kind == DEF_MANY_PARTS ? 128 : kind == DEF_BATCH_SUM ? 1024 : 64; }
+int launch_deferred(DeferredEntry* entries, int count, hipStream_t stream);
diff --git a/cgc-net_amd/csrc/rowops.hip b/cgc-net_amd/csrc/rowops.hip
--- a/cgc-net_amd/csrc/rowops.hip
+++ b/cgc-net_amd/csrc/rowops.hip
@@ -2,6 +2,7 @@
 
 #include "common.hpp"
 #include "groups.hpp"
+#include "reduce_order.hpp"
 
 #define L2_EPS 1e-12f
 #define RENORM_EPS 1e-15f
@@ -83,31 +84,14 @@
   }
 }
 
-#define RS_GROUPS 32
 template <typename OUT, typename IN = float>
 __global__ __launch_bounds__(32 * RS_GROUPS) void k_reduce_slots(const IN* __restrict__ ws, int slots, int width, OUT* __restrict__ out) {
   __shared__ double part[RS_GROUPS][32];
   const int cl = threadIdx.x & 31, grp = threadIdx.x >> 5;
   const int c = blockIdx.x * 32 + cl;
-  double s = 0.0;
-  if (c < width) {
-    double a[4] = {0.0, 0.0, 0.0, 0.0};
-    int k = grp;
-    for (; k + 3 * RS_GROUPS < slots; k += 4 * RS_GROUPS) {
-#pragma unroll
-      for (int u = 0; u < 4; ++u) a[u] += (double)ws[(size_t)(k + RS_GROUPS * u) * width + c];
-    }
-    for (; k < slots; k += RS_GROUPS) a[0] += (double)ws[(size_t)k * width + c];
-    s = (a[0] + a[1]) + (a[2] + a[3]);
-  }
-  part[grp][cl] = s;
+  part[grp][cl] = c < width ? slots_group_sum(ws, slots, width, c, grp) : 0.0;
   __syncthreads();
-  if (grp == 0 && c < width) {
-    double t[4] = {0.0, 0.0, 0.0, 0.0};
-#pragma unroll
-    for (int g = 0; g < RS_GROUPS; g += 4) { t[0] += part[g][cl]; t[1] += part[g + 1][cl]; t[2] += part[g + 2][cl]; t[3] += part[g + 3][cl]; }
-    out[c] = (OUT)((t[0] + t[1]) + (t[2] + t[3]));
-  }
+  if (grp == 0 && c < width) out[c] = (OUT)slots_fold(part, cl);
 }
 #define REDUCE_SLOTS_GRID(width) dim3(ceil_div((width), 32))
 
@@ -118,25 +102,9 @@
   __shared__ double part[RS_GROUPS][32];
   const int cl = threadIdx.x & 31, grp = threadIdx.x >> 5;
   const int c = blockIdx.x * 32 + cl;
-  double s = 0.0;
-  if (c < width) {
-    double a[4] = {0.0, 0.0, 0.0, 0.0};
-    int k = grp;
-    for (; k + 3 * RS_GROUPS < slots; k += 4 * RS_GROUPS) {
-#pragma unroll
-      for (int u = 0; u < 4; ++u) a[u] += (double)ws[(size_t)(k + RS_GROUPS * u) * width + c];
-    }
-    for (; k < slots; k += RS_GROUPS) a[0] += (double)ws[(size_t)k * width + c];
-    s = (a[0] + a[1]) + (a[2] + a[3]);
-  }
-  part[grp][cl] = s;
+  part[grp][cl] = c < width ? slots_group_sum(ws, slots, width, c, grp) : 0.0;
   __syncthreads();
-  if (grp == 0 && c < width) {
-    double t[4] = {0.0, 0.0, 0.0, 0.0};
-#pragma unroll
-    for (int g = 0; g < RS_GROUPS; g += 4) { t[0] += part[g][cl]; t[1] += part[g + 1][cl]; t[2] += part[g + 2][cl]; t[3] += part[g + 3][cl]; }
-    out[c] = (float)((t[0] + t[1]) + (t[2] + t[3]));
-  }
+  if (grp == 0 && c < width) out[c] = (float)slots_fold(part, cl);
 }
 int launch_reduce_slots_f32_pair(const float* ws0, float* out0, const float* ws1, float* out1, int ng, int slots, int width, hipStream_t stream) {
   hipLaunchKernelGGL(k_reduce_slots_pair, dim3(ceil_div(width, 32), ng), dim3(32 * RS_GROUPS), 0, stream, ws0, out0, ws1, out1, slots, width);
@@ -710,6 +678,23 @@
   if (ws != nullptr) col_reduce_store<VEC, MAXJ, 1>(csum, F, lpr, smem, ws + (size_t)blockIdx.x * F);
 }
 
+int bn_act_l2_bwd_partials(const float* dy, int ldy, const float* hn, const float* rinv, int n, int F, int act, int normalize, int mode,
+                           const float* mean, const float* istd, const float* gamma, const float* sums, double count, float* dh,
+                           int want_colsum, float* ws, int* slots_out, hipStream_t stream) {
+  if (want_colsum && ws == nullptr) return CGC_EINVAL;
+  const bool vec = (F % 4 == 0) && (ldy % 4 == 0) && aligned16(dy) && aligned16(hn) && aligned16(dh);
+  ColCfg cfg = col_cfg(n, F, vec);
+  if (!cfg.ok) return CGC_EINVAL;
+  if (!want_colsum) cfg.blocks = row_blocks(n, cfg.lpr);
+  const float inv_count = (float)(1.0 / count);
+  const size_t smem = sizeof(float) * (3 + 5) * F;
+  DISPATCH_COL(k_bn_act_l2_bwd, cfg, smem, stream, dy, ldy, hn, rinv, n, F, cfg.lpr, act, normalize, mode, mean, istd,
+               gamma, sums, inv_count, dh, want_colsum ? ws : (float*)nullptr);
+  CGC_RETURN_IF_LAUNCH_FAILED();
+  if (slots_out != nullptr) *slots_out = cfg.blocks;
+  return 0;
+}
+
 extern "C" int cgc_bn_act_l2_bwd(const float* dy, int ldy, const float* hn, const float* rinv, int n, int F, int act,
                                  int normalize, int mode, const float* mean, const float* istd, const float* gamma,
                                  const float* sums, double count, float* dh, float* dh_colsum, float* ws, cgc_stream_t stream) {
@@ -718,18 +703,12 @@
     if (dh_colsum) (void)hipMemsetAsync(dh_colsum, 0, sizeof(float) * F, as_stream(stream));
     return 0;
   }
-  if (dh_colsum != nullptr && ws == nullptr) return CGC_EINVAL;
-  const bool vec = (F % 4 == 0) && (ldy % 4 == 0) && aligned16(dy) && aligned16(hn) && aligned16(dh);
-  ColCfg cfg = col_cfg(n, F, vec);
-  if (!cfg.ok) return CGC_EINVAL;
-  if (dh_colsum == nullptr) cfg.blocks = row_blocks(n, cfg.lpr);
-  const float inv_count = (float)(1.0 / count);
-  const size_t smem = sizeof(float) * (3 + 5) * F;
-  DISPATCH_COL(k_bn_act_l2_bwd, cfg, smem, as_stream(stream), dy, ldy, hn, rinv, n, F, cfg.lpr, act, normalize, mode, mean, istd,
-               gamma, sums, inv_count, dh, dh_colsum ? ws : (float*)nullptr);
-  CGC_RETURN_IF_LAUNCH_FAILED();
+  int slots = 0;
+  const int rc = bn_act_l2_bwd_partials(dy, ldy, hn, rinv, n, F, act, normalize, mode, mean, istd, gamma, sums, count, dh, dh_colsum != nullptr,
+                                        ws, &slots, as_stream(stream));
+  if (rc != 0) return rc;
   if (dh_colsum) {
-    hipLaunchKernelGGL(k_reduce_slots<float>, REDUCE_SLOTS_GRID(F), dim3(32 * RS_GROUPS), 0, as_stream(stream), ws, cfg.blocks, F, dh_colsum);
+    hipLaunchKernelGGL(k_reduce_slots<float>, REDUCE_SLOTS_GRID(F), dim3(32 * RS_GROUPS), 0, as_stream(stream), ws, slots, F, dh_colsum);
     CGC_RETURN_IF_LAUNCH_FAILED();
   }
   return 0;
@@ -933,6 +912,20 @@
   return 0;
 }
 
+int softmax_bwd_partials(const float* S, const float* dS, int n, int C, int ld, float* dx, int want_colsum, float* ws, int* slots_out,
+                         hipStream_t stream) {
+  if (ld < C || (want_colsum && ws == nullptr)) return CGC_EINVAL;
+  const bool vec = (C % 4 == 0) && (ld % 4 == 0) && aligned16(S) && aligned16(dS) && aligned16(dx);
+  ColCfg cfg = col_cfg(n, C, vec);
+  if (!cfg.ok) return CGC_EINVAL;
+  if (!want_colsum) cfg.blocks = row_blocks(n, cfg.lpr);
+  const size_t smem = want_colsum ? sizeof(float) * 3 * C : 0;
+  DISPATCH_COL(k_softmax_bwd, cfg, smem, stream, S, dS, n, C, ld, cfg.lpr, dx, want_colsum ? ws : (float*)nullptr);
+  CGC_RETURN_IF_LAUNCH_FAILED();
+  if (slots_out != nullptr) *slots_out = cfg.blocks;
+  return 0;
+}
+
 extern "C" int cgc_softmax_bwd(const float* S, const float* dS, int n, int C, int ld, float* dx, float* dx_colsum, float* ws,
                                cgc_stream_t stream) {
   if (C <= 0) return 0;
@@ -941,16 +934,11 @@
     if (dx_colsum) (void)hipMemsetAsync(dx_colsum, 0, sizeof(float) * C, as_stream(stream));
     return 0;
   }
-  if (dx_colsum != nullptr && ws == nullptr) return CGC_EINVAL;
-  const bool vec = (C % 4 == 0) && (ld % 4 == 0) && aligned16(S) && aligned16(dS) && aligned16(dx);
-  ColCfg cfg = col_cfg(n, C, vec);
-  if (!cfg.ok) return CGC_EINVAL;
-  if (dx_colsum == nullptr) cfg.blocks = row_blocks(n, cfg.lpr);
-  const size_t smem = dx_colsum ? sizeof(float) * 3 * C : 0;
-  DISPATCH_COL(k_softmax_bwd, cfg, smem, as_stream(stream), S, dS, n, C, ld, cfg.lpr, dx, dx_colsum ? ws : (float*)nullptr);
-  CGC_RETURN_IF_LAUNCH_FAILED();
+  int slots = 0;
+  const int rc = softmax_bwd_partials(S, dS, n, C, ld, dx, dx_colsum != nullptr, ws, &slots, as_stream(stream));
+  if (rc != 0) return rc;
   if (dx_colsum) {
-    hipLaunchKernelGGL(k_reduce_slots<float>, REDUCE_SLOTS_GRID(C), dim3(32 * RS_GROUPS), 0, as_stream(stream), ws, cfg.blocks, C, dx_colsum);
+    hipLaunchKernelGGL(k_reduce_slots<float>, REDUCE_SLOTS_GRID(C), dim3(32 * RS_GROUPS), 0, as_stream(stream), ws, slots, C, dx_colsum);
     CGC_RETURN_IF_LAUNCH_FAILED();
   }
   return 0;
diff --git a/cgc-net_amd/csrc/sagenarrow.hip b/cgc-net_amd/csrc/sagenarrow.hip
--- a/cgc-net_amd/csrc/sagenarrow.hip
+++ b/cgc-net_amd/csrc/sagenarrow.hip
@@ -155,6 +155,17 @@
     for (int i = 0; i < ng; ++i) (void)hipMemsetAsync(dwdb[i], 0, sizeof(float) * width, st);
     return 0;
   }
+  int slots = 0;
+  const int rc = sage_narrow_bwd_partials(g, ng, ldy, n, F, act, normalize, mode, count, lda, fin, ldd, &slots, st);
+  if (rc != 0) return rc;
+  return launch_reduce_slots_f32_pair(g[0].ws, dwdb[0], g[ng - 1].ws, dwdb[ng - 1], ng, slots, width, st);
+}
+
+int sage_narrow_bwd_partials(const SnBwdPtrs* g, int ng, int ldy, int n, int F, int act, int normalize, int mode, double count, int lda, int fin,
+                             int ldd, int* slots, hipStream_t st) {
+  if (F <= 0 || fin <= 0 || n <= 0 || F > 32 || fin > 32 || ng < 1 || ng > 2) return CGC_EINVAL;
+  for (int i = 0; i < ng; ++i)
+    if (g[i].ws == nullptr || (g[i].dagg != nullptr && ldd < fin)) return CGC_EINVAL;
   const int tiles = ceil_div(n, 32), grid = sn_grid(n);
   const float inv_count = (float)(1.0 / count);
   const int fs = (F + 1) / 2;
@@ -173,7 +184,8 @@
 #undef SN_ACT
 #undef SN_LAUNCH
   CGC_RETURN_IF_LAUNCH_FAILED();
-  return launch_reduce_slots_f32_pair(g[0].ws, dwdb[0], g1.ws, dwdb[ng - 1], ng, grid, width, st);
+  *slots = grid;
+  return 0;
 }
 
 extern "C" int cgc_sage_narrow_bwd(const float* dy, int ldy, const float* hn, const float* rinv, int n, int F, int act, int normalize,
diff --git a/cgc-net_amd/csrc/spmm.hip b/cgc-net_amd/csrc/spmm.hip
--- a/cgc-net_amd/csrc/spmm.hip
+++ b/cgc-net_amd/csrc/spmm.hip
@@ -1,13 +1,18 @@
 #include "common.hpp"
 
 constexpr int GATHER_U = 9;
+
+struct SpmmAddends {
+  const float *a, *b;
+  int lda, ldb, wa;
+};
 
 template <int VEC>
 __global__ __launch_bounds__(256) void k_spmm(const int* __restrict__ rowptr, const int* __restrict__ col, const int* __restrict__ perm,
                                               const float* __restrict__ val, const float* __restrict__ pre,
                                               const float* __restrict__ post, const float* __restrict__ x, float* __restrict__ out,
                                               int n, int W, int ld, int lpr, int n_ctiles, int rows_per_block, int blocks_per_ct,
-                                              int n_chunks, int nt_store, const int* __restrict__ gptr) {
+                                              int n_chunks, int nt_store, const int* __restrict__ gptr, const SpmmAddends add) {
   const int nb = gridDim.x, b = blockIdx.x;
   const int vb = (nb % 8 == 0) ? (b % 8) * (nb / 8) + b / 8 : b;
   const int per_chunk = blocks_per_ct * n_ctiles;
@@ -75,7 +80,17 @@
     if (valid && colok) {
       const float ps = post != nullptr ? post[r] : 1.f;
       float* op = out + (size_t)r * ld + c0;
-      if (nt_store && VEC == 4) {
+      if (add.a != nullptr) {
+        Vec<VEC> o;
+#pragma unroll
+        for (int v = 0; v < VEC; ++v) {
+          const int c = c0 + v;
+          float t = 0.f;
+          if (c < W) t = c < add.wa ? add.a[(size_t)r * add.lda + c] : add.b[(size_t)r * add.ldb + (c - add.wa)];
+          o.v[v] = __fadd_rn(__fmul_rn(acc[v], ps), t);
+        }
+        o.store(op);
+      } else if (nt_store && VEC == 4) {
         typedef float f4v __attribute__((ext_vector_type(4)));
         f4v o4 = {acc[0] * ps, acc[VEC > 1 ? 1 : 0] * ps, acc[VEC > 2 ? 2 : 0] * ps, acc[VEC > 3 ? 3 : 0] * ps};
         __builtin_nontemporal_store(o4, reinterpret_cast<f4v*>(op));
@@ -192,10 +207,12 @@
 
 static int launch_gather(const int* rowptr, const int* col, const int* perm, const float* val, const float* pre, const float* post,
                          const float* x, float* out, int n, int width, int ld, const int* gptr, int B, int nmax, int order,
-                         hipStream_t stream, const int* gorder = nullptr) {
+                         hipStream_t stream, const int* gorder = nullptr, const SpmmAddends* add = nullptr) {
   const bool vec = (width % 4 == 0) && (ld % 4 == 0) && aligned16(x) && aligned16(out);
   const int chunks = vec ? width / 4 : width;
   const int lpr = pick_lpr(chunks);
+  if (add != nullptr && vec && lpr == 64) return CGC_EINVAL;
+  const SpmmAddends ad = add != nullptr ? *add : SpmmAddends{nullptr, nullptr, 0, 0, 0};
   const int n_ctiles = ceil_div(chunks, lpr);
   const int rpw = 64 / lpr;
   const int rows_per_block = 4 * rpw * SPMM_PASSES;
@@ -239,10 +256,10 @@
   const int nt = n_ctiles > 1 ? 1 : 0;
   if (vec)
     hipLaunchKernelGGL(k_spmm<4>, grid, block, 0, stream, rowptr, col, perm, val, pre, post, x, out, n, width, ld, lpr,
-                       n_ctiles, rows_per_block, blocks_per_ct, n_chunks, nt, gptr);
+                       n_ctiles, rows_per_block, blocks_per_ct, n_chunks, nt, gptr, ad);
   else
     hipLaunchKernelGGL(k_spmm<1>, grid, block, 0, stream, rowptr, col, perm, val, pre, post, x, out, n, width, ld, lpr,
-                       n_ctiles, rows_per_block, blocks_per_ct, n_chunks, nt, gptr);
+                       n_ctiles, rows_per_block, blocks_per_ct, n_chunks, nt, gptr, ad);
   CGC_RETURN_IF_LAUNCH_FAILED();
   return 0;
 }
@@ -263,3 +280,20 @@
   cgc_timing_end(trec, as_stream(stream));
   return rc;
 }
+
+int spmm_takes_addends(const float* x, const float* out, int width, int ld) {
+  const bool vec = (width % 4 == 0) && (ld % 4 == 0) && aligned16(x) && aligned16(out);
+  return !(vec && pick_lpr(width / 4) == 64);
+}
+int spmm_graphs_add(const int* rowptr, const int* col, const float* val, const float* pre, const float* post, const float* x, float* out, int n,
+                    int width, int ld, const int* gptr, int B, int nmax, const float* a, int lda, int wa, const float* b, int ldb,
+                    hipStream_t stream) {
+  if (n <= 0 || width <= 0) return 0;
+  if (ld < width || a == nullptr || wa < 0 || wa > width || (wa < width && b == nullptr) || lda < wa || (wa < width && ldb < width - wa))
+    return CGC_EINVAL;
+  const SpmmAddends add{a, b, lda, ldb, wa};
+  const int trec = width > 64 ? cgc_timing_begin(CGC_TAG_SPMM_WIDE, n, width, ld, val != nullptr, 0, 0, 0, stream) : -1;
+  const int rc = launch_gather(rowptr, col, nullptr, val, pre, post, x, out, n, width, ld, gptr, B, nmax, 0, stream, nullptr, &add);
+  cgc_timing_end(trec, stream);
+  return rc;
+}
```
